# zbqq/aicp_mapping

Hardware: AMD Instinct MI355X
Metric: aligned_clouds_per_s (ICP iterations/sec + aligned clouds/sec, 80-scan VLP-16 batch) (higher is better)
Workload: dtype f32 (point arithmetic; 6x6/3x3 reductions and solves in f64)

## Files before the change

### aicp_mapping_amd/_lib.py

```python
from __future__ import annotations

import ctypes as C
import hashlib
import os

import numpy as np

PKG_DIR = os.path.dirname(os.path.abspath(__file__))
LIB_PATH = os.environ.get("AICP_HIP_LIB") or os.path.join(PKG_DIR, "libaicp_hip.so")

AICP_OK = 0
AICP_ERR_CONVERGENCE = 1
AICP_ERR_INVALID = 2
AICP_ERR_HIP = 3
AICP_ERR_UNSUPPORTED = 4
AICP_ERR_TRANSFORMATION = 5

AICP_RUN_OVERLAP = 1
AICP_RUN_ICP = 2
AICP_RUN_TIME_NN = 4
AICP_SEQ_DEBUG = 8

EXPORTS = [
    "aicp_hip_create", "aicp_hip_destroy", "aicp_hip_last_error", "aicp_hip_version",
    "aicp_hip_default_config", "aicp_hip_parse_pm_yaml", "aicp_hip_replace_ratio_config_file",
    "aicp_hip_autotune_ratio", "aicp_hip_register", "aicp_hip_register_batch",
    "aicp_hip_overlap", "aicp_hip_overlap_batch", "aicp_hip_align_batch", "aicp_hip_transform", "aicp_hip_crop_box",
    "aicp_hip_batch_upload", "aicp_hip_batch_run", "aicp_hip_batch_free",
    "aicp_hip_last_nn_timing", "aicp_hip_last_phase_ms", "aicp_hip_knn", "aicp_hip_normals",
    "aicp_hip_dists_quantile", "aicp_hip_solve6", "aicp_hip_default_prefilter", "aicp_hip_prefilter",
    "aicp_hip_last_prefilter_stats", "aicp_hip_map_create", "aicp_hip_map_free", "aicp_hip_map_size",
    "aicp_hip_map_download", "aicp_hip_map_crop", "aicp_hip_map_merge", "aicp_hip_map_prefilter",
    "aicp_hip_default_sequence_params", "aicp_hip_sequence_run", "aicp_hip_last_sequence_timing",
    "aicp_hip_map_register_batch", "aicp_hip_multi_create", "aicp_hip_multi_destroy", "aicp_hip_multi_size",
    "aicp_hip_multi_context", "aicp_hip_multi_last_error", "aicp_hip_multi_align_batch",
    "aicp_hip_reference_cache_stats", "aicp_hip_default_options", "aicp_hip_set_options", "aicp_hip_get_options",
    "aicp_hip_test_force_scan_stall", "aicp_hip_sequence_run_raw", "aicp_hip_build_info",
]


_NEWEST = {"aicp_hip_reference_cache_stats", "aicp_hip_default_options", "aicp_hip_set_options",
           "aicp_hip_get_options", "aicp_hip_test_force_scan_stall",
           "aicp_hip_sequence_run_raw", "aicp_hip_build_info"}


class IcpConfig(C.Structure):
    _fields_ = [
        ("knn_normals", C.c_int32),
        ("nn_epsilon", C.c_float),
        ("nn_max_dist", C.c_float),
        ("trimmed_ratio", C.c_float),
        ("max_iter", C.c_int32),
        ("min_diff_rot", C.c_float),
        ("min_diff_trans", C.c_float),
        ("smooth_length", C.c_int32),
        ("bucket_size", C.c_int32),
        ("knn_match", C.c_int32),
    ]


class IcpStats(C.Structure):
    _fields_ = [
        ("status", C.c_int32),
        ("iterations", C.c_int32),
        ("converged", C.c_int32),
        ("degenerate_normals", C.c_int32),
        ("inlier_ratio", C.c_float),
        ("trimmed_ratio", C.c_float),
        ("overlap_percent", C.c_float),
        ("tree_depth", C.c_int32),
        ("nn_points_touched", C.c_uint64),
        ("nn_nodes_touched", C.c_uint64),
        ("overlap_keys", C.c_uint64 * 3),
    ]

    def as_dict(self):
        d = {k: getattr(self, k) for k, _ in self._fields_ if k != "overlap_keys"}
        d["overlap_keys"] = [int(x) for x in self.overlap_keys]
        return d


class Pair(C.Structure):
    _fields_ = [
        ("ref", C.POINTER(C.c_float)),
        ("n_ref", C.c_uint64),
        ("ref_stride", C.c_uint64),
        ("read", C.POINTER(C.c_float)),
        ("n_read", C.c_uint64),
        ("read_stride", C.c_uint64),
        ("init_T", C.POINTER(C.c_float)),
        ("ref_origin", C.c_double * 3),
        ("read_origin", C.c_double * 3),
    ]


class PrefilterParams(C.Structure):
    _fields_ = [
        ("leaf_size", C.c_float),
        ("normal_k", C.c_int32),
        ("neighbours", C.c_int32),
        ("min_cluster_size", C.c_int32),
        ("max_cluster_size", C.c_int32),
        ("smoothness_rad", C.c_float),
        ("curvature_threshold", C.c_float),
        ("viewpoint", C.c_float * 3),
    ]


class PrefilterStats(C.Structure):
    _fields_ = [
        ("voxel_ms", C.c_double),
        ("normals_ms", C.c_double),
        ("segment_ms", C.c_double),
        ("device_ms", C.c_double),
        ("wall_ms", C.c_double),
        ("knn_ms", C.c_double),
        ("knn_queries", C.c_uint64),
        ("knn_points_touched", C.c_uint64),
        ("knn_nodes_touched", C.c_uint64),
        ("propagation_passes", C.c_int32),
        ("pad", C.c_int32),
    ]


class Cloud(C.Structure):
    _fields_ = [
# ... 31 lines not shown


class Options(C.Structure):
    _fields_ = [
        ("profile", C.c_int32),
        ("nn_engine", C.c_int32),
        ("overlap_path", C.c_int32),
        ("normals_knn_engine", C.c_int32),
        ("select_pair", C.c_int32),
        ("select_fused_from", C.c_int32),
        ("raw_tree_first", C.c_int32),
        ("raw_first_at", C.c_int32),
        ("no_early_exit", C.c_int32),
        ("tree_plan", C.c_int32),
        ("tree_lvl_min", C.c_uint32),
        ("reference_cache", C.c_int32),
        ("oneshot_keep_mib", C.c_uint32),
        ("early_reference", C.c_int32),
        ("read_order_min", C.c_uint64),
    ]

    def as_dict(self):
        return {k: getattr(self, k) for k, _ in self._fields_}


class SequenceTiming(C.Structure):
    _fields_ = [
        ("windows", C.c_int32),
        ("replans", C.c_int32),
        ("wall_ms", C.c_double),
        ("device_ms", C.c_double),
    ]


def _load():
    if not os.path.exists(LIB_PATH):
        raise ImportError(
            f"{LIB_PATH} is missing: build it with `python -c 'import __graft_entry__ as g; g.build()'` "
            "(hipcc --offload-arch=gfx950). There is no CPU fallback.")
    L = C.CDLL(LIB_PATH)
    for name in EXPORTS:
        if not hasattr(L, name) and not (os.environ.get("AICP_HIP_LIB") and name in _NEWEST):
            raise ImportError(f"{LIB_PATH} does not export {name}")
    vp = C.c_void_p
    fp = C.POINTER(C.c_float)
    dp = C.POINTER(C.c_double)
    ip = C.POINTER(C.c_int32)
    up = C.POINTER(C.c_uint64)
    cfgp = C.POINTER(IcpConfig)
    stp = C.POINTER(IcpStats)
    pp = C.POINTER(Pair)
    sz = C.c_size_t
    L.aicp_hip_create.argtypes = [C.c_int, C.POINTER(vp)]
    L.aicp_hip_destroy.argtypes = [vp]
    L.aicp_hip_destroy.restype = None
    L.aicp_hip_last_error.argtypes = [vp]
    L.aicp_hip_last_error.restype = C.c_char_p
    L.aicp_hip_version.restype = C.c_char_p
    if hasattr(L, "aicp_hip_build_info"):
        L.aicp_hip_build_info.restype = C.c_char_p
    L.aicp_hip_default_config.argtypes = [cfgp]
    L.aicp_hip_default_config.restype = None
    L.aicp_hip_parse_pm_yaml.argtypes = [C.c_char_p, cfgp]
    L.aicp_hip_replace_ratio_config_file.argtypes = [C.c_char_p, C.c_char_p, C.c_float]
    L.aicp_hip_autotune_ratio.argtypes = [C.c_float]
    L.aicp_hip_autotune_ratio.restype = C.c_float
    L.aicp_hip_register.argtypes = [vp, cfgp, pp, fp, stp]
    L.aicp_hip_register_batch.argtypes = [vp, cfgp, pp, sz, fp, stp]
    L.aicp_hip_overlap.argtypes = [vp, pp, C.c_double, fp]
    L.aicp_hip_overlap_batch.argtypes = [vp, pp, sz, C.c_double, fp, stp]
    L.aicp_hip_align_batch.argtypes = [vp, cfgp, pp, sz, C.c_double, C.c_int, fp, stp]
    L.aicp_hip_transform.argtypes = [vp, fp, fp, sz, sz, fp]
    L.aicp_hip_crop_box.argtypes = [vp, fp, sz, sz, C.c_float, C.c_float, fp, fp, C.POINTER(C.c_size_t), fp]
    L.aicp_hip_batch_upload.argtypes = [vp, pp, sz, C.POINTER(vp)]
    L.aicp_hip_batch_run.argtypes = [vp, vp, cfgp, C.c_double, C.c_int, fp, stp]
    L.aicp_hip_batch_free.argtypes = [vp, vp]
    L.aicp_hip_batch_free.restype = None
    L.aicp_hip_last_nn_timing.argtypes = [vp, C.POINTER(C.c_int), dp, dp, up]
    L.aicp_hip_last_phase_ms.argtypes = [vp, dp]
    L.aicp_hip_knn.argtypes = [vp, fp, sz, sz, fp, sz, sz, C.c_int, C.c_float, C.c_float, ip, fp, up]
    L.aicp_hip_normals.argtypes = [vp, fp, sz, sz, C.c_int, fp, ip]
    L.aicp_hip_dists_quantile.argtypes = [vp, fp, sz, C.c_float, fp]
    L.aicp_hip_solve6.argtypes = [vp, dp, dp, dp, ip]
    L.aicp_hip_default_prefilter.argtypes = [C.POINTER(PrefilterParams)]
    L.aicp_hip_default_prefilter.restype = None
    L.aicp_hip_prefilter.argtypes = [vp, C.POINTER(PrefilterParams), fp, sz, sz, fp, C.POINTER(C.c_size_t), fp, ip,
                                     C.POINTER(C.c_size_t), C.POINTER(C.c_size_t)]
    L.aicp_hip_last_prefilter_stats.argtypes = [vp, C.POINTER(PrefilterStats)]
    szp = C.POINTER(C.c_size_t)
    L.aicp_hip_map_create.argtypes = [vp, fp, sz, sz, C.POINTER(vp)]
    L.aicp_hip_map_free.argtypes = [vp, vp]
    L.aicp_hip_map_free.restype = None
    L.aicp_hip_map_size.argtypes = [vp, szp]
    L.aicp_hip_map_download.argtypes = [vp, vp, fp, sz, szp]
    L.aicp_hip_map_crop.argtypes = [vp, vp, C.c_float, C.c_float, fp, fp, sz, szp]
    L.aicp_hip_map_merge.argtypes = [vp, vp, fp, sz, sz, fp]
    L.aicp_hip_map_prefilter.argtypes = [vp, vp, C.POINTER(PrefilterParams)]
    L.aicp_hip_default_sequence_params.argtypes = [C.POINTER(SequenceParams)]
    L.aicp_hip_default_sequence_params.restype = None
    L.aicp_hip_sequence_run.argtypes = [vp, cfgp, C.POINTER(SequenceParams), C.POINTER(Cloud), C.POINTER(Cloud), sz,
                                        fp, C.POINTER(SequenceResult), C.POINTER(C.c_size_t)]
    L.aicp_hip_last_sequence_timing.argtypes = [vp, C.POINTER(SequenceTiming)]
    if hasattr(L, "aicp_hip_sequence_run_raw"):
        L.aicp_hip_sequence_run_raw.argtypes = [vp, cfgp, C.POINTER(SequenceParams), C.POINTER(PrefilterParams),
                                                C.POINTER(Cloud), C.POINTER(Cloud), sz, fp, C.POINTER(SequenceResult),
                                                C.POINTER(C.c_size_t)]
    L.aicp_hip_map_register_batch.argtypes = [vp, cfgp, vp, C.c_float, C.c_float, C.POINTER(Cloud), fp, sz, C.c_int,
                                              fp, stp]
    if hasattr(L, "aicp_hip_reference_cache_stats"):
        L.aicp_hip_reference_cache_stats.argtypes = [vp, C.POINTER(C.c_uint64)]
    if hasattr(L, "aicp_hip_set_options"):
        L.aicp_hip_default_options.argtypes = [C.POINTER(Options)]
        L.aicp_hip_default_options.restype = None
        L.aicp_hip_set_options.argtypes = [vp, C.POINTER(Options)]
        L.aicp_hip_get_options.argtypes = [vp, C.POINTER(Options)]
        L.aicp_hip_test_force_scan_stall.argtypes = [C.c_int]
    L.aicp_hip_multi_create.argtypes = [ip, C.c_int, C.POINTER(vp)]
    L.aicp_hip_multi_destroy.argtypes = [vp]
    L.aicp_hip_multi_destroy.restype = None
    L.aicp_hip_multi_size.argtypes = [vp]
    L.aicp_hip_multi_context.argtypes = [vp, C.c_int]
    L.aicp_hip_multi_context.restype = vp
    L.aicp_hip_multi_last_error.argtypes = [vp]
    L.aicp_hip_multi_last_error.restype = C.c_char_p
    L.aicp_hip_multi_align_batch.argtypes = [vp, cfgp, pp, sz, C.c_double, C.c_int, fp, stp, ip]
    return L


lib = _load()


def build_info() -> str:
    return lib.aicp_hip_build_info().decode() if hasattr(lib, "aicp_hip_build_info") else ""


def source_hash(csrc: str = os.path.join(PKG_DIR, "csrc")) -> str:
    mk = os.path.join(csrc, "Makefile")
    lists = {}
    text = open(mk).read().replace("\\\n", " ")
    for line in text.splitlines():
        for key in ("SRCS_HIP", "SRCS_CPP", "HDRS"):
            if line.startswith(key + " ="):
                lists[key] = line.split("=", 1)[1].split()
    h = hashlib.sha256()
    for f in lists["SRCS_HIP"] + lists["SRCS_CPP"] + lists["HDRS"] + ["Makefile"]:
        with open(os.path.join(csrc, f), "rb") as fh:
            h.update(fh.read())
    return h.hexdigest()[:16]


def provenance() -> dict:
    info = build_info()
    src = info.split()[1] if info.startswith("src ") else ""
    try:
        tree = source_hash()
    except OSError:
        tree = ""
    return {"library": os.path.abspath(LIB_PATH), "build_info": info, "tree_source_hash": tree,
            "built_from_tree": bool(src) and src == tree}


class AicpError(RuntimeError):
    def __init__(self, code, msg):
        super().__init__(f"aicp_hip error {code}: {msg}")
        self.code = code

# ... 58 lines not shown
    ref = as_points(ref)
    read = as_points(read)
    keep = [ref, read]
    p = Pair()
    p.ref = _fptr(ref)
    p.n_ref = ref.shape[0]
    p.ref_stride = ref.shape[1] * 4
    p.read = _fptr(read)
    p.n_read = read.shape[0]
    p.read_stride = read.shape[1] * 4
    if init_T is not None:
        t = np.ascontiguousarray(np.asarray(init_T, np.float32).reshape(4, 4).T.reshape(16))
        keep.append(t)
        p.init_T = _fptr(t)
    for k in range(3):
        p.ref_origin[k] = float(ref_origin[k])
        p.read_origin[k] = float(read_origin[k])
    return p, keep


def default_sequence_params(**kw) -> SequenceParams:
    p = SequenceParams()
    lib.aicp_hip_default_sequence_params(C.byref(p))
    for k, v in kw.items():
        setattr(p, k, v)
    return p


def make_cloud(pts, origin=(0, 0, 0)):
    a = as_points(pts)
    c = Cloud()
    c.pts = _fptr(a)
    c.n = a.shape[0]
    c.stride = a.shape[1] * 4
    for k in range(3):
        c.origin[k] = float(origin[k])
    return c, a


def default_prefilter(**kw) -> PrefilterParams:
    p = PrefilterParams()
    lib.aicp_hip_default_prefilter(C.byref(p))
    for k, v in kw.items():
        if k == "viewpoint":
            for i in range(3):
                p.viewpoint[i] = float(v[i])
        else:
            setattr(p, k, v)
    return p


CONTEXT_OPTIONS: dict = {}


class Context:

    def __init__(self, device: int = 0):
        h = C.c_void_p()
        rc = lib.aicp_hip_create(int(device), C.byref(h))
        if rc != AICP_OK:
            raise AicpError(rc, f"aicp_hip_create(device={device}) failed (no HIP device?)")
        self.h = h
        self.device = device
        if CONTEXT_OPTIONS:
            self.set_options(**CONTEXT_OPTIONS)

    def close(self):
        if getattr(self, "h", None):
            lib.aicp_hip_destroy(self.h)
            self.h = None

    def __del__(self):
        self.close()

    def last_error(self) -> str:
        return lib.aicp_hip_last_error(self.h).decode()

    def get_options(self) -> Options:
        o = Options()
        self.check(lib.aicp_hip_get_options(self.h, C.byref(o)))
        return o

    def set_options(self, opt: Options = None, **kw) -> Options:
        old = self.get_options()
        new = Options.from_buffer_copy(opt if opt is not None else old)
        for k, v in kw.items():
            if not hasattr(new, k):
                raise AttributeError(f"aicp_hip_options has no field {k}")
            setattr(new, k, v)
        self.check(lib.aicp_hip_set_options(self.h, C.byref(new)))
        return old

    def options(self, **kw):
        ctx = self

        class _Scope:
            def __enter__(self):
                self.old = ctx.set_options(**kw)
                return ctx

            def __exit__(self, *exc):
                ctx.set_options(self.old)
                return False

        return _Scope()

    def check(self, rc):
        if rc == AICP_ERR_CONVERGENCE:
            raise ConvergenceError(rc, self.last_error())
        if rc == AICP_ERR_TRANSFORMATION:
            raise TransformationError(rc, self.last_error())
        if rc != AICP_OK:
            raise AicpError(rc, self.last_error())

    def align_batch(self, pairs, cfg=None, resolution=0.2, flags=AICP_RUN_ICP, raise_on_error=True):
        cfg = cfg or default_config()
        arr = (Pair * len(pairs))()
        keep = []
        for i, pr in enumerate(pairs):
            p, k = make_pair(pr["ref"], pr["read"], pr.get("ref_origin", (0, 0, 0)),
                             pr.get("read_origin", (0, 0, 0)), pr.get("init_T"))
            arr[i] = p
            keep.append(k)
        outT = np.zeros((len(pairs), 16), np.float32)
        st = (IcpStats * len(pairs))()
        rc = lib.aicp_hip_align_batch(self.h, C.byref(cfg), arr, len(pairs), float(resolution),
                                      int(flags), _fptr(outT), st)
        if raise_on_error and rc != AICP_OK:
            self.check(rc)
        T = outT.reshape(-1, 4, 4).transpose(0, 2, 1).copy()
        return T, [s.as_dict() for s in st], rc

    def register(self, ref, read, cfg=None):
        cfg = cfg or default_config()
        p, keep = make_pair(ref, read)
        outT = np.zeros(16, np.float32)
        st = IcpStats()
        self.check(lib.aicp_hip_register(self.h, C.byref(cfg), C.byref(p), _fptr(outT), C.byref(st)))
        return outT.reshape(4, 4).T.copy(), st.as_dict()

    def overlap(self, ref, read, ref_origin=(0, 0, 0), read_origin=(0, 0, 0), resolution=0.2):
        p, keep = make_pair(ref, read, ref_origin, read_origin)
        out = np.zeros(1, np.float32)
        self.check(lib.aicp_hip_overlap(self.h, C.byref(p), float(resolution), _fptr(out)))
        return float(out[0])

    def reference_cache_stats(self):
        a = (C.c_uint64 * 4)()
        self.check(lib.aicp_hip_reference_cache_stats(self.h, a))
        return dict(tree_hits=a[0], tree_builds=a[1], ovl_hits=a[2], ovl_builds=a[3])

    def upload(self, pairs):
        return ResidentBatch(self, pairs)

    def sequence_run(self, first, first_origin, readings, origins, cfg=None, params=None, raise_on_error=True,
                     prefilter=None):
        cfg = cfg or default_config()
        prm = params or default_sequence_params()
        if prefilter is True:
            prefilter = default_prefilter()
        n = len(readings)
        fc, keep0 = make_cloud(first, first_origin)
        arr = (Cloud * max(n, 1))()
        keep = [keep0]
        for i, r in enumerate(readings):
            c, k = make_cloud(r, origins[i])
            arr[i] = c
            keep.append(k)
        outT = np.zeros((max(n, 1), 16), np.float32)
        res = (SequenceResult * max(n, 1))()
        done = C.c_size_t(0)
        if prefilter is not None:
            rc = lib.aicp_hip_sequence_run_raw(self.h, C.byref(cfg), C.byref(prm), C.byref(prefilter), C.byref(fc), arr,
                                               n, _fptr(outT), res, C.byref(done))
        else:
            rc = lib.aicp_hip_sequence_run(self.h, C.byref(cfg), C.byref(prm), C.byref(fc), arr, n, _fptr(outT), res,
                                           C.byref(done))
        if raise_on_error and rc != AICP_OK:
            self.check(rc)
        T = outT[:n].reshape(-1, 4, 4).transpose(0, 2, 1).copy()
        return T, [res[i].as_dict() for i in range(done.value)], done.value, rc

    def last_sequence_timing(self):
        t = SequenceTiming()
        self.check(lib.aicp_hip_last_sequence_timing(self.h, C.byref(t)))
        return {k: getattr(t, k) for k, _ in SequenceTiming._fields_}

    def last_nn_timing(self):
        n = C.c_int()
        ms = C.c_double()
        by = C.c_double()
        q = C.c_uint64()
        lib.aicp_hip_last_nn_timing(self.h, C.byref(n), C.byref(ms), C.byref(by), C.byref(q))
        return dict(launches=n.value, total_ms=ms.value, bytes=by.value, queries=q.value)

    def last_phase_ms(self):
        a = (C.c_double * 5)()
        lib.aicp_hip_last_phase_ms(self.h, a)
        return dict(overlap=a[0], normals=a[1], matcher_tree=a[2], icp_loop=a[3], total=a[4])

    def knn(self, pts, queries, k=1, eps=0.0, max_dist=float("inf")):
        pts = as_points(pts)
        q = as_points(queries)
        ids = np.zeros((q.shape[0], k), np.int32)
        d2 = np.zeros((q.shape[0], k), np.float32)
        touched = np.zeros(2, np.uint64)
        rc = lib.aicp_hip_knn(self.h, _fptr(pts), pts.shape[0], pts.shape[1] * 4, _fptr(q), q.shape[0],
                              q.shape[1] * 4, int(k), float(eps), float(max_dist),
                              ids.ctypes.data_as(C.POINTER(C.c_int32)), _fptr(d2),
                              touched.ctypes.data_as(C.POINTER(C.c_uint64)))
        self.check(rc)
        return ids, d2, int(touched[0]), int(touched[1])

    def normals(self, pts, knn=20):
        pts = as_points(pts)
        out = np.zeros((pts.shape[0], 3), np.float32)
        deg = C.c_int32()
        rc = lib.aicp_hip_normals(self.h, _fptr(pts), pts.shape[0], pts.shape[1] * 4, int(knn), _fptr(out),
                                  C.byref(deg))
        self.check(rc)
        return out, deg.value

    def dists_quantile(self, d2, quantile):
        d2 = np.ascontiguousarray(d2, np.float32).ravel()
        out = C.c_float()
        rc = lib.aicp_hip_dists_quantile(self.h, _fptr(d2), d2.size, float(quantile), C.byref(out))
        self.check(rc)
        return out.value

    def solve6(self, A, b):
        A = np.ascontiguousarray(A, np.float64).reshape(36)
        b = np.ascontiguousarray(b, np.float64).reshape(6)
        x = np.zeros(6, np.float64)
        path = C.c_int32()
        dp = C.POINTER(C.c_double)
        rc = lib.aicp_hip_solve6(self.h, A.ctypes.data_as(dp), b.ctypes.data_as(dp), x.ctypes.data_as(dp),
                                 C.byref(path))
        self.check(rc)
        return x, path.value

    def transform(self, T, pts):
        pts = as_points(pts)
        t = np.ascontiguousarray(np.asarray(T, np.float32).reshape(4, 4).T.reshape(16))
        out = np.zeros((pts.shape[0], 3), np.float32)
        rc = lib.aicp_hip_transform(self.h, _fptr(t), _fptr(pts), pts.shape[0], pts.shape[1] * 4, _fptr(out))
        self.check(rc)
        return out

    def crop_box(self, pts, mn, mx, origin):
        pts = as_points(pts)
        o = np.ascontiguousarray(np.asarray(origin, np.float32).reshape(4, 4).T.reshape(16))
        out = np.zeros((pts.shape[0], 3), np.float32)
        m = C.c_size_t(0)
        rpy = np.zeros(3, np.float32)
        rc = lib.aicp_hip_crop_box(self.h, _fptr(pts), pts.shape[0], pts.shape[1] * 4, mn, mx, _fptr(o),
                                   _fptr(out), C.byref(m), _fptr(rpy))
        self.check(rc)
        return out[:m.value].copy(), rpy

    def last_prefilter_stats(self):
        st = PrefilterStats()
        self.check(lib.aicp_hip_last_prefilter_stats(self.h, C.byref(st)))
        return {k: getattr(st, k) for k, _ in PrefilterStats._fields_ if k != "pad"}

    def prefilter(self, pts, params=None, details=False):
        pts = as_points(pts)
        n = pts.shape[0]
        prm = params or default_prefilter()
        out = np.zeros((max(n, 1), 3), np.float32)
        m, ns, nc = C.c_size_t(0), C.c_size_t(0), C.c_size_t(0)
        sampled = np.zeros((max(n, 1), 8), np.float32) if details else None
        labels = np.zeros(max(n, 1), np.int32) if details else None
        rc = lib.aicp_hip_prefilter(self.h, C.byref(prm), _fptr(pts), n, pts.shape[1] * 4, _fptr(out), C.byref(m),
                                    _fptr(sampled) if details else None,
                                    labels.ctypes.data_as(C.POINTER(C.c_int32)) if details else None,
                                    C.byref(ns), C.byref(nc))
        self.check(rc)
        if not details:
            return out[:m.value].copy()
        V = ns.value
        return dict(out=out[:m.value].copy(), sampled=sampled[:V].copy(), labels=labels[:V].copy(),
                    n_clusters=nc.value)


class ResidentBatch:

    def __init__(self, ctx: Context, pairs):
        self.ctx = ctx
        self.n = len(pairs)
        arr = (Pair * self.n)()
        keep = []
        for i, pr in enumerate(pairs):
            p, k = make_pair(pr["ref"], pr["read"], pr.get("ref_origin", (0, 0, 0)),
                             pr.get("read_origin", (0, 0, 0)), pr.get("init_T"))
            arr[i] = p
            keep.append(k)
        h = C.c_void_p()
        rc = lib.aicp_hip_batch_upload(ctx.h, arr, self.n, C.byref(h))
        ctx.check(rc)
        self.h = h
        self.outT = np.zeros((self.n, 16), np.float32)
        self.stats = (IcpStats * self.n)()

    def run(self, cfg=None, resolution=0.2, flags=AICP_RUN_ICP | AICP_RUN_OVERLAP, raise_on_error=True):
        cfg = cfg or default_config()
        rc = lib.aicp_hip_batch_run(self.ctx.h, self.h, C.byref(cfg), float(resolution), int(flags),
                                    _fptr(self.outT), self.stats)
        if raise_on_error and rc != AICP_OK:
            self.ctx.check(rc)
        return rc

    def transforms(self):
        return self.outT.reshape(-1, 4, 4).transpose(0, 2, 1).copy()

    def stats_dicts(self):
        return [s.as_dict() for s in self.stats]

    def free(self):
        if getattr(self, "h", None):
            lib.aicp_hip_batch_free(self.ctx.h, self.h)
# ... 49 lines not shown
```

### aicp_mapping_amd/csrc/aicp_hip.cpp

```cpp
#include <hip/hip_runtime.h>

#include <algorithm>
#include <atomic>
#include <deque>
#include <chrono>
#include <cmath>
#include <cstdio>
#include <cstdlib>
#include <cstring>
#include <limits>
#include <string>
#include <thread>
#include <vector>

#include "../../include/aicp_hip.h"
#include "aicp_common.hpp"
#include "icp_math.hpp"
#include "kernels.hpp"
#include "runtime.hpp"

using namespace aicp;
using namespace aicp::rt;

namespace aicp {
// ... 795 lines not shown
    HIPC(hipEventRecord(ctx->ev[9], s));
    prm.maxE2 = (1 + cfg->nn_epsilon) * (1 + cfg->nn_epsilon);
    prm.maxR2 = cfg->nn_max_dist * cfg->nn_max_dist;
    prm.max_iter = cfg->max_iter;
    prm.smooth = cfg->smooth_length;
    prm.min_rot = cfg->min_diff_rot;
    prm.min_trans = cfg->min_diff_trans;
    prm.knn_normals = cfg->knn_normals;
    uint32_t reads = 0, max_read = 0;
    for (size_t i = 0; i < P; ++i) {
      reads += B->desc[i].n_read;
      max_read = std::max(max_read, B->desc[i].n_read);
    }
    ActiveList* al = ctx->active.as<ActiveList>();
    const int sel_ff = ctx->opt.select_fused_from;
    const bool sel_pair = sel_pair_fits(P, max_read, ctx->opt.select_pair);
    if (!ctx->poll_host) {
      HIPC(hipHostMalloc((void**)&ctx->poll_host, kBatchPolls * 4, hipHostMallocMapped));
      HIPC(hipHostGetDevicePointer((void**)&ctx->poll_dev, ctx->poll_host, 0));
    }
    const bool early = !ctx->opt.no_early_exit;
    auto polled = [&](int k) { return early && k >= cfg->smooth_length && k < kBatchPolls && k < cfg->max_iter; };
    auto written = [&](int k) { return early && k < kBatchPolls; };
    std::deque<int> pending;
    bool stop = false;
    for (int it = 0; it < cfg->max_iter && !stop; ++it) {
      while (!pending.empty() && pending.front() < it && !stop) {
        const int k = pending.front();
        volatile uint32_t* w = ctx->poll_host;
        const auto t0 = std::chrono::steady_clock::now();
        while (w[k] == 0xffffffffu) {
          int m = k - 1;
          while (m >= 0 && w[m] == 0xffffffffu) --m;
          if (m >= 0 && w[m] == 0u) break;
          if (std::chrono::steady_clock::now() - t0 > std::chrono::milliseconds(20)) {
            const hipError_t q = hipStreamQuery(s);
            if (q != hipErrorNotReady) {
              HIPC(q);
              std::atomic_thread_fence(std::memory_order_seq_cst);
              break;
            }
          }
          std::this_thread::yield();
        }
        stop = w[k] == 0u || w[k] == 0xffffffffu;
        pending.pop_front();
      }
      if (stop) break;
      if (it == 0) {
        uint32_t* hn0 = nullptr;
        if (written(0)) {
          ctx->poll_host[0] = 0xffffffffu;
          hn0 = ctx->poll_dev;
        }
        launch_active_list(s, (int)P, dDesc, dState, al, dCtr, hn0);
      }
      prm.prof_slot = nn_launches;
      launch_icp_nn(s, (int)reads, dDesc, dState, al, readc, nodes, ctx->tl_total ? ctx->tl.as<uint4>() : nullptr,
                    nullptr, bpts, ctx->tl_total ? ctx->ptl.as<uint2>() : nullptr, ctx->match.as<int32_t>(),
                    ctx->d2.as<float>(), ctx->touch.as<uint32_t>(), dCtr, prm,
                    timeNN ? ctx->nn_ev[2 * nn_launches] : nullptr, timeNN ? ctx->nn_ev[2 * nn_launches + 1] : nullptr);
      HIPC(hipGetLastError());
      ++nn_launches;
      IcpIterSync y = icp_sync_layout(ctx->isync.as<uint32_t>(), P, 0);
      y.np = (int)P;
      y.pd = dDesc;
      y.st = dState;
      y.al = al;
      y.ctr = dCtr;
      if (written(it + 1)) {
        ctx->poll_host[it + 1] = 0xffffffffu;
        y.host_n = ctx->poll_dev + it + 1;
        if (polled(it + 1)) pending.push_back(it + 1);
      }
      if (sel_pair)
        launch_icp_select_pair(s, (int)P, dDesc, dState, ctx->d2.as<float>(), ctx->sel_cand.as<uint32_t>(), y);
      else if (sel_ff > 0 && it >= sel_ff)
        launch_icp_select_fused(s, B->m_sel, dDesc, dState, ctx->d2.as<float>(), ctx->sel_hist.as<uint32_t>(),
                                ctx->sel_cand.as<uint32_t>(), ctx->sel_cnt.as<uint32_t>(), y);
      else
        launch_icp_select_f(s, B->m_sel, dDesc, dState, ctx->d2.as<float>(), ctx->sel_hist.as<uint32_t>(),
                            ctx->sel_cand.as<uint32_t>(), ctx->sel_cnt.as<uint32_t>(), y);
      launch_icp_reduce_f(s, B->m_red, dDesc, dState, readc, ctx->match.as<int32_t>(), ctx->d2.as<float>(),
                          ctx->touch.as<uint32_t>(), bpts, bnrm, ctx->slab.as<double>(), prm, y);
    }
    launch_finalize(s, (int)P, dDesc, dState, ctx->outT.as<float>());
    if (ctx->opt.profile) {
      HIPC(hipStreamSynchronize(s));
      nn_prof_dump();
      tree_prof_dump();
    }
  } else {
    HIPC(hipEventRecord(ctx->ev[8], s));
    HIPC(hipEventRecord(ctx->ev[10], s));
    HIPC(hipEventRecord(ctx->ev[12], s));
    HIPC(hipEventRecord(ctx->ev[3], s));
    HIPC(hipEventRecord(ctx->ev[4], s));
    HIPC(hipEventRecord(ctx->ev[9], s));
  }
  HIPC(hipGetLastError());
  HIPC(hipEventRecord(ctx->ev[5], s));
  HIPC(hipMemcpyAsync(ctx->pin_state.p, dState, P * sizeof(PairState), hipMemcpyDeviceToHost, s));
  if (doIcp) HIPC(hipMemcpyAsync(ctx->pin_out.p, ctx->outT.p, P * 64, hipMemcpyDeviceToHost, s));
  HIPC(hipMemcpyAsync(pdC, dDesc, P * sizeof(PairDesc), hipMemcpyDeviceToHost, s));
  HIPC(hipStreamSynchronize(s));
  if (doIcp && !hit_trees) {
    rcache.trees = false;
    rc = device_trees_check(ctx->tb[0], ctx->err);
    if (!rc) rc = device_trees_check(ctx->tb[1], ctx->err);
    if (rc) return rc;
    if (ctx->tl_total && (ctx->tb[1].pin_ctl.as<TreeCtl>()->error & 4))
      FAIL(AICP_ERR_HIP, "matcher treelets exceed their allotment");
    if (rcache.use && R == 1) {
      rcache.trees = true;
      rcache.bucket = cfg->bucket_size;
      rcache.knn = cfg->knn_normals;
      rcache.tl_total = ctx->tl_total;
      ++rcache.tree_builds;
    }
  }
  const PairState* hs = ctx->pin_state.as<PairState>();
  int first_err = AICP_OK;
  uint64_t queries = 0, tp = 0, tn = 0;
  for (size_t i = 0; i < P; ++i) {
    const PairState& st = hs[i];
    int status = st.status;
    if (doOvl && st.ovl_err && !status) status = AICP_ERR_HIP;
    if (status && !first_err) first_err = status;
    if (outT && doIcp) std::memcpy(outT + 16 * i, ctx->pin_out.as<float>() + 16 * i, 64);
    if (out_overlap) out_overlap[i] = st.overlap;
    queries += (uint64_t)st.iters * desc[i].n_read;
    const uint64_t ptp = st.touched_pts, ptn = st.touched_nodes;
    tp += ptp;
    tn += ptn;
    if (stats) {
      aicp_icp_stats& o = stats[i];
      std::memset(&o, 0, sizeof(o));
      o.status = status;
      o.iterations = st.iters;
      o.converged = st.converged;
      o.degenerate_normals = st.degenerate;
      o.inlier_ratio = st.inlier_ratio;
      o.trimmed_ratio = st.ratio;
      o.overlap_percent = st.overlap;
      o.tree_depth = pdC[i].tree_depth;
      o.nn_points_touched = ptp;
      o.nn_nodes_touched = ptn;
      for (int k = 0; k < 3; ++k) o.overlap_keys[k] = st.ovl_counts[k];
    }
  }
  ctx->last_nn_launches = timeNN ? nn_launches : 0;
  ctx->last_nn_ms = 0;
  if (timeNN)
    for (int it = 0; it < nn_launches; ++it) ctx->last_nn_ms += ev_ms(ctx->nn_ev[2 * it], ctx->nn_ev[2 * it + 1]);
  ctx->last_nn_bytes = timeNN ? (double)queries * 20.0 + (double)tp * 16.0 + (double)tn * 8.0 : 0.0;
  ctx->last_queries = queries;
  ctx->last_phase[0] = doOvl ? ev_ms(ctx->ev[0], ctx->ev[1]) + ev_ms(ctx->ev[6], ctx->ev[2]) : 0;
  ctx->last_phase[1] = doIcp ? ev_ms(ctx->ev[8], ctx->ev[10]) : 0;
  ctx->last_phase[2] = doIcp ? ev_ms(ctx->ev[12], ctx->ev[3]) : 0;
  ctx->last_phase[3] = doIcp ? ev_ms(ctx->ev[9], ctx->ev[5]) : 0;
  ctx->last_phase[4] =
      std::chrono::duration<double, std::milli>(std::chrono::steady_clock::now() - t_start).count();
  if (first_err) ctx->err = "pair status " + std::to_string(first_err);
  return first_err;
}

void free_batch(aicp_hip_batch* B) {
  if (!B) return;
  release(B->ref_raw);
  release(B->read_raw);
  release(B->maps);
  delete B;
}

int upload_tree(aicp_hip_ctx* ctx, const float* pts, size_t n, size_t stride, PairDesc& d) {
  hipStream_t s = ctx->stream;
  ctx->refc.invalidate();
  HIPC(ensure(ctx->ref1, n * 16));
  HIPC(ensure(ctx->pin_io, n * 16));
  pack_xyz4(pts, n, stride, ctx->pin_io.as<float>());
  HIPC(hipMemcpyAsync(ctx->ref1.p, ctx->pin_io.p, n * 16, hipMemcpyHostToDevice, s));
  d = PairDesc{};
  d.n_ref = (uint32_t)n;
  d.ratio = 0.5f;
  ident4(d.Tin);
  HIPC(ensure(ctx->desc, sizeof(PairDesc)));
  HIPC(hipMemcpyAsync(ctx->desc.p, &d, sizeof(d), hipMemcpyHostToDevice, s));
  int rc = device_trees_begin(ctx->tb[0], ctx->err, s, 1, n, ctx->desc.as<PairDesc>(), ctx->ref1.as<float4>(), 0, 8,
                              ctx->bpts, ctx->nodes);
  if (rc) return rc;
  rc = device_trees_end(ctx->tb[0], ctx->err, s, 1, n, ctx->desc.as<PairDesc>(), 8, ctx->bpts, ctx->nodes, 0);
  if (rc) return rc;
  HIPC(hipMemcpyAsync(&d, ctx->desc.p, sizeof(d), hipMemcpyDeviceToHost, s));
  HIPC(hipStreamSynchronize(s));
  return AICP_OK;
}

}
}

extern "C" {

const char* aicp_hip_version(void) { return "aicp_hip 0.1 (gfx950)"; }

void aicp_hip_default_options(aicp_hip_options* o) {
  if (!o) return;
  *o = aicp_hip_options{};
  o->select_pair = -1;
  o->select_fused_from = 3;
  o->raw_tree_first = -1;
  o->raw_first_at = 2;
  o->tree_lvl_min = 1u << 22;
  o->reference_cache = 1;
  o->oneshot_keep_mib = 4096;
  o->early_reference = 1;
  o->read_order_min = kReadOrderMin;
}

int aicp_hip_set_options(aicp_hip_ctx* ctx, const aicp_hip_options* o) {
  if (!ctx || !o) return AICP_ERR_INVALID;
  if (o->nn_engine < 0 || o->nn_engine > 1 || o->overlap_path < 0 || o->overlap_path > 1 ||
      o->normals_knn_engine < 0 || o->normals_knn_engine > 2 || o->select_pair < -1 || o->select_pair > 1 ||
      o->select_fused_from < 0 || o->raw_tree_first < -1 || o->raw_tree_first > 1 || o->raw_first_at < 1 ||
      o->raw_first_at > 2 || o->tree_plan < -1 || o->reference_cache < 0 || o->reference_cache > 1 ||
      o->early_reference < 0 || o->early_reference > 1)
    FAIL(AICP_ERR_INVALID, "aicp_hip_set_options: value out of range");
  ctx->refc.invalidate();
  ctx->rdc.valid = false;
  ctx->opt = *o;
  for (auto& t : ctx->tb) tree_opts(t, ctx->opt);
  return AICP_OK;
}

int aicp_hip_get_options(const aicp_hip_ctx* ctx, aicp_hip_options* out) {
  if (!ctx || !out) return AICP_ERR_INVALID;
  *out = ctx->opt;
  return AICP_OK;
}

int aicp_hip_test_force_scan_stall(int on) { return set_lb_force_stall(on) == hipSuccess ? AICP_OK : AICP_ERR_HIP; }

int aicp_hip_create(int device, aicp_hip_ctx** out) {
  if (!out) return AICP_ERR_INVALID;
  *out = nullptr;
  int n = 0;
  if (hipGetDeviceCount(&n) != hipSuccess || n <= 0) return AICP_ERR_HIP;
  if (device < 0 || device >= n) return AICP_ERR_INVALID;
  if (hipSetDevice(device) != hipSuccess) return AICP_ERR_HIP;
  aicp_hip_ctx* c = new aicp_hip_ctx();
  c->device = device;
  aicp_hip_default_options(&c->opt);
  for (auto& t : c->tb) tree_opts(t, c->opt);
  int prio_lo = 0, prio_hi = 0;
  if (hipDeviceGetStreamPriorityRange(&prio_lo, &prio_hi) != hipSuccess) prio_lo = prio_hi = 0;
  const int prio3 = prio_hi;
  if (hipStreamCreateWithPriority(&c->stream, hipStreamNonBlocking, prio_lo) != hipSuccess ||
      hipStreamCreateWithPriority(&c->stream2, hipStreamNonBlocking, prio_hi) != hipSuccess ||
      hipStreamCreateWithPriority(&c->stream3, hipStreamNonBlocking, prio3) != hipSuccess) {
    for (hipStream_t q : {c->stream, c->stream2, c->stream3})
      if (q) (void)hipStreamDestroy(q);
    delete c;
    return AICP_ERR_HIP;
  }
  *out = c;
  return AICP_OK;
}

void aicp_hip_destroy(aicp_hip_ctx* ctx) {
  if (!ctx) return;
  (void)hipSetDevice(ctx->device);
  (void)hipDeviceSynchronize();
  for (DevBuf* b : {&ctx->read_s, &ctx->ord_k0, &ctx->ord_k1, &ctx->ord_v0, &ctx->ord_v1, &ctx->ord_tmp, &ctx->read_c, &ctx->bpts, &ctx->bnrm, &ctx->nodes, &ctx->match, &ctx->d2, &ctx->desc,
                    &ctx->state, &ctx->touch, &ctx->slab, &ctx->bitmap, &ctx->outT, &ctx->scratch, &ctx->active,
                    &ctx->ctrs, &ctx->nbids, &ctx->ref1, &ctx->sel_hist, &ctx->sel_cand, &ctx->sel_cnt,
                    &ctx->qmap, &ctx->ovl, &ctx->rdesc, &ctx->rstate, &ctx->rdesc_raw, &ctx->bpts_raw,
                    &ctx->nodes_raw, &ctx->nrm_raw, &ctx->inv, &ctx->gdesc, &ctx->gstate, &ctx->tl, &ctx->ptl,
                    &ctx->tl_rank, &ctx->pf_a, &ctx->pf_b, &ctx->pf_bpts, &ctx->pf_nodes})
    release(*b);
  for (auto& t : ctx->tb) t.release_all();
  free_batch(ctx->oneshot);
  free_batch(ctx->mapbatch);
  release(ctx->crop_ws);
  release(ctx->ovl_sp);
  release(ctx->ovl_keys);
  release(ctx->isync);
  release(ctx->refc.gst);
  release(ctx->pin_crop);
  release(ctx->pin_maps);
  if (ctx->poll_host) (void)hipHostFree(ctx->poll_host);
  delete ctx->pool;
  seq_state_free(ctx->seq);
  for (PinBuf* b : {&ctx->pin_desc, &ctx->pin_state, &ctx->pin_out, &ctx->pin_io, &ctx->pin_ovl,
                    &ctx->pin_rdesc, &ctx->pin_gdesc, &ctx->pin_gstate, &ctx->pin_pf})
    release(*b);
  for (auto e : ctx->nn_ev) (void)hipEventDestroy(e);
  for (auto e : ctx->ev)
    if (e) (void)hipEventDestroy(e);
  for (auto e : ctx->pf_ev)
    if (e) (void)hipEventDestroy(e);
  (void)hipStreamDestroy(ctx->stream);
  if (ctx->stream2) (void)hipStreamDestroy(ctx->stream2);
  if (ctx->stream3) (void)hipStreamDestroy(ctx->stream3);
  delete ctx;
}

const char* aicp_hip_last_error(const aicp_hip_ctx* ctx) { return ctx ? ctx->err.c_str() : "null context"; }

int aicp_hip_batch_upload(aicp_hip_ctx* ctx, const aicp_pair* pairs, size_t n_pairs, aicp_hip_batch** out) {
  if (!ctx || !out) return AICP_ERR_INVALID;
  HIPC(hipSetDevice(ctx->device));
  aicp_hip_batch* B = new aicp_hip_batch();
  const int rc = upload_pairs(ctx, pairs, n_pairs, B, false);
  if (rc) {
    free_batch(B);
    *out = nullptr;
    return rc;
  }
  *out = B;
  return AICP_OK;
}

// ... 332 lines not shown
  HIPC(hipMemcpy(out_ids, ctx->match.p, nq * (size_t)k * 4, hipMemcpyDeviceToHost));
  HIPC(hipMemcpy(out_d2, ctx->d2.p, nq * (size_t)k * 4, hipMemcpyDeviceToHost));
  if (out_touched) HIPC(hipMemcpy(out_touched, ctx->scratch.p, 16, hipMemcpyDeviceToHost));
  return AICP_OK;
}

int aicp_hip_normals(aicp_hip_ctx* ctx, const float* pts, size_t n, size_t stride, int knn, float* out_normals,
                     int32_t* out_degenerate) {
  if (!ctx || !pts || !out_normals || n == 0 || stride < 12) return AICP_ERR_INVALID;
  HIPC(hipSetDevice(ctx->device));
  PairDesc d;
  int rc = upload_tree(ctx, pts, n, stride, d);
  if (rc) return rc;
  hipStream_t st_ = ctx->stream;
  HIPC(ensure(ctx->state, sizeof(PairState)));
  HIPC(ensure(ctx->bnrm, n * 16));
  HIPC(ensure(ctx->nbids, n * 4 * (size_t)std::max(knn, 1)));
  HIPC(ensure(ctx->ctrs, kCtrWords * 4));
  HIPC(hipMemsetAsync(ctx->ctrs.p, 0, kCtrWords * 4, st_));
  launch_init_state(st_, 1, ctx->desc.as<PairDesc>(), ctx->state.as<PairState>());
  if (!launch_normals(st_, 1, (uint32_t)n, ctx->desc.as<PairDesc>(), ctx->state.as<PairState>(),
                      ctx->nodes.as<uint4>(), nullptr, ctx->bpts.as<float4>(),
                      ctx->bnrm.as<float4>(), knn, ctx->nbids.as<int32_t>(), ctx->ctrs.as<uint32_t>(),
                      ctx->opt.normals_knn_engine))
    FAIL(AICP_ERR_UNSUPPORTED, "knn must be 10, 20 or 30");
  HIPC(hipGetLastError());
  HIPC(hipStreamSynchronize(st_));
  std::vector<float> nb(4 * n), bp(4 * n);
  HIPC(hipMemcpy(nb.data(), ctx->bnrm.p, n * 16, hipMemcpyDeviceToHost));
  HIPC(hipMemcpy(bp.data(), ctx->bpts.p, n * 16, hipMemcpyDeviceToHost));
  PairState st;
  HIPC(hipMemcpy(&st, ctx->state.p, sizeof(st), hipMemcpyDeviceToHost));
  for (size_t j = 0; j < n; ++j) {
    int32_t id;
    std::memcpy(&id, &bp[4 * j + 3], 4);
    for (int k = 0; k < 3; ++k) out_normals[3 * (size_t)id + k] = nb[4 * j + k];
  }
  if (out_degenerate) *out_degenerate = st.degenerate;
  return AICP_OK;
}

int aicp_hip_dists_quantile(aicp_hip_ctx* ctx, const float* d2, size_t n, float quantile, float* out_limit) {
  if (!ctx || !d2 || !out_limit || n == 0 || n >= (1ull << 31)) return AICP_ERR_INVALID;
  if (!(quantile >= 0.f && quantile <= 1.f)) return AICP_ERR_INVALID;
  HIPC(hipSetDevice(ctx->device));
  hipStream_t st_ = ctx->stream;
  PairDesc d{};
  d.n_read = (uint32_t)n;
  d.ratio = quantile;
  HIPC(ensure(ctx->desc, sizeof(PairDesc)));
  HIPC(ensure(ctx->state, sizeof(PairState)));
  HIPC(ensure(ctx->d2, n * 4));
  HIPC(ensure(ctx->pin_io, n * 4));
  std::memcpy(ctx->pin_io.p, d2, n * 4);
  HIPC(hipMemcpyAsync(ctx->desc.p, &d, sizeof(d), hipMemcpyHostToDevice, st_));
  HIPC(hipMemcpyAsync(ctx->d2.p, ctx->pin_io.p, n * 4, hipMemcpyHostToDevice, st_));
  const uint32_t per = kNNBlock * kSelPerThread, nb = (uint32_t)((n + per - 1) / per);
  HIPC(ensure(ctx->qmap, (size_t)nb * 8));
  HIPC(ensure(ctx->pin_desc, (size_t)nb * 8));
  uint32_t* hm = ctx->pin_desc.as<uint32_t>();
  for (uint32_t b = 0; b < nb; ++b) {
    hm[b] = 0;
    hm[nb + b] = b * per;
  }
  HIPC(hipMemcpyAsync(ctx->qmap.p, hm, (size_t)nb * 8, hipMemcpyHostToDevice, st_));
  BlockMap qm{ctx->qmap.as<int32_t>(), ctx->qmap.as<uint32_t>() + nb, nb};
  HIPC(ensure(ctx->sel_hist, kHistBins * 4));
  HIPC(ensure(ctx->sel_cand, n * 4));
  HIPC(ensure(ctx->sel_cnt, 4));
  HIPC(hipMemsetAsync(ctx->sel_hist.p, 0, kHistBins * 4, st_));
  HIPC(hipMemsetAsync(ctx->sel_cnt.p, 0, 4, st_));
  launch_init_state(st_, 1, ctx->desc.as<PairDesc>(), ctx->state.as<PairState>());
  launch_icp_select(st_, qm, 1, ctx->desc.as<PairDesc>(), ctx->state.as<PairState>(), ctx->d2.as<float>(),
                    ctx->sel_hist.as<uint32_t>(), ctx->sel_cand.as<uint32_t>(), ctx->sel_cnt.as<uint32_t>());
  HIPC(hipGetLastError());
  HIPC(hipStreamSynchronize(st_));
  PairState st;
  HIPC(hipMemcpy(&st, ctx->state.p, sizeof(st), hipMemcpyDeviceToHost));
  if (st.status) FAIL(st.status, "no outlier to filter");
  *out_limit = st.limit;
  return AICP_OK;
}

int aicp_hip_solve6(aicp_hip_ctx* ctx, const double* A, const double* b, double* out_x, int32_t* out_path) {
  if (!ctx || !A || !b || !out_x) return AICP_ERR_INVALID;
  HIPC(hipSetDevice(ctx->device));
  HIPC(ensure(ctx->scratch, 8 * (36 + 6 + 6) + 8));
  char* d = ctx->scratch.as<char>();
  HIPC(hipMemcpy(d, A, 36 * 8, hipMemcpyHostToDevice));
  HIPC(hipMemcpy(d + 288, b, 6 * 8, hipMemcpyHostToDevice));
  launch_solve6(ctx->stream, (const double*)d, (const double*)(d + 288), (double*)(d + 336), (int32_t*)(d + 384));
  HIPC(hipGetLastError());
  HIPC(hipStreamSynchronize(ctx->stream));
  HIPC(hipMemcpy(out_x, d + 336, 48, hipMemcpyDeviceToHost));
  int32_t path = 0;
  HIPC(hipMemcpy(&path, d + 384, 4, hipMemcpyDeviceToHost));
  if (out_path) *out_path = path;
  return AICP_OK;
}

void aicp_hip_default_prefilter(aicp_prefilter_params* p) {
  if (!p) return;
  *p = aicp_prefilter_params{};
  p->leaf_size = 0.08f;
  p->normal_k = 30;
  p->neighbours = 15;
  p->min_cluster_size = 50;
  p->max_cluster_size = 1000000;
  p->smoothness_rad = (float)(3.0 / 180.0 * M_PI);
  p->curvature_threshold = 1.0f;
}

struct PfRun {
  uint32_t V = 0, n_out = 0, n_clusters = 0;
  const float4* out4 = nullptr;
  const float4* nrm = nullptr;
  const uint32_t* inv = nullptr;
  const int32_t* cluster_of = nullptr;
};
struct PfHost {
  PfCtl hc;
  unsigned long long ht[2];
  uint32_t tl_err;
  uint32_t hf[2];
};
struct PfLayout {
  PfCtl* ctl;
  float4* pts4;
  PfWork W;
};

static int pf_check(aicp_hip_ctx* ctx, const aicp_prefilter_params* prm) {
  if (!(prm->leaf_size > 0.f) || !std::isfinite(prm->leaf_size)) FAIL(AICP_ERR_INVALID, "leaf size must be > 0");
  const int K = prm->normal_k, NB = prm->neighbours;
  if (K != 10 && K != 20 && K != 30) FAIL(AICP_ERR_UNSUPPORTED, "normal_k must be 10, 20 or 30");
  if (NB < 1 || NB > kPfMaxNbrs || NB > K) FAIL(AICP_ERR_UNSUPPORTED, "neighbours must be 1..min(16, normal_k)");
  return AICP_OK;
}

static int pf_layout(aicp_hip_ctx* ctx, size_t n, PfLayout* L) {
  const size_t wn = (n + 1 + 63) & ~size_t(63);
  const size_t temp_b = pf_temp_bytes(n + 1);
  const size_t off_pts = 256, off_w = off_pts + n * 16, off_temp = off_w + 9 * wn * 4;
  HIPC(ensure(ctx->pf_a, off_temp + temp_b));
  char* A = ctx->pf_a.as<char>();
  uint32_t* wb = (uint32_t*)(A + off_w);
  L->ctl = (PfCtl*)A;
  L->pts4 = (float4*)(A + off_pts);
  L->W = PfWork{wb, wb + wn, wb + 2 * wn, wb + 3 * wn, wb + 4 * wn, wb + 5 * wn, wb + 6 * wn, wb + 7 * wn, wb + 8 * wn,
                A + off_temp, temp_b};
  return AICP_OK;
}

static int pf_core(aicp_hip_ctx* ctx, const aicp_prefilter_params* prm, size_t n, const PfLayout& Lo, PfRun* o) {
  hipStream_t s = ctx->stream;
  const int K = prm->normal_k, NB = prm->neighbours;
  for (auto& e : ctx->pf_ev)
    if (!e) HIPC(hipEventCreate(&e));
  hipEvent_t* E = ctx->pf_ev;
  PfCtl* dctl = Lo.ctl;
  const PfWork& W = Lo.W;
  HIPC(ensure(ctx->ref1, n * 16));
  HIPC(ensure(ctx->pin_pf, sizeof(PfHost)));
  HIPC(hipStreamSynchronize(s));
  PfHost& H = *ctx->pin_pf.as<PfHost>();
  PfCtl& hc = H.hc;
  hc = PfCtl{};
  for (int k = 0; k < 3; ++k) hc.lo[k] = 0xFFFFFFFFu;
  HIPC(hipMemcpyAsync(dctl, &hc, sizeof(hc), hipMemcpyHostToDevice, s));
  HIPC(hipStreamSynchronize(s));
  HIPC(hipEventRecord(E[0], s));
  HIPC(launch_pf_voxel(s, (uint32_t)n, Lo.pts4, 1.f / prm->leaf_size, dctl, W, ctx->ref1.as<float4>()));
  HIPC(hipEventRecord(E[1], s));
  HIPC(hipMemcpyAsync(&hc, dctl, sizeof(hc), hipMemcpyDeviceToHost, s));
  HIPC(hipStreamSynchronize(s));
  if (hc.passthrough && hc.n_bad)
    FAIL(AICP_ERR_UNSUPPORTED, "voxel grid overflows 32-bit indices and the cloud has non-finite points");
  const uint32_t V = hc.n_fin ? hc.n_vox : 0u;
  *o = PfRun{};
  o->V = V;
  if (V == 0) return AICP_OK;
// ... 493 lines not shown
```

### aicp_mapping_amd/csrc/icp_math.hpp

```cpp
#pragma once
#include <hip/hip_runtime.h>
#include <math.h>
#include <stdint.h>

#define AICP_HD __host__ __device__ inline

namespace aicp {

constexpr float kFltEps = 1.1920928955078125e-07f;
constexpr double kDblEps = 2.220446049250313e-16;
constexpr double kDblMin = 2.2250738585072014e-308;

AICP_HD float m4(const float* m, int r, int c) { return m[c * 4 + r]; }

AICP_HD void mul4(const float* A, const float* B, float* C) {
  float t[16];
  for (int c = 0; c < 4; ++c)
    for (int r = 0; r < 4; ++r) {
      float s = m4(A, r, 0) * m4(B, 0, c);
      s += m4(A, r, 1) * m4(B, 1, c);
      s += m4(A, r, 2) * m4(B, 2, c);
      s += m4(A, r, 3) * m4(B, 3, c);
      t[c * 4 + r] = s;
    }
  for (int i = 0; i < 16; ++i) C[i] = t[i];
}

AICP_HD void apply4(const float* T, float x, float y, float z, float* o) {
  for (int r = 0; r < 3; ++r) {
    float s = m4(T, r, 0) * x;
    s += m4(T, r, 1) * y;
    s += m4(T, r, 2) * z;
    s += m4(T, r, 3);
    o[r] = s;
  }
}

AICP_HD void ident4(float* T) {
  for (int i = 0; i < 16; ++i) T[i] = (i % 5 == 0) ? 1.f : 0.f;
}

AICP_HD bool rigid_ok(const float* T) {
  const float d0 = m4(T, 0, 0) * (m4(T, 1, 1) * m4(T, 2, 2) - m4(T, 1, 2) * m4(T, 2, 1));
  const float d1 = m4(T, 1, 0) * (m4(T, 0, 1) * m4(T, 2, 2) - m4(T, 0, 2) * m4(T, 2, 1));
  const float d2 = m4(T, 2, 0) * (m4(T, 0, 1) * m4(T, 1, 2) - m4(T, 0, 2) * m4(T, 1, 1));
  const float det = (d0 - d1) + d2;
  return !(fabsf(1.f - det) > 0.001f);
}

AICP_HD void delta_transform(const float* x, float* T) {
  const float sq = (x[0] * x[0] + x[1] * x[1]) + x[2] * x[2];
  const float angle = sqrtf(sq);
  float axis[3] = {x[0], x[1], x[2]};
  if (sq > 0.f) {
    for (int i = 0; i < 3; ++i) axis[i] = x[i] / angle;
  }
  const float sa = (float)sin((double)angle);
  const float c = (float)cos((double)angle);
  float sin_axis[3], cos1_axis[3];
  for (int i = 0; i < 3; ++i) {
    sin_axis[i] = sa * axis[i];
    cos1_axis[i] = (1.f - c) * axis[i];
  }
  float R[9];
  float tmp = cos1_axis[0] * axis[1];
  R[0 * 3 + 1] = tmp - sin_axis[2];
  R[1 * 3 + 0] = tmp + sin_axis[2];
  tmp = cos1_axis[0] * axis[2];
  R[0 * 3 + 2] = tmp + sin_axis[1];
  R[2 * 3 + 0] = tmp - sin_axis[1];
  tmp = cos1_axis[1] * axis[2];
  R[1 * 3 + 2] = tmp - sin_axis[0];
  R[2 * 3 + 1] = tmp + sin_axis[0];
  for (int i = 0; i < 3; ++i) R[i * 3 + i] = cos1_axis[i] * axis[i] + c;
  bool nan = false;
  for (int r = 0; r < 3; ++r)
    for (int cc = 0; cc < 3; ++cc) {
      T[cc * 4 + r] = R[r * 3 + cc];
      nan |= (R[r * 3 + cc] != R[r * 3 + cc]);
    }
  for (int r = 0; r < 3; ++r) {
    T[12 + r] = x[3 + r];
    nan |= (x[3 + r] != x[3 + r]);
  }
  T[3] = T[7] = T[11] = 0.f;
  T[15] = 1.f;
  if (nan)
    for (int r = 0; r < 3; ++r)
      for (int cc = 0; cc < 3; ++cc) T[cc * 4 + r] = (r == cc) ? 1.f : 0.f;
}

AICP_HD void quat_from_T(const float* T, double* q) {
  double m[3][3];
  for (int r = 0; r < 3; ++r)
    for (int c = 0; c < 3; ++c) m[r][c] = (double)m4(T, r, c);
  double t = (m[0][0] + m[1][1]) + m[2][2];
  if (t > 0) {
    t = sqrt(t + 1.0);
    q[0] = 0.5 * t;
    t = 0.5 / t;
    q[1] = (m[2][1] - m[1][2]) * t;
    q[2] = (m[0][2] - m[2][0]) * t;
    q[3] = (m[1][0] - m[0][1]) * t;
  } else {
    int i = 0;
    if (m[1][1] > m[0][0]) i = 1;
    if (m[2][2] > m[i][i]) i = 2;
    const int j = (i + 1) % 3, k = (j + 1) % 3;
    t = sqrt(m[i][i] - m[j][j] - m[k][k] + 1.0);
    double v[3];
    v[i] = 0.5 * t;
    t = 0.5 / t;
    q[0] = (m[k][j] - m[j][k]) * t;
    v[j] = (m[j][i] + m[i][j]) * t;
    v[k] = (m[k][i] + m[i][k]) * t;
    q[1] = v[0];
    q[2] = v[1];
    q[3] = v[2];
  }
}

AICP_HD double quat_angdist(const double* a, const double* b) {
  const double bw = b[0], bx = -b[1], by = -b[2], bz = -b[3];
  const double w = a[0] * bw - a[1] * bx - a[2] * by - a[3] * bz;
  const double x = a[0] * bx + a[1] * bw + a[2] * bz - a[3] * by;
  const double y = a[0] * by + a[2] * bw + a[3] * bx - a[1] * bz;
  const double z = a[0] * bz + a[3] * bw + a[1] * by - a[2] * bx;
  return 2.0 * atan2(sqrt(x * x + y * y + z * z), fabs(w));
}

#define AICP_UNROLL _Pragma("unroll")

template <int N>
struct PivQR {
  int nonzero, rank;
  double a[N * N];
  double tau[N];
  int rowT[N], colT[N];
  double maxpivot;
};

template <int N>
AICP_HD void pivqr(const double* A, PivQR<N>& q) {
  AICP_UNROLL for (int i = 0; i < N * N; ++i) q.a[i] = A[i];
  const double prec = (double)kFltEps * N;
  q.nonzero = N;
  q.maxpivot = 0;
  double biggest = 0;
  bool stop = false;
  AICP_UNROLL for (int k = 0; k < N; ++k) {
    if (stop) {
      q.rowT[k] = k;
      q.colT[k] = k;
      q.tau[k] = 0;
      continue;
    }
    int br = k, bc = k;
    double bv = -1;
    AICP_UNROLL for (int c = k; c < N; ++c)
      AICP_UNROLL for (int r = k; r < N; ++r) {
        const double v = fabs(q.a[r * N + c]);
        if (v > bv) {
          bv = v;
          br = r;
          bc = c;
        }
      }
    if (k == 0) biggest = bv;
    if (bv <= biggest * prec) {
      q.nonzero = k;
      q.rowT[k] = k;
      q.colT[k] = k;
      q.tau[k] = 0;
      stop = true;
      continue;
    }
    q.rowT[k] = br;
    q.colT[k] = bc;
    AICP_UNROLL for (int r = k + 1; r < N; ++r)
      if (r == br)
        AICP_UNROLL for (int c = k; c < N; ++c) {
          const double t = q.a[k * N + c];
          q.a[k * N + c] = q.a[r * N + c];
          q.a[r * N + c] = t;
        }
    AICP_UNROLL for (int c = k + 1; c < N; ++c)
      if (c == bc)
        AICP_UNROLL for (int r = 0; r < N; ++r) {
          const double t = q.a[r * N + k];
          q.a[r * N + k] = q.a[r * N + c];
          q.a[r * N + c] = t;
        }
    double tailSq = 0;
    AICP_UNROLL for (int r = k + 1; r < N; ++r) tailSq += q.a[r * N + k] * q.a[r * N + k];
    const double c0 = q.a[k * N + k];
    double beta, tau;
    if (tailSq <= kDblMin) {
      tau = 0;
      beta = c0;
      AICP_UNROLL for (int r = k + 1; r < N; ++r) q.a[r * N + k] = 0;
    } else {
// ... 136 lines not shown
    const int r = qr.rank;
    double Q[36];
    pivqr_Q<6>(qr, Q);
    int perm[6];
    AICP_UNROLL for (int i = 0; i < n; ++i) perm[i] = i;
    AICP_UNROLL for (int k = 0; k < n; ++k) {
      const int c = (k < qr.nonzero) ? qr.colT[k] : k;
      AICP_UNROLL for (int j = k + 1; j < n; ++j)
        if (j == c) {
          const int t = perm[k];
          perm[k] = perm[j];
          perm[j] = t;
        }
    }
    double AP[36];
    AICP_UNROLL for (int j = 0; j < n; ++j)
      AICP_UNROLL for (int k = 0; k < n; ++k) {
        double v = A[k * n + 0];
        AICP_UNROLL for (int c = 1; c < n; ++c) v = (perm[j] == c) ? A[k * n + c] : v;
        AP[k * n + j] = v;
      }
    double R1[36], RRt[36], qb[6], y[6];
    AICP_UNROLL for (int i = 0; i < n; ++i)
      if (i < r)
        AICP_UNROLL for (int j = 0; j < n; ++j) {
          double s = 0;
          AICP_UNROLL for (int k = 0; k < n; ++k) s += Q[k * n + i] * AP[k * n + j];
          R1[i * n + j] = s;
        }
    AICP_UNROLL for (int i = 0; i < n; ++i)
      AICP_UNROLL for (int j = 0; j < n; ++j)
        if (i < r && j < r) {
          double s = 0;
          AICP_UNROLL for (int k = 0; k < n; ++k) s += R1[i * n + k] * R1[j * n + k];
          RRt[i * n + j] = s;
        }
    AICP_UNROLL for (int i = 0; i < n; ++i)
      if (i < r) {
        double s = 0;
        AICP_UNROLL for (int k = 0; k < n; ++k) s += Q[k * n + i] * b[k];
        qb[i] = s;
      }
    if (llt_solve<6>(RRt, r, qb, y)) {
      double z[6];
      AICP_UNROLL for (int j = 0; j < n; ++j) {
        double s = 0;
        AICP_UNROLL for (int i = 0; i < n; ++i)
          if (i < r && j >= i) s += R1[i * n + j] * y[i];
        z[j] = s;
      }
      AICP_UNROLL for (int c = 0; c < n; ++c) {
        double v = 0;
        AICP_UNROLL for (int i = 0; i < n; ++i) v = (perm[i] == c) ? z[i] : v;
        x[c] = v;
      }
      double nb = 0, nax = 0, nd = 0;
      AICP_UNROLL for (int i = 0; i < n; ++i) {
        double s = 0;
        AICP_UNROLL for (int k = 0; k < n; ++k) s += A[i * n + k] * x[k];
        nb += b[i] * b[i];
        nax += s * s;
        nd += (b[i] - s) * (b[i] - s);
      }
      if (nd <= 1e-10 * (nb < nax ? nb : nax)) return 1;
    }
  }
  double w[6], V[36];
  jacobi_eig<6>(A, w, V);
  double wmax = 0;
  AICP_UNROLL for (int i = 0; i < n; ++i) wmax = fmax(wmax, fabs(w[i]));
  double thr = wmax * (n * kDblEps);
  if (thr < kDblMin) thr = kDblMin;
  AICP_UNROLL for (int i = 0; i < n; ++i) x[i] = 0;
  AICP_UNROLL for (int e = 0; e < n; ++e) {
    if (fabs(w[e]) <= thr) continue;
    double s = 0;
    AICP_UNROLL for (int k = 0; k < n; ++k) s += V[k * n + e] * b[k];
    s /= w[e];
    AICP_UNROLL for (int k = 0; k < n; ++k) x[k] += V[k * n + e] * s;
  }
  return 2;
}

AICP_HD bool normal_from_cov(const double* C, float* nrm) {
  PivQR<3> qr;
  pivqr<3>(C, qr);
  if (qr.rank + 1 >= 3) {
    double w[3], V[9];
    jacobi_eig<3>(C, w, V);
    int s = 0;
    double sv = 1.79769313486231570e308;
    AICP_UNROLL for (int j = 0; j < 3; ++j)
      if (w[j] < sv) {
        sv = w[j];
        s = j;
      }
    AICP_UNROLL for (int r = 0; r < 3; ++r) nrm[r] = (float)(s == 0 ? V[r * 3] : (s == 1 ? V[r * 3 + 1] : V[r * 3 + 2]));
    return false;
  }
  nrm[0] = 0.f;
  nrm[1] = 1.f;
  nrm[2] = 0.f;
  return true;
}

AICP_HD void corrected_origin(const float* T, const double* o, double* out) {
  float m[3][3];
  for (int r = 0; r < 3; ++r)
    for (int c = 0; c < 3; ++c) m[r][c] = T[c * 4 + r];
  float q[4];
  float t = (m[0][0] + m[1][1]) + m[2][2];
  if (t > 0.f) {
    t = (float)sqrt((double)(t + 1.f));
    q[3] = 0.5f * t;
    t = 0.5f / t;
    q[0] = (m[2][1] - m[1][2]) * t;
    q[1] = (m[0][2] - m[2][0]) * t;
    q[2] = (m[1][0] - m[0][1]) * t;
  } else {
    int i = 0;
    if (m[1][1] > m[0][0]) i = 1;
    if (m[2][2] > m[i][i]) i = 2;
    const int j = (i + 1) % 3, k = (j + 1) % 3;
    t = (float)sqrt((double)(((m[i][i] - m[j][j]) - m[k][k]) + 1.f));
    q[i] = 0.5f * t;
    t = 0.5f / t;
    q[3] = (m[k][j] - m[j][k]) * t;
    q[j] = (m[j][i] + m[i][j]) * t;
    q[k] = (m[k][i] + m[i][k]) * t;
  }
  const double x = q[0], y = q[1], z = q[2], w = q[3];
  const double tx = 2.0 * x, ty = 2.0 * y, tz = 2.0 * z;
  const double twx = tx * w, twy = ty * w, twz = tz * w;
  const double txx = tx * x, txy = ty * x, txz = tz * x;
  const double tyy = ty * y, tyz = tz * y, tzz = tz * z;
  const double R[3][3] = {{1.0 - (tyy + tzz), txy - twz, txz + twy},
                          {txy + twz, 1.0 - (txx + tzz), tyz - twx},
                          {txz - twy, tyz + twx, 1.0 - (txx + tyy)}};
  for (int r = 0; r < 3; ++r) out[r] = ((R[r][0] * o[0] + R[r][1] * o[1]) + R[r][2] * o[2]) + (double)T[12 + r];
}

AICP_HD bool correction_rejected(const float* T, float max_corr) {
  return fabsf(T[12]) > max_corr || fabsf(T[13]) > max_corr || fabsf(T[14]) > max_corr;
}

AICP_HD float quantize_ratio_fast(float r) {
  const double m = rint((double)r * 1e6);
  return (float)(m / 1e6);
}

AICP_HD float autotune_ratio_fast(float overlap_percent) {
  float cur = (float)(overlap_percent / 100.0);
  if (cur < 0.25)
    cur = 0.25f;
  else if (cur > 0.70)
    cur = 0.70f;
  if (cur != cur) return cur;
  return quantize_ratio_fast(cur);
}

}

namespace aicp {

AICP_HD int64_t fixed40(float x) {
  const double v = rint((double)x * 1099511627776.0);
// ... 19 lines not shown
```

### aicp_mapping_amd/csrc/kernels.hpp

```cpp
#pragma once
#include <hip/hip_runtime.h>
#include <stdint.h>

#include "aicp_common.hpp"

namespace aicp {

struct BlockMap {
  const int32_t* pair;
  const uint32_t* start;
  uint32_t n_blocks;
};

void launch_prepare_read(hipStream_t s, BlockMap m, const PairDesc* pd, const float4* read_raw,
                         float4* read_c);
size_t read_order_temp_bytes(size_t n, int n_pairs);
hipError_t launch_read_order(hipStream_t s, BlockMap m, int n_pairs, const PairDesc* pd, const float4* raw,
                             uint32_t total, uint64_t* keys0, uint64_t* keys1, uint32_t* vals0, uint32_t* vals1,
                             void* temp, size_t temp_bytes, float4* out);
void launch_gather_ref(hipStream_t s, BlockMap m, const PairDesc* pd, const float4* ref_raw,
                       const int32_t* perm, float4* bpts);
void launch_init_state(hipStream_t s, int n_pairs, const PairDesc* pd, PairState* st);
bool launch_normals(hipStream_t s, int n_pairs, uint32_t total_ref, const PairDesc* pd, PairState* st,
                    const uint4* nodes, const int32_t* parent, const float4* bpts, float4* bnrm, int knn,
                    int32_t* ids, uint32_t* ctr, int engine);
bool launch_knn_ids(hipStream_t s, int n_pairs, uint32_t total_ref, const PairDesc* pd, const uint4* nodes,
                    const float4* bpts, int knn, int32_t* ids, uint32_t* ctr, unsigned long long* touched,
                    int engine);
void launch_active_list(hipStream_t s, int n_pairs, const PairDesc* pd, const PairState* st,
                        ActiveList* al, uint32_t* ctr, uint32_t* host_n = nullptr, uint64_t* done_sig = nullptr,
                        const uint64_t* ticket = nullptr, float* outT = nullptr, int src_pair = -1);
struct IcpIterSync {
  uint32_t* sel1;
  uint32_t* sel2;
  uint32_t* red;
  uint32_t* pairs;
  int np;
  const PairDesc* pd;
  PairState* st;
  ActiveList* al;
  uint32_t* ctr;
  uint32_t* host_n;
  uint64_t* done_sig;
  const uint64_t* ticket;
  float* outT;
  int src_pair = -1;
};
void tree_prof_dump();
void iter_prof_dump();
inline size_t icp_sync_words(size_t n_pairs) { return 3 * n_pairs + 2; }
IcpIterSync icp_sync_layout(uint32_t* words, size_t n_pairs, int group);
void launch_icp_select_f(hipStream_t s, BlockMap m, const PairDesc* pd, PairState* st, const float* d2,
                         uint32_t* hist1, uint32_t* cand, uint32_t* cand_cnt, const IcpIterSync& y);
void launch_icp_select_pair(hipStream_t s, int n_pairs, const PairDesc* pd, PairState* st, const float* d2,
                            uint32_t* cand, const IcpIterSync& y);
bool sel_pair_fits(size_t n_pairs, uint64_t max_read, int force);
void launch_icp_select_fused(hipStream_t s, BlockMap m, const PairDesc* pd, PairState* st, const float* d2,
                             uint32_t* hist1, uint32_t* cand, uint32_t* cand_cnt, const IcpIterSync& y);
void launch_icp_reduce_f(hipStream_t s, BlockMap m, const PairDesc* pd, PairState* st, const float4* read_c,
                         const int32_t* match, const float* d2, const uint32_t* touched, const float4* bpts,
                         const float4* bnrm, double* slab, const IcpParams& prm, const IcpIterSync& y);
void launch_icp_nn(hipStream_t s, int grid_items, const PairDesc* pd, const PairState* st,
                   const ActiveList* al, const float4* read_c, const uint4* nodes, const uint4* tl,
                   const int32_t* parent, const float4* bpts, const uint2* ptl, int32_t* match, float* d2,
                   uint32_t* touched, uint32_t* ctr, const IcpParams& prm, hipEvent_t e0 = nullptr,
                   hipEvent_t e1 = nullptr);
void launch_icp_select(hipStream_t s, BlockMap m, int n_pairs, const PairDesc* pd, PairState* st,
                       const float* d2, uint32_t* hist1, uint32_t* cand, uint32_t* cand_cnt, int p0 = 0);
void launch_icp_reduce(hipStream_t s, BlockMap m, const PairDesc* pd, const PairState* st,
                       const float4* read_c, const int32_t* match, const float* d2,
                       const uint32_t* touched, const float4* bpts, const float4* bnrm, double* slab);
void launch_icp_update(hipStream_t s, int n_pairs, const PairDesc* pd, PairState* st,
                       const double* slab, const IcpParams& prm);
void launch_finalize(hipStream_t s, int n_pairs, const PairDesc* pd, PairState* st,
                     float* outT);

void nn_prof_dump();

bool launch_knn_generic(hipStream_t s, uint32_t nq, const float4* q, const uint4* nodes,
                        const int32_t* parent, const float4* bpts, int k, float maxE2,
                        float maxR2, int32_t* ids, float* d2, unsigned long long* touched,
                        uint32_t* ctr);
void launch_transform(hipStream_t s, int n, const float* T, const float4* in, float4* out);
size_t crop_tiles(size_t n);
void launch_crop_box(hipStream_t s, int n, const float inv[9], const float t[3], float mn, float mx,
                     const float4* pts, uint32_t* tile_cnt, uint32_t* tile_off, uint32_t* total,
                     float4* out);
size_t crop_args_bytes();
void pack_crop_args(const float inv[9], const float t[3], float mn, float mx, void* dst);
void launch_crop_count_multi(hipStream_t s, int n, int n_crops, const void* args, const float4* pts,
                             uint32_t* tile_cnt, uint32_t* tile_off, uint32_t* totals);
void launch_crop_scatter_multi(hipStream_t s, int n, int n_crops, const void* args, const float4* pts,
                               const uint32_t* tile_off, const uint32_t* base_of, float4* out);
void launch_solve6(hipStream_t s, const double* A, const double* b, double* x, int32_t* path);

struct TreeWork {
  float4* W[2];
  int32_t* segof[2];
  TreeSeg* seg[2];
  uint32_t* flag;
  uint32_t* X1;
  uint32_t* X2;
  uint32_t* posL;
  uint32_t* posR;
  NodeEvent* ev;
  uint8_t* valid;
  SubSeg* subs;
  SubSeg* mids;
  uint32_t* ecnt;
  uint64_t* sums;
  int32_t* pair_depth;
  TreeCtl* ctl;
  void* scan_temp;
  size_t scan_temp_bytes;
  size_t max_seg;
  int n_pairs;
  uint64_t* lb;
  size_t lb_stride;
  uint32_t mid_max;
  uint32_t lvl_min;
};
uint32_t tree_mid_max();
hipError_t set_lb_force_stall(int on);
size_t tree_sum_tiles(size_t n);
size_t tree_scan_temp_bytes(size_t n);
size_t lb_bytes(uint32_t total);
size_t lb_stride_words(uint32_t total);
hipError_t launch_treelets(hipStream_t s, int n_refs, uint32_t cap, const PairDesc* rd, const uint4* nodes,
                           int bucket, uint32_t* rank, uint4* tl, uint2* link, const TreeWork& w);
hipError_t launch_tree_prepare(hipStream_t s, int n_pairs, uint32_t total, PairDesc* pd, const float4* raw,
                               int center, const TreeWork& w, float4* bpts, int bucket, int part = 0);
hipError_t launch_tree_level(hipStream_t s, int level, uint32_t total, const TreeWork& w, float4* bpts,
                             int bucket, bool last);
hipError_t launch_tree_mid(hipStream_t s, uint32_t total, const TreeWork& w, float4* bpts, int bucket);
hipError_t launch_tree_subtrees(hipStream_t s, uint32_t total, const TreeWork& w, float4* bpts,
                                int bucket);
hipError_t launch_tree_finish(hipStream_t s, int n_pairs, uint32_t total, PairDesc* pd, const TreeWork& w,
                              uint4* nodes);

void launch_pairs_from_refs(hipStream_t s, int n_pairs, PairDesc* pd, const PairDesc* rd);
void launch_normals_to_matcher(hipStream_t s, int n_refs, uint32_t total, const PairDesc* rd, const float4* bpts,
                               const float4* bpts_raw, const float4* nrm_raw, uint32_t* inv, float4* bnrm);
void launch_pairs_degenerate(hipStream_t s, int n_pairs, const PairDesc* pd, PairState* st, const PairState* rst);
void launch_pairs_degenerate_part(hipStream_t s, int n_pairs, const PairDesc* pd, PairState* st, const PairState* rst,
                                  int what);

void launch_ovl_init(hipStream_t s, int n, const PairDesc* pd, PairState* st, double res, int sides);
void launch_ovl_bbox(hipStream_t s, BlockMap m, const PairDesc* pd, PairState* st,
                     const float4* pts, int side, double res);
void launch_ovl_mark(hipStream_t s, BlockMap m, const PairDesc* pd, const OvlDesc* od, PairState* st,
                     const float4* pts, int side, double res, uint8_t* maps, bool filter,
                     unsigned max_blocks = 0);
void launch_ovl_count(hipStream_t s, int n_pairs, int n_groups, const PairDesc* pd, const OvlDesc* od_read,
                      const OvlDesc* od_ref, PairState* st, PairState* gst, const uint8_t* maps);
void launch_ovl_popcount(hipStream_t s, int n, const OvlDesc* od, PairState* st, int slot, const uint8_t* maps,
                         bool wide = false);
void launch_ovl_intersect(hipStream_t s, int n_pairs, const PairDesc* pd, const OvlDesc* od_read, const OvlDesc* od_ref,
                          PairState* st, const uint8_t* maps, bool wide = false);
void launch_ovl_finish(hipStream_t s, int n_pairs, const PairDesc* pd, PairState* st, const PairState* gst,
                       int set_ratio);

size_t ovl_sparse_scan_bytes(size_t n_points);
size_t ovl_sparse_sort_bytes(size_t n_keys);
hipError_t launch_ovl_sparse_count(hipStream_t s, uint32_t n_blocks, const uint32_t* blk_cloud,
                                   const uint32_t* blk_start, const OvlCloud* clouds, const float4* ref,
                                   const float4* read, double res, uint32_t n_points, uint32_t* cnt, uint64_t* off,
                                   void* temp, size_t temp_bytes);
hipError_t launch_ovl_sparse_sets(hipStream_t s, uint32_t n_blocks, const uint32_t* blk_cloud,
                                  const uint32_t* blk_start, const OvlCloud* clouds, const float4* ref,
                                  const float4* read, double res, const uint64_t* off, uint64_t n_keys,
                                  uint64_t* keys0, uint64_t* keys1, void* temp, size_t temp_bytes, int n_groups,
                                  int n_pairs, const PairDesc* pd, unsigned long long* per_cloud,
                                  unsigned long long* per_pair, PairState* gst, PairState* st);

struct OvlKeySide {
  OvlCloud* clouds;
  int n_clouds;
// ... 70 lines not shown
```

### aicp_mapping_amd/csrc/kernels_icp.hip

```cpp
#include <hip/hip_ext.h>
#include <hip/hip_runtime.h>

#include <algorithm>
#include <atomic>
#include <type_traits>
#include <cstdio>

#include <cstdlib>

#include "aicp_common.hpp"
#include "icp_math.hpp"
#include "kernels.hpp"

namespace aicp {

template <int K>
struct Best {
  float v[K];
  int32_t id[K];
};

template <int K>
__device__ __forceinline__ void best_init(Best<K>& b) {
#pragma unroll
// ... 577 lines not shown
struct is_coop<Trav2C> {
  static constexpr bool value = true;
};

constexpr int kDppXor1 = 0xB1, kDppXor2 = 0x4E, kDppHalfMirror = 0x141;

__device__ __forceinline__ float octet_min(float v) {
  v = fminf(v, __int_as_float(__builtin_amdgcn_mov_dpp(__float_as_int(v), kDppXor1, 0xF, 0xF, false)));
  v = fminf(v, __int_as_float(__builtin_amdgcn_mov_dpp(__float_as_int(v), kDppXor2, 0xF, 0xF, false)));
  v = fminf(v, __int_as_float(__builtin_amdgcn_mov_dpp(__float_as_int(v), kDppHalfMirror, 0xF, 0xF, false)));
  return v;
}

template <class Eng>
__device__ __forceinline__ void coop_bucket(Eng& t, bool act, const float4* __restrict__ pts, float maxR2,
                                            float4* xch) {
  const int lane = threadIdx.x & 63;
  const int oct = lane & ~7, i = lane & 7;
  const uint32_t cnt = act ? min(t.lcnt, (uint32_t)kLeafBatch) : 0u;
  xch[lane] = make_float4(t.q0, t.q1, t.q2, __uint_as_float(((t.pbase + t.lb0) << 4) | cnt));
  __builtin_amdgcn_wave_barrier();
  float3 P[kLeafBatch];
#pragma unroll
  for (int j = 0; j < kLeafBatch; ++j) {
    const uint32_t w = __float_as_uint(xch[oct + j].w);
    if ((uint32_t)i < (w & 15u)) {
      const float4 p = pts[(w >> 4) + i];
      P[j] = make_float3(p.x, p.y, p.z);
    }
  }
  float res_d = __builtin_inff();
  uint32_t res_i = 0;
#pragma unroll
  for (int j = 0; j < kLeafBatch; ++j) {
    float dist = __builtin_inff();
    const float4 Q = xch[oct + j];
    if ((uint32_t)i < (__float_as_uint(Q.w) & 15u)) {
      const float d0 = Q.x - P[j].x, d1 = Q.y - P[j].y, d2 = Q.z - P[j].z;
      float d = 0.f;
      d += d0 * d0;
      d += d1 * d1;
      d += d2 * d2;
      if (d <= maxR2) dist = d;
    }
    const float m = octet_min(dist);
    const uint32_t hit = (uint32_t)(__ballot(dist == m) >> oct) & 0xFFu;
    if (i == j) {
      res_d = m;
      res_i = (uint32_t)__builtin_ctz(hit | 0x100u);
    }
  }
  __builtin_amdgcn_wave_barrier();
  if (act && res_d < t.best.v[0]) best_replace<1>(t.best, (int32_t)(t.lb0 + res_i), res_d);
}

#if AICP_XCD_PROF
__device__ unsigned long long g_xcd_prof[64 * kXcdGroups * 2];
__device__ unsigned long long g_xcd_cost[64 * kXcdGroups];
#endif
#if AICP_QLAT_PROF
__device__ unsigned long long g_qlat[512];
#endif
#if AICP_NN_PROF
__device__ unsigned long long g_nn_prof[8];
#endif
#if AICP_ITER_PROF
__device__ unsigned long long g_iter_prof[16];
#define AICP_IP_T0 const uint64_t ip_t0 = __builtin_amdgcn_s_memrealtime()
#define AICP_IP_BODY(k)                                                                          \
  do {                                                                                           \
    if (threadIdx.x == 0) {                                                                      \
      atomicAdd(&g_iter_prof[4 * (k)], (unsigned long long)(__builtin_amdgcn_s_memrealtime() - ip_t0)); \
      atomicAdd(&g_iter_prof[4 * (k) + 1], 1ull);                                                \
    }                                                                                            \
  } while (0)
#define AICP_IP_TAIL0 const uint64_t ip_t1 = __builtin_amdgcn_s_memrealtime()
#define AICP_IP_TAIL(k)                                                                          \
  do {                                                                                           \
    if (threadIdx.x == 0) {                                                                      \
      atomicAdd(&g_iter_prof[4 * (k) + 2], (unsigned long long)(__builtin_amdgcn_s_memrealtime() - ip_t1)); \
      atomicAdd(&g_iter_prof[4 * (k) + 3], 1ull);                                                \
    }                                                                                            \
  } while (0)
#else
#define AICP_IP_T0 \
  do {             \
  } while (0)
#define AICP_IP_BODY(k) \
  do {                  \
  } while (0)
#define AICP_IP_TAIL0 \
  do {                \
  } while (0)
#define AICP_IP_TAIL(k) \
  do {                  \
  } while (0)
#endif

__device__ __forceinline__ uint32_t head_lo(uint32_t lo, uint32_t hi, uint32_t h) {
  return h >= (uint32_t)kHeads ? hi : lo + ((uint32_t)(((uint64_t)(hi - lo) * h) / kHeads) & ~63u);
}
template <class Eng, class OnChunk, class Fetch, class Done>
__device__ __forceinline__ void persistent_xcd(uint32_t total, uint32_t* ctr, float maxE2, float maxR2,
                                               const uint4* __restrict__ nodes, const float4* __restrict__ pts,
                                               OnChunk&& on_chunk, Fetch&& fetch, Done&& done) {
  const int lane = threadIdx.x & 63;
  const uint32_t g = blockIdx.x % kXcdGroups;
  const uint32_t lo = (uint32_t)(((uint64_t)total * g) / kXcdGroups) & ~63u;
  const uint32_t hi = g + 1 == kXcdGroups ? total : (uint32_t)(((uint64_t)total * (g + 1)) / kXcdGroups) & ~63u;
  uint32_t* gctr = ctr + g * kGroupCtrs * kCtrStride;
  uint32_t h = ((blockIdx.x / kXcdGroups) * (blockDim.x >> 6) + (threadIdx.x >> 6)) % kHeads;
  h = __builtin_amdgcn_readfirstlane(h);
  Eng t;
  typename Eng::Stack fs;
  bool has = false;
  uint32_t pool = 0, pool_end = 0, my = 0;
  bool exhausted = false;
#if AICP_NN_PROF
  uint64_t pf_t = __builtin_amdgcn_s_memtime(), pf_fill = 0, pf_desc = 0, pf_buck = 0, pf_climb = 0, pf_rounds = 0,
           pf_lanes = 0;
#define AICP_PF(acc)                                    \
  do {                                                  \
    const uint64_t now_ = __builtin_amdgcn_s_memtime(); \
    acc += now_ - pf_t;                                 \
    pf_t = now_;                                        \
  } while (0)
#else
#define AICP_PF(acc) \
  do {               \
  } while (0)
#endif
  for (;;) {
    for (;;) {
      const uint64_t needm = __ballot(!has);
      if (needm == 0 || exhausted) break;
      if (pool >= pool_end) {
        uint32_t base = 0, end = 0;
        for (;;) {
          const uint32_t hl = head_lo(lo, hi, h);
          end = head_lo(lo, hi, h + 1);
          uint32_t b = 0;
          if (lane == 0) b = atomicAdd(gctr + h * kCtrStride, 64u);
          base = hl + __builtin_amdgcn_readfirstlane(b);
          if (base < end) break;
          uint32_t m = 0;
          if (lane == 0) m = atomicOr(gctr + kHeads * kCtrStride, 1u << h);
          m = __builtin_amdgcn_readfirstlane(m) | (1u << h);
          if (m == (1u << kHeads) - 1u) {
            exhausted = true;
            break;
          }
          h = (uint32_t)__builtin_ctz(~m & ((1u << kHeads) - 1u));
        }
        if (exhausted) break;
        pool = base;
        pool_end = min(base + 64u, end);
        if constexpr (std::is_invocable_v<OnChunk, uint32_t, Eng&>) on_chunk(base, t);
        else on_chunk(base);
      }
      const uint32_t rank = (uint32_t)__popcll(needm & ((1ull << lane) - 1ull));
      const uint32_t avail = pool_end - pool;
      if (!has && rank < avail) {
        my = pool + rank;
        has = fetch(my, t);
      }
      pool += min(avail, (uint32_t)__popcll(needm));
    }
// ... 43 lines not shown
#if AICP_NN_PROF
  if (lane == 0) {
    atomicAdd(&g_nn_prof[0], (unsigned long long)pf_fill);
    atomicAdd(&g_nn_prof[1], (unsigned long long)pf_desc);
    atomicAdd(&g_nn_prof[2], (unsigned long long)pf_buck);
    atomicAdd(&g_nn_prof[3], (unsigned long long)pf_climb);
    atomicAdd(&g_nn_prof[4], (unsigned long long)pf_rounds);
    atomicAdd(&g_nn_prof[5], (unsigned long long)pf_lanes);
  }
#endif
}

__device__ __forceinline__ void block_map(const BlockMap& m, int& pair, uint32_t& local) {
  pair = m.pair[blockIdx.x];
  local = m.start[blockIdx.x] + threadIdx.x;
}

__global__ __launch_bounds__(256) void k_prepare_read(BlockMap m, const PairDesc* __restrict__ pd,
                                                      const float4* __restrict__ raw,
                                                      float4* __restrict__ out) {
  int pair;
  uint32_t j;
  block_map(m, pair, j);
  const PairDesc& d = pd[pair];
  if (j >= d.n_read) return;
  const float4 p = raw[d.read_off + j];
  float o[3];
  apply4(d.Tinit, p.x, p.y, p.z, o);
  out[d.read_off + j] = make_float4(o[0], o[1], o[2], 1.f);
}

__global__ __launch_bounds__(256) void k_gather_ref(BlockMap m, const PairDesc* __restrict__ pd,
                                                    const float4* __restrict__ raw,
                                                    const int32_t* __restrict__ perm,
                                                    float4* __restrict__ bpts) {
  int pair;
  uint32_t j;
  block_map(m, pair, j);
  const PairDesc& d = pd[pair];
  if (j >= d.n_ref) return;
  const int32_t id = perm[d.ref_off + j];
  const float4 p = raw[d.ref_off + id];
  bpts[d.ref_off + j] =
      make_float4(p.x - d.mean[0], p.y - d.mean[1], p.z - d.mean[2], __int_as_float(id));
}

__global__ void k_init_state(int n_pairs, const PairDesc* __restrict__ pd, PairState* st) {
  const int p = blockIdx.x * blockDim.x + threadIdx.x;
  if (p >= n_pairs) return;
  PairState& s = st[p];
  ident4(s.T);
  s.limit = 0.f;
  s.ratio = pd[p].ratio;
  s.active = 1;
  s.status = 0;
  s.iters = 0;
  s.converged = 0;
  s.kept = 0;
  s.n_finite = 0;
  s.hist_count = 1;
  s.degenerate = 0;
  s.inlier_ratio = 0.f;
  s.overlap = -1.f;
  s.touched_pts = 0;
  s.touched_nodes = 0;
  for (int i = 0; i < 3; ++i) s.ovl_counts[i] = 0;
  s.ovl_err = 0;
  s.sel_b1 = 0;
  s.sel_r1 = 0;
  s.sel_miss = 0;
  quat_from_T(s.T, s.qh[0]);
  s.th[0][0] = s.th[0][1] = s.th[0][2] = 0.0;
}

__device__ void active_list_body(int n_pairs, const PairDesc* __restrict__ pd, const PairState* __restrict__ st,
                                 ActiveList* al, uint32_t* ctr, uint32_t* host_n, uint64_t* done_sig,
                                 const uint64_t* ticket, float* outT, int src_pair) {
  __shared__ uint32_t wsum[16];
  __shared__ uint32_t wcnt[16];
  __shared__ uint32_t carry_off, carry_cnt;
  __shared__ uint32_t r_off[1024];
  const int t = threadIdx.x, lane = t & 63, wave = t >> 6, nt = (int)blockDim.x, nw = nt >> 6;
  uint16_t* chunk = al_chunks(al);
  if (t == 0) carry_off = carry_cnt = 0;
  if (t < kXcdGroups * kGroupCtrs) ctr[t * kCtrStride] = 0;
  __syncthreads();
  for (int base = 0; base < n_pairs; base += nt) {
    const int p = base + t;
    const bool a = p < n_pairs && st[p].active;
    const uint32_t v = a ? (pd[p].n_read + 63u) & ~63u : 0u;
    uint32_t x = v, c = a ? 1u : 0u;
#pragma unroll
    for (int off = 1; off < 64; off <<= 1) {
      const uint32_t y = __shfl_up(x, off, 64), z = __shfl_up(c, off, 64);
      if (lane >= off) {
        x += y;
        c += z;
      }
    }
    if (lane == 63) {
      wsum[wave] = x;
      wcnt[wave] = c;
    }
    __syncthreads();
    const uint32_t e0 = carry_cnt, o0 = carry_off;
    uint32_t bo = o0, bc = e0;
    for (int w = 0; w < wave; ++w) {
      bo += wsum[w];
      bc += wcnt[w];
    }
    uint32_t rn = 0, rs = 0;
    for (int w = 0; w < nw; ++w) {
      rn += wcnt[w];
      rs += wsum[w];
    }
    if (a) {
      const uint32_t e = bc + c - 1, o = bo + x - v;
      al->pair[e] = p;
      al->off[e] = o;
      const PairDesc& d = pd[p];
      al->ent[e] = NnEntry{o, d.n_read, d.read_off, d.tl_off, d.node_off, d.ref_off, p, 0u};
      r_off[e - e0] = o;
    }
    __syncthreads();
    for (uint32_t i = (uint32_t)wave; i < rn; i += (uint32_t)nw) {
      const uint32_t c0 = r_off[i] >> 6, c1 = (i + 1 < rn ? r_off[i + 1] : o0 + rs) >> 6;
      for (uint32_t j = c0 + (uint32_t)lane; j < c1; j += 64) chunk[j] = (uint16_t)(e0 + i);
    }
    if (t == nt - 1) {
      carry_off = bo + x;
      carry_cnt = bc + c;
    }
    __syncthreads();
  }
  if (t == 0) {
    al->n = carry_cnt;
    al->total = carry_off;
    al->off[carry_cnt] = carry_off;
    const bool src_on = src_pair >= 0 && src_pair < n_pairs && st[src_pair].active;
    if (host_n)
      __hip_atomic_store(host_n, carry_cnt | (src_on ? 0x80000000u : 0u), __ATOMIC_RELAXED, __HIP_MEMORY_SCOPE_SYSTEM);
  }
  if (done_sig && carry_cnt == 0) {
    for (int p = t; p < n_pairs; p += nt) {
      float tmp[16];
      mul4(pd[p].Tmean, st[p].T, tmp);
      mul4(tmp, pd[p].Tinit, outT + 16 * (size_t)p);
    }
    __threadfence_system();
    __syncthreads();
    if (t == 0) __hip_atomic_store(done_sig, *ticket, __ATOMIC_RELEASE, __HIP_MEMORY_SCOPE_SYSTEM);
  }
}

__global__ __launch_bounds__(256) void k_active_list(int n_pairs, const PairDesc* __restrict__ pd,
                                                      const PairState* __restrict__ st,
                                                      ActiveList* al, uint32_t* ctr, uint32_t* host_n,
                                                      uint64_t* done_sig, const uint64_t* ticket, float* outT,
                                                      int src_pair) {
  active_list_body(n_pairs, pd, st, al, ctr, host_n, done_sig, ticket, outT, src_pair);
}

__device__ __forceinline__ bool last_arrival(uint32_t* cnt, uint32_t n_expected) {
  __shared__ uint32_t s_last;
  asm volatile("s_waitcnt vmcnt(0)" ::: "memory");
  __syncthreads();
  if (threadIdx.x == 0) {
    __builtin_amdgcn_fence(__ATOMIC_RELEASE, "agent");
    asm volatile("s_waitcnt vmcnt(0)" ::: "memory");
    const uint32_t old = atomicAdd(cnt, 1u);
    const bool last = old + 1 == n_expected;
    if (last) {
      __hip_atomic_store(cnt, 0u, __ATOMIC_RELAXED, __HIP_MEMORY_SCOPE_AGENT);
      __builtin_amdgcn_fence(__ATOMIC_ACQUIRE, "agent");
      asm volatile("s_waitcnt vmcnt(0)" ::: "memory");
    }
    s_last = last ? 1u : 0u;
  }
  __syncthreads();
  return s_last != 0;
}

__device__ __forceinline__ int pair_of_ref(const PairDesc* __restrict__ pd, int n_pairs, uint32_t s) {
  int lo = 0, hi = n_pairs - 1;
  while (lo < hi) {
    const int mid = (lo + hi + 1) >> 1;
    if (pd[mid].ref_off <= s) lo = mid;
    else hi = mid - 1;
  }
  return lo;
}

template <int K>
#ifndef AICP_KNN_WAVES
#define AICP_KNN_WAVES 0
#endif
#if AICP_KNN_WAVES > 0
#define AICP_KNN_ATTR __attribute__((amdgpu_waves_per_eu(AICP_KNN_WAVES)))
#else
#define AICP_KNN_ATTR
#endif
__global__ __launch_bounds__(256) AICP_KNN_ATTR void k_knn_ids(int n_pairs, uint32_t total, const PairDesc* __restrict__ pd,
                                                 const uint4* __restrict__ nodes,
                                                 const int32_t* __restrict__ parent,
                                                 const float4* __restrict__ bpts,
                                                 int32_t* __restrict__ ids, uint32_t* ctr,
                                                 unsigned long long* touched) {
  __shared__ LdsFrame knn_frames[(kKnnLdsFrames > 0 ? kKnnLdsFrames : 1) * kNNBlock];
  uint32_t tp = 0, tn = 0;
  int cur = -1;
  uint32_t cur_end = 0, cur_off = 0;
  persistent_xcd<Trav<K>>(
      total, ctr, 1.f, __builtin_inff(), nodes, bpts, [](uint32_t) {},
      [&](uint32_t s, Trav<K>& t) {
        if (cur < 0 || s < cur_off || s >= cur_end) {
          cur = pair_of_ref(pd, n_pairs, s);
          cur_off = pd[cur].ref_off;
          cur_end = cur_off + pd[cur].n_ref;
        }
        const PairDesc& d = pd[cur];
        t.nodes = nodes + d.node_off;
        t.pts = bpts + d.ref_off;
// ... 1191 lines not shown
    }
    if (fabs(beta) > maxpivot) maxpivot = fabs(beta);
    double v[N];
#pragma unroll
    for (int r = k + 1; r < N; ++r) v[r] = bcast_d(col[r], k);
    if (lane > k && lane < N) {
      double sum = col[k];
#pragma unroll
      for (int r = k + 1; r < N; ++r) sum += v[r] * col[r];
      sum *= tau;
      col[k] -= sum;
#pragma unroll
      for (int r = k + 1; r < N; ++r) col[r] -= sum * v[r];
    }
  }
  const double thr = fabs(maxpivot) * ((double)kFltEps * N);
  int rank = 0;
#pragma unroll
  for (int i = 0; i < N; ++i)
    if (i < nonzero) rank += fabs(bcast_d(col[i], i)) > thr ? 1 : 0;
  return rank;
}

template <class Get>
__device__ bool wave_llt_solve6(Get get, const double* b, double* x) {
  constexpr int N = 6;
  const int lane = threadIdx.x & 63;
  const int i = lane < N ? lane : 0;
  double L[N];
#pragma unroll
  for (int k = 0; k < N; ++k) L[k] = 0;
  bool ok = true;
#pragma unroll
  for (int j = 0; j < N; ++j) {
    double Lj[N];
#pragma unroll
    for (int k = 0; k < j; ++k) Lj[k] = bcast_d(L[k], j);
    double d = get(j, j);
#pragma unroll
    for (int k = 0; k < j; ++k) d -= Lj[k] * Lj[k];
    if (!(d > 0)) ok = false;
    const double ljj = sqrt(d);
    if (lane == j) L[j] = ljj;
    if (lane > j && lane < N) {
      double sum = get(i, j);
#pragma unroll
      for (int k = 0; k < j; ++k) sum -= L[k] * Lj[k];
      L[j] = sum / ljj;
    }
  }
  if (!ok) return false;
  double y[N];
#pragma unroll
  for (int r = 0; r < N; ++r) {
    double Lr[N];
#pragma unroll
    for (int k = 0; k <= r; ++k) Lr[k] = bcast_d(L[k], r);
    double sum = b[r];
#pragma unroll
    for (int k = 0; k < r; ++k) sum -= Lr[k] * y[k];
    y[r] = sum / Lr[r];
  }
#pragma unroll
  for (int r = N - 1; r >= 0; --r) {
    double sum = y[r];
#pragma unroll
    for (int k = r + 1; k < N; ++k) sum -= bcast_d(L[r], k) * x[k];
    x[r] = sum / bcast_d(L[r], r);
  }
  return true;
}

__device__ __forceinline__ void normal_system(const double* tot, double* A, double* b) {
  int c = 0;
  for (int a = 0; a < 6; ++a)
    for (int bb = a; bb < 6; ++bb) {
      A[a * 6 + bb] = tot[c];
      A[bb * 6 + a] = tot[c];
      ++c;
    }
  for (int a = 0; a < 6; ++a) b[a] = -tot[21 + a];
}

__device__ void update_serial(const PairDesc& d, PairState& s, const double* tot, const IcpParams& prm,
                              const double* x_full) {
  s.touched_pts += (uint64_t)tot[28];
  s.touched_nodes += (uint64_t)tot[29];
  const int32_t kept = (int32_t)tot[27];
  s.kept = kept;
  if (kept == 0) {
    s.status = 1;
    s.active = 0;
    return;
  }
  double xd[6];
  if (x_full) {
    for (int a = 0; a < 6; ++a) xd[a] = x_full[a];
  } else {
    double A[36], b[6];
    normal_system(tot, A, b);
    solve6(A, b, xd);
  }
  float x[6];
  for (int a = 0; a < 6; ++a) x[a] = (float)xd[a];
  float dT[16];
  delta_transform(x, dT);
  mul4(dT, s.T, s.T);
  s.inlier_ratio = (float)((double)(float)kept / (double)d.n_read);
  if (!rigid_ok(s.T)) {
    s.iters += 1;
    s.status = 5;
    s.active = 0;
    return;
  }
  bool iterate = true;
  s.iters += 1;
  if (s.iters >= prm.max_iter) iterate = false;
  const int h = s.hist_count % kHistRing;
  quat_from_T(s.T, s.qh[h]);
  for (int i = 0; i < 3; ++i) s.th[h][i] = (double)s.T[12 + i];
  if (s.hist_count >= 1) {
    const int bprev = (s.hist_count - 1) % kHistRing;
    s.dq[h] = fabs(quat_angdist(s.qh[h], s.qh[bprev]));
    const double dx = s.th[h][0] - s.th[bprev][0];
    const double dy = s.th[h][1] - s.th[bprev][1];
    const double dz = s.th[h][2] - s.th[bprev][2];
    s.dt[h] = sqrt(dx * dx + dy * dy + dz * dz);
  }
  s.hist_count += 1;
  const int sz = s.hist_count;
  if (sz > prm.smooth) {
    double cv0 = 0, cv1 = 0;
    for (int i = sz - 1; i >= sz - prm.smooth; --i) {
      const int a = i % kHistRing;
      cv0 += s.dq[a];
      cv1 += s.dt[a];
    }
    cv0 /= prm.smooth;
    cv1 /= prm.smooth;
    if (cv0 != cv0 || cv1 != cv1) {
      s.status = 1;
      s.active = 0;
      return;
    }
    if (cv0 < (double)prm.min_rot && cv1 < (double)prm.min_trans) {
      if (iterate) s.converged = 1;
      iterate = false;
    }
  }
  s.active = iterate ? 1 : 0;
}

__device__ void icp_update_body(const PairDesc& d, PairState& s, const double* __restrict__ slab,
                                const IcpParams& prm) {
  constexpr int kGroups = 256 / kRedCols;
  __shared__ double part[kGroups][kRedCols];
  __shared__ double tot[kRedCols];
  const int t = threadIdx.x;
  if (t < kGroups * kRedCols) {
    const int g = t / kRedCols, c = t - g * kRedCols;
    const double* col = slab + (size_t)d.red_blk_off * kRedCols + c;
    double v = 0.0;
    for (uint32_t r0 = g; r0 < d.n_red_blk; r0 += 16u * kGroups) {
      double x[16];
#pragma unroll
      for (int u = 0; u < 16; ++u) {
        const uint32_t r = r0 + (uint32_t)u * kGroups;
        x[u] = r < d.n_red_blk ? col[(size_t)r * kRedCols] : 0.0;
      }
#pragma unroll
      for (int u = 0; u < 16; ++u)
        if (r0 + (uint32_t)u * kGroups < d.n_red_blk) v += x[u];
    }
    part[g][c] = v;
  }
  __syncthreads();
  if (t < kRedCols) {
    double v = part[0][t];
#pragma unroll
    for (int g = 1; g < kGroups; ++g) v += part[g][t];
    tot[t] = v;
  }
  __syncthreads();
  __shared__ int rank_llt[2];
  __shared__ double xs[6];
  auto tri = [&](int r, int c) {
    const int a = r < c ? r : c, bb = r < c ? c : r;
    return tot[a * 6 - a * (a - 1) / 2 + (bb - a)];
  };
  if (t >= 64 && t < 128) {
    double b[6], x[6];
    for (int a = 0; a < 6; ++a) b[a] = -tot[21 + a];
    const bool ok = wave_llt_solve6(tri, b, x);
    if (t == 64) {
      rank_llt[1] = ok ? 1 : 0;
      for (int a = 0; a < 6; ++a) xs[a] = x[a];
    }
  }
  if (t < 64) {
    const int rk = wave_pivqr_rank6(tri);
    if (t == 0) rank_llt[0] = rk;
  }
  __syncthreads();
  if (t == 0) update_serial(d, s, tot, prm, rank_llt[0] == 6 && rank_llt[1] ? xs : nullptr);
}

__global__ __launch_bounds__(256) void k_icp_update(const PairDesc* __restrict__ pd, PairState* st,
                                                    const double* __restrict__ slab, IcpParams prm) {
  const int pair = blockIdx.x;
  PairState& s = st[pair];
  if (!s.active) return;
  icp_update_body(pd[pair], s, slab, prm);
}

__global__ __launch_bounds__(256) void k_icp_update_f(const PairDesc* __restrict__ pd, PairState* st,
                                                      const double* __restrict__ slab, IcpParams prm, IcpIterSync y) {
  AICP_IP_T0;
  const int pair = blockIdx.x;
  PairState& s = st[pair];
  if (!s.active) return;
  icp_update_body(pd[pair], s, slab, prm);
  AICP_IP_BODY(3);
  AICP_IP_TAIL0;
  pair_done(y);
  AICP_IP_TAIL(3);
}

__global__ void k_finalize(int n_pairs, const PairDesc* __restrict__ pd,
                           PairState* __restrict__ st, float* __restrict__ outT) {
  const int p = blockIdx.x * blockDim.x + threadIdx.x;
  if (p >= n_pairs) return;
  float tmp[16], T[16];
  mul4(pd[p].Tmean, st[p].T, tmp);
  mul4(tmp, pd[p].Tinit, T);
  for (int i = 0; i < 16; ++i) outT[p * 16 + i] = T[i];
  if (st[p].status == 0 && !rigid_ok(T)) st[p].status = 5;
}

template <int K>
__global__ __launch_bounds__(256) void k_knn_generic(uint32_t nq, const float4* __restrict__ q,
                                                     const uint4* __restrict__ nodes,
                                                     const int32_t* __restrict__ parent,
                                                     const float4* __restrict__ bpts, float maxE2,
                                                     float maxR2, int32_t* __restrict__ ids,
                                                     float* __restrict__ d2, unsigned long long* touched,
                                                     uint32_t* ctr) {
  uint32_t tp = 0, tn = 0;
  persistent_xcd<Trav<K>>(
      nq, ctr, maxE2, maxR2, nodes, bpts, [](uint32_t) {},
      [&](uint32_t s, Trav<K>& t) {
        t.nodes = nodes;
        t.pts = bpts;
        const float4 x = q[s];
        t.reset(x.x, x.y, x.z);
        return true;
      },
      [&](uint32_t s, Trav<K>& t) {
#pragma unroll
        for (int j = 0; j < K; ++j) {
          ids[(size_t)s * K + j] = t.best.id[j] < 0 ? -1 : __float_as_int(bpts[t.best.id[j]].w);
          d2[(size_t)s * K + j] = t.best.v[j];
        }
        tp += t.tp;
        tn += t.tn;
      });
  unsigned long long a = tp, b = tn;
#pragma unroll
  for (int o = 32; o > 0; o >>= 1) {
    a += __shfl_xor(a, o, 64);
    b += __shfl_xor(b, o, 64);
  }
  if ((threadIdx.x & 63) == 0) {
    atomicAdd(&touched[0], a);
    atomicAdd(&touched[1], b);
  }
}

template <class Eng>
__global__ __launch_bounds__(256) void k_knn1_generic(uint32_t nq, const float4* __restrict__ q,
                                                      const uint4* __restrict__ nodes,
                                                      const float4* __restrict__ bpts, float maxE2, float maxR2,
                                                      int32_t* __restrict__ ids, float* __restrict__ d2,
                                                      unsigned long long* touched, uint32_t* ctr) {
  uint32_t tp = 0, tn = 0;
  persistent_xcd<Eng>(
      nq, ctr, maxE2, maxR2, nodes, bpts, [](uint32_t) {},
      [&](uint32_t s, Eng& t) {
        t.bind(nodes, bpts, 0, 0);
        const float4 x = q[s];
        t.reset(x.x, x.y, x.z);
        return true;
      },
      [&](uint32_t s, Eng& t) {
        const int32_t id = t.res_id();
        ids[s] = id < 0 ? -1 : __float_as_int(bpts[id].w);
        d2[s] = t.res_d2();
        tp += t.tp;
        tn += t.tn;
      });
  unsigned long long a = tp, b = tn;
#pragma unroll
  for (int o = 32; o > 0; o >>= 1) {
    a += __shfl_xor(a, o, 64);
    b += __shfl_xor(b, o, 64);
  }
  if ((threadIdx.x & 63) == 0) {
    atomicAdd(&touched[0], a);
    atomicAdd(&touched[1], b);
// ... 63 lines not shown
void launch_init_state(hipStream_t s, int n_pairs, const PairDesc* pd, PairState* st) {
  k_init_state<<<(n_pairs + 63) / 64, 64, 0, s>>>(n_pairs, pd, st);
}
bool launch_normals(hipStream_t s, int n_pairs, uint32_t total_ref, const PairDesc* pd, PairState* st,
                    const uint4* nodes, const int32_t* parent, const float4* bpts, float4* bnrm, int knn,
                    int32_t* ids, uint32_t* ctr, int engine) {
  if (!total_ref) return true;
  if (!launch_knn_ids(s, n_pairs, total_ref, pd, nodes, bpts, knn, ids, ctr, nullptr, engine)) return false;
  const int gu = (int)((total_ref + 255) / 256);
  switch (knn) {
    case 10: k_normals_from_ids<10><<<gu, 256, 0, s>>>(n_pairs, total_ref, pd, st, bpts, ids, bnrm); break;
    case 20: k_normals_from_ids<20><<<gu, 256, 0, s>>>(n_pairs, total_ref, pd, st, bpts, ids, bnrm); break;
    case 30: k_normals_from_ids<30><<<gu, 256, 0, s>>>(n_pairs, total_ref, pd, st, bpts, ids, bnrm); break;
    default: return false;
  }
  return true;
}
constexpr uint32_t kKnnOctMax = 300000;
static bool knn_oct_enabled(uint32_t n_queries, int engine) {
  return engine == 0 ? n_queries <= kKnnOctMax : engine == 1;
}

bool launch_knn_ids(hipStream_t s, int n_pairs, uint32_t total_ref, const PairDesc* pd, const uint4* nodes,
                    const float4* bpts, int knn, int32_t* ids, uint32_t* ctr, unsigned long long* touched,
                    int engine) {
  if (!total_ref) return true;
  if (knn_oct_enabled(total_ref, engine)) {
    const unsigned go = (unsigned)(((uint64_t)total_ref * 8 + 255) / 256);
    switch (knn) {
      case 10: k_knn_oct<10, 8><<<go, 256, 0, s>>>(n_pairs, total_ref, pd, nodes, bpts, ids, touched); break;
      case 20: k_knn_oct<20, 8><<<go, 256, 0, s>>>(n_pairs, total_ref, pd, nodes, bpts, ids, touched); break;
      case 30: k_knn_oct<30, 8><<<go, 256, 0, s>>>(n_pairs, total_ref, pd, nodes, bpts, ids, touched); break;
      default: return false;
    }
    return true;
  }
  if (hipMemsetAsync(ctr, 0, kPersistCtrWords * 4, s) != hipSuccess) return false;
  const int g = persistent_grid((int)total_ref);
  switch (knn) {
    case 10: k_knn_ids<10><<<g, 256, 0, s>>>(n_pairs, total_ref, pd, nodes, nullptr, bpts, ids, ctr, touched); break;
    case 20: k_knn_ids<20><<<g, 256, 0, s>>>(n_pairs, total_ref, pd, nodes, nullptr, bpts, ids, ctr, touched); break;
    case 30: k_knn_ids<30><<<g, 256, 0, s>>>(n_pairs, total_ref, pd, nodes, nullptr, bpts, ids, ctr, touched); break;
    default: return false;
  }
  return true;
}
void launch_active_list(hipStream_t s, int n_pairs, const PairDesc* pd, const PairState* st, ActiveList* al,
                        uint32_t* ctr, uint32_t* host_n, uint64_t* done_sig, const uint64_t* ticket, float* outT,
                        int src_pair) {
  k_active_list<<<1, 256, 0, s>>>(n_pairs, pd, st, al, ctr, host_n, done_sig, ticket, outT, src_pair);
}
template <class E, class Tree>
static void nn_launch(hipStream_t s, int g, hipEvent_t e0, hipEvent_t e1, const PairDesc* pd, const PairState* st,
                      const ActiveList* al, const float4* read_c, const Tree* tree, const int32_t* parent,
                      const float4* bpts, const uint2* ptl, int32_t* match, float* d2, uint32_t* touched,
                      uint32_t* ctr, const IcpParams& prm) {
  if (e0)
    hipExtLaunchKernelGGL(k_icp_nn<E>, dim3(g), dim3(256), 0, s, e0, e1, 0, pd, st, al, read_c, tree, parent, bpts,
                          ptl, match, d2, touched, ctr, prm);
  else
    k_icp_nn<E><<<g, 256, 0, s>>>(pd, st, al, read_c, tree, parent, bpts, ptl, match, d2, touched, ctr, prm);
}

void launch_icp_nn(hipStream_t s, int grid_items, const PairDesc* pd, const PairState* st, const ActiveList* al,
                   const float4* read_c, const uint4* nodes, const uint4* tl, const int32_t* parent,
                   const float4* bpts, const uint2* ptl, int32_t* match, float* d2, uint32_t* touched,
                   uint32_t* ctr, const IcpParams& prm, hipEvent_t e0, hipEvent_t e1) {
  const int g = persistent_grid(grid_items, AICP_NN_WAVES);
  if (g == 0) {
    if (e0) (void)hipEventRecord(e0, s);
    if (e1) (void)hipEventRecord(e1, s);
    return;
  }
  if (tl && ptl)
    nn_launch<Trav2C>(s, g, e0, e1, pd, st, al, read_c, tl, parent, bpts, ptl, match, d2, touched, ctr, prm);
  else
    nn_launch<Trav<1>>(s, g, e0, e1, pd, st, al, read_c, nodes, parent, bpts, (const uint2*)nullptr, match, d2,
                       touched, ctr, prm);
}
void iter_prof_dump() {
#if AICP_ITER_PROF
  unsigned long long h[16];
  if (hipMemcpyFromSymbol(h, HIP_SYMBOL(g_iter_prof), sizeof(h)) == hipSuccess) {
    const char* nm[4] = {"hist_f", "compact_f", "reduce", "update_f(body=slab+solve, tail=active list)"};
    for (int k = 0; k < 4; ++k)
      fprintf(stderr, "[iter prof] %s: body %.2f us avg over %llu, tail %.2f us avg over %llu\n", nm[k],
              h[4 * k + 1] ? h[4 * k] / 100.0 / h[4 * k + 1] : 0.0, h[4 * k + 1],
              h[4 * k + 3] ? h[4 * k + 2] / 100.0 / h[4 * k + 3] : 0.0, h[4 * k + 3]);
  }
  unsigned long long z[16] = {};
  (void)hipMemcpyToSymbol(HIP_SYMBOL(g_iter_prof), z, sizeof(z));
#endif
}

void nn_prof_dump() {
#if AICP_XCD_PROF
  static unsigned long long h[64 * kXcdGroups * 2];
  if (hipMemcpyFromSymbol(h, HIP_SYMBOL(g_xcd_prof), sizeof(h)) == hipSuccess) {
    for (int l = 0; l < 64; ++l) {
      unsigned long long t0 = ~0ull, t1 = 0;
      for (int g = 0; g < kXcdGroups; ++g) {
        if (h[(l * kXcdGroups + g) * 2]) t0 = std::min(t0, h[(l * kXcdGroups + g) * 2]);
        t1 = std::max(t1, h[(l * kXcdGroups + g) * 2 + 1]);
      }
      if (t1 == 0) continue;
      unsigned long long c[kXcdGroups];
      (void)hipMemcpyFromSymbol(c, HIP_SYMBOL(g_xcd_cost), sizeof(c), sizeof(c) * l);
      fprintf(stderr, "xcd launch %2d: %6.1f us | per group: start end (us), queries, mean tn+tp:", l,
              (t1 - t0) / 100.0);
      for (int g = 0; g < kXcdGroups; ++g) {
        const unsigned long long q = c[g] >> 40, w = c[g] & ((1ull << 40) - 1);
        const unsigned long long s0 = h[(l * kXcdGroups + g) * 2];
        fprintf(stderr, " [%.1f %.1f %llu %.1f]", s0 ? (s0 - t0) / 100.0 : -1.0,
                (h[(l * kXcdGroups + g) * 2 + 1] - t0) / 100.0, q, q ? (double)w / q : 0.0);
      }
      fprintf(stderr, "\n");
    }
  }
  for (int i = 0; i < 64 * kXcdGroups; ++i) {
    h[2 * i] = ~0ull;
    h[2 * i + 1] = 0;
  }
  (void)hipMemcpyToSymbol(HIP_SYMBOL(g_xcd_prof), h, sizeof(h));
  static unsigned long long zc[64 * kXcdGroups] = {};
  (void)hipMemcpyToSymbol(HIP_SYMBOL(g_xcd_cost), zc, sizeof(zc));
#endif
#if AICP_NN_PROF
  unsigned long long h[8];
  if (hipMemcpyFromSymbol(h, HIP_SYMBOL(g_nn_prof), sizeof(h)) == hipSuccess) {
    const double tot = (double)(h[0] + h[1] + h[2] + h[3]);
    fprintf(stderr, "nn_prof: fill %.1f%% descent %.1f%% bucket %.1f%% climb %.1f%% | rounds %llu, mean active lanes %.1f | cached starts %llu, full %llu\n",
            100.0 * h[0] / tot, 100.0 * h[1] / tot, 100.0 * h[2] / tot, 100.0 * h[3] / tot, h[4],
            h[4] ? (double)h[5] / h[4] : 0.0, h[6], h[7]);
  }
  unsigned long long z[8] = {};
  (void)hipMemcpyToSymbol(HIP_SYMBOL(g_nn_prof), z, sizeof(z));
#endif
#if AICP_QLAT_PROF
  static unsigned long long q[512];
  if (hipMemcpyFromSymbol(q, HIP_SYMBOL(g_qlat), sizeof(q)) == hipSuccess) {
    const char* nm[2] = {"query latency", "completion after wave start"};
    for (int k = 0; k < 2; ++k) {
      const unsigned long long* h = q + 256 * k;
      unsigned long long n = 0, acc = 0;
      double mean = 0;
      for (int b = 0; b < 256; ++b) n += h[b], mean += (b + 0.5) * h[b];
      if (!n) continue;
      fprintf(stderr, "qlat %s: n %llu mean %.1f us |", nm[k], n, mean / n);
      const double ps[6] = {0.5, 0.9, 0.99, 0.999, 0.9999, 1.0};
      int p = 0;
      for (int b = 0; b < 256 && p < 6; ++b) {
        acc += h[b];
        while (p < 6 && acc >= (unsigned long long)(ps[p] * n)) {
          fprintf(stderr, " p%g %d", ps[p] * 100, b + 1);
          ++p;
        }
      }
      fprintf(stderr, " us\nqlat %s histogram (2 us bins):", nm[k]);
      for (int b = 0; b < 256; b += 2) {
        const unsigned long long c = h[b] + h[b + 1];
        if (c) fprintf(stderr, " %d:%llu", b, c);
      }
      fprintf(stderr, "\n");
    }
  }
  for (auto& v : q) v = 0;
  (void)hipMemcpyToSymbol(HIP_SYMBOL(g_qlat), q, sizeof(q));
#endif
}

void launch_icp_select(hipStream_t s, BlockMap m, int n_pairs, const PairDesc* pd, PairState* st, const float* d2,
                       uint32_t* hist1, uint32_t* cand, uint32_t* cand_cnt, int p0) {
  if (!m.n_blocks) return;
  k_sel_hist<<<m.n_blocks, 256, 0, s>>>(m, pd, st, d2, hist1);
  k_sel_find1<<<n_pairs, 1024, 0, s>>>(st + p0, hist1 + (size_t)p0 * kHistBins);
  k_sel_compact<<<m.n_blocks, 256, 0, s>>>(m, pd, st, d2, cand, cand_cnt);
  k_sel_final<<<n_pairs, 1024, 0, s>>>(pd + p0, st + p0, cand, cand_cnt + p0);
}
IcpIterSync icp_sync_layout(uint32_t* words, size_t n_pairs, int group) {
  IcpIterSync y{};
  y.sel1 = words;
  y.sel2 = words + n_pairs;
  y.red = words + 2 * n_pairs;
  y.pairs = words + 3 * n_pairs + group;
  return y;
}
void launch_icp_select_f(hipStream_t s, BlockMap m, const PairDesc* pd, PairState* st, const float* d2,
                         uint32_t* hist1, uint32_t* cand, uint32_t* cand_cnt, const IcpIterSync& y) {
  if (!m.n_blocks) return;
  k_sel_hist_f<kSelHistThreads><<<m.n_blocks, kSelHistThreads, 0, s>>>(m, pd, st, d2, hist1, y);
  k_sel_compact_f<kSelCompactThreads><<<m.n_blocks, kSelCompactThreads, 0, s>>>(m, pd, st, d2, cand, cand_cnt, y);
}
void launch_icp_select_fused(hipStream_t s, BlockMap m, const PairDesc* pd, PairState* st, const float* d2,
                             uint32_t* hist1, uint32_t* cand, uint32_t* cand_cnt, const IcpIterSync& y) {
  if (!m.n_blocks) return;
  if (m.n_blocks > 2048)
    k_sel_fused<256, kHistBins><<<m.n_blocks, 256, 0, s>>>(m, pd, st, d2, hist1, cand, cand_cnt, y);
  else
    k_sel_fused<256, kFinalLds><<<m.n_blocks, 256, 0, s>>>(m, pd, st, d2, hist1, cand, cand_cnt, y);
}
void launch_icp_select_pair(hipStream_t s, int n_pairs, const PairDesc* pd, PairState* st, const float* d2,
                            uint32_t* cand, const IcpIterSync& y) {
  if (n_pairs > 0) k_sel_pair<<<n_pairs, kSelPairThreads, 0, s>>>(pd, st, d2, cand, y);
}
bool sel_pair_fits(size_t n_pairs, uint64_t max_read, int force) {
  if (max_read > kSelPairMax) return false;
  if (force >= 0) return force == 1;
  return n_pairs >= 256;
}
void launch_icp_reduce_f(hipStream_t s, BlockMap m, const PairDesc* pd, PairState* st, const float4* read_c,
                         const int32_t* match, const float* d2, const uint32_t* touched, const float4* bpts,
                         const float4* bnrm, double* slab, const IcpParams& prm, const IcpIterSync& y) {
  if (!m.n_blocks) return;
  k_icp_reduce<<<m.n_blocks, kNNBlock, 0, s>>>(m, pd, st, read_c, match, d2, touched, bpts, bnrm, slab);
  k_icp_update_f<<<y.np, 256, 0, s>>>(y.pd, y.st, slab, prm, y);
}
void launch_icp_reduce(hipStream_t s, BlockMap m, const PairDesc* pd, const PairState* st, const float4* read_c,
                       const int32_t* match, const float* d2, const uint32_t* touched, const float4* bpts,
                       const float4* bnrm, double* slab) {
  if (m.n_blocks)
    k_icp_reduce<<<m.n_blocks, kNNBlock, 0, s>>>(m, pd, st, read_c, match, d2, touched, bpts, bnrm, slab);
}
void launch_icp_update(hipStream_t s, int n_pairs, const PairDesc* pd, PairState* st, const double* slab,
                       const IcpParams& prm) {
  k_icp_update<<<n_pairs, 256, 0, s>>>(pd, st, slab, prm);
}
void launch_finalize(hipStream_t s, int n_pairs, const PairDesc* pd, PairState* st, float* outT) {
  k_finalize<<<(n_pairs + 63) / 64, 64, 0, s>>>(n_pairs, pd, st, outT);
}
bool launch_knn_generic(hipStream_t s, uint32_t nq, const float4* q, const uint4* nodes, const int32_t* parent,
                        const float4* bpts, int k, float maxE2, float maxR2, int32_t* ids, float* d2,
                        unsigned long long* touched, uint32_t* ctr) {
  if (!nq) return true;
  const int g = persistent_grid((int)nq);
  switch (k) {
    case 1: k_knn1_generic<Trav<1>><<<g, 256, 0, s>>>(nq, q, nodes, bpts, maxE2, maxR2, ids, d2, touched, ctr); break;
    case 4: k_knn_generic<4><<<g, 256, 0, s>>>(nq, q, nodes, parent, bpts, maxE2, maxR2, ids, d2, touched, ctr); break;
    case 10: k_knn_generic<10><<<g, 256, 0, s>>>(nq, q, nodes, parent, bpts, maxE2, maxR2, ids, d2, touched, ctr); break;
    case 20: k_knn_generic<20><<<g, 256, 0, s>>>(nq, q, nodes, parent, bpts, maxE2, maxR2, ids, d2, touched, ctr); break;
    case 30: k_knn_generic<30><<<g, 256, 0, s>>>(nq, q, nodes, parent, bpts, maxE2, maxR2, ids, d2, touched, ctr); break;
    default: return false;
  }
  return true;
}
void launch_transform(hipStream_t s, int n, const float* T, const float4* in, float4* out) {
  if (n > 0) k_transform<<<(n + 255) / 256, 256, 0, s>>>(n, T, in, out);
}
void launch_solve6(hipStream_t s, const double* A, const double* b, double* x, int32_t* path) {
  k_solve6<<<1, 64, 0, s>>>(A, b, x, path);
}

}
```

### aicp_mapping_amd/csrc/runtime.hpp

```cpp
#pragma once
#include <hip/hip_runtime.h>

#include <algorithm>
#include <atomic>
#include <condition_variable>
#include <functional>
#include <mutex>
#include <string>
#include <thread>
#include <vector>

#include "../../include/aicp_hip.h"
#include "aicp_common.hpp"
#include "kernels.hpp"

namespace aicp {
namespace rt {

struct DevBuf {
  void* p = nullptr;
  size_t cap = 0;
  template <class T>
  T* as() const {
    return reinterpret_cast<T*>(p);
// ... 169 lines not shown
  bool ovl = false;
  double origin[3] = {0, 0, 0};
  double res = 0;
  OvlDesc od{};
  DevBuf gst;
  bool use = false;
  bool hit_trees = false, hit_ovl = false;
  uint64_t tree_hits = 0, tree_builds = 0, ovl_hits = 0, ovl_builds = 0;
  void invalidate() {
    trees = ovl = false;
    hit_trees = hit_ovl = use = false;
  }
};

struct ReadCache {
  const float* ptr = nullptr;
  uint64_t n = 0, stride = 0;
  std::vector<float> pts;
  bool valid = false;
  bool sorted = false;
  bool hit = false;
  uint64_t hits = 0;
};

struct SeqState;
void seq_state_free(SeqState* s);

}
}

struct aicp_hip_batch {
  size_t P = 0;
  std::vector<aicp::PairDesc> desc;
  std::vector<aicp::PairDesc> rdesc;
  std::vector<aicp::PairDesc> gdesc;
  uint64_t total_ref = 0, total_read = 0;
  uint32_t n_red_total = 0;
  aicp::rt::DevBuf ref_raw, read_raw, maps;
  aicp::BlockMap m_read{}, m_gref{}, m_red{}, m_sel{};
  bool refs_event = false;
};

struct aicp_hip_map {
  aicp::rt::DevBuf pts;
  size_t n = 0;
};

struct aicp_hip_ctx {
  int device = 0;
  hipStream_t stream = nullptr;
  hipStream_t stream2 = nullptr;
  hipStream_t stream3 = nullptr;
  std::string err;
  aicp::rt::DevBuf read_c, bpts, bnrm, nodes, match, d2, desc, state, touch, slab, bitmap, outT, scratch, active,
      ctrs, nbids, ref1, sel_hist, sel_cand, sel_cnt, qmap, ovl, rdesc, rstate, rdesc_raw, bpts_raw, nodes_raw,
      nrm_raw, inv, gdesc, gstate, read_s, ord_k0, ord_k1, ord_v0, ord_v1, ord_tmp, tl, ptl,
      tl_rank, pf_a, pf_b, pf_bpts, pf_nodes;
  uint64_t tl_total = 0;
  aicp::rt::TreeBufs tb[2];
  aicp::rt::PinBuf pin_desc, pin_state, pin_out, pin_io, pin_ovl, pin_rdesc, pin_gdesc, pin_gstate;
  aicp::rt::PinBuf pin_pf;
  std::vector<hipEvent_t> nn_ev;
  hipEvent_t ev[16] = {};
  int last_nn_launches = 0;
  double last_nn_ms = 0, last_nn_bytes = 0;
  uint64_t last_queries = 0;
  double last_phase[5] = {0, 0, 0, 0, 0};
  aicp_prefilter_stats last_pf{};
  aicp_hip_batch* oneshot = nullptr;
  hipEvent_t pf_ev[8] = {};
  aicp::rt::SeqState* seq = nullptr;
  aicp_hip_batch* mapbatch = nullptr;
  aicp::rt::DevBuf crop_ws;
  aicp::rt::DevBuf ovl_sp, ovl_keys;
  aicp::rt::DevBuf isync;
  aicp::rt::PinBuf pin_crop;
  aicp::rt::PinBuf pin_maps;
  aicp::rt::RefCache refc;
  aicp::rt::ReadCache rdc;
  aicp::rt::WorkerPool* pool = nullptr;
  uint32_t* poll_host = nullptr;
  uint32_t* poll_dev = nullptr;
  aicp_hip_options opt{};
};
constexpr int kBatchPolls = 64;

#define HIPC(x)                                                                   \
  do {                                                                            \
    const hipError_t e_ = (x);                                                    \
    if (e_ != hipSuccess) {                                                       \
      ctx->err = std::string(#x) + ": " + hipGetErrorString(e_);                  \
      return AICP_ERR_HIP;                                                        \
    }                                                                             \
  } while (0)

#define FAIL(code, msg)   \
  do {                    \
    ctx->err = (msg);     \
    return (code);        \
  } while (0)

#define TCHK(x)                                                                   \
  do {                                                                            \
    const hipError_t e_ = (x);                                                    \
    if (e_ != hipSuccess) {                                                       \
      err = std::string(#x) + ": " + hipGetErrorString(e_);                       \
      return AICP_ERR_HIP;                                                        \
    }                                                                             \
  } while (0)
#define TFAIL(code, msg) \
  do {                   \
    err = (msg);         \
    return (code);       \
  } while (0)
```

### aicp_mapping_amd/csrc/sequence.cpp

```cpp
#include <hip/hip_runtime.h>

#include <algorithm>
#include <atomic>
#include <chrono>
#include <cmath>
#include <condition_variable>
#include <cstdio>
#include <cstdlib>
#include <cstring>
#include <deque>
#include <functional>
#include <mutex>
#include <string>
#include <thread>
#include <type_traits>
#include <vector>

#include "../../include/aicp_hip.h"
#include "aicp_common.hpp"
#include "icp_math.hpp"
#include "kernels.hpp"
#include "runtime.hpp"

using namespace aicp;
using namespace aicp::rt;

namespace aicp {
namespace rt {

struct GraphCache {
  std::vector<uint64_t> key;
  hipGraphExec_t exec = nullptr;
  bool broken = false;
  void reset() {
    if (exec) (void)hipGraphExecDestroy(exec);
    exec = nullptr;
    key.clear();
  }
};


struct Key {
  std::vector<uint64_t> v;
  template <class T>
  Key& operator<<(const T& x) {
    static_assert(std::is_trivially_copyable<T>::value, "plain values");
    uint64_t w[(sizeof(T) + 7) / 8] = {};
    std::memcpy(w, &x, sizeof(T));
    v.insert(v.end(), w, w + (sizeof(T) + 7) / 8);
    return *this;
  }
};

constexpr int kSlots = 3;
constexpr int kMaxPolls = 64;


struct SeqSlot {
  DevBuf read_raw, read_s, read_c, match, d2, touch, cand, slab, ord_k0, ord_k1, ord_v0, ord_v1, ord_tmp, maps, bitmap,
      ovl, caps, sel_hist, sel_cnt, ctrs, active;
  DevBuf ref_src, ref_raw, bpts, bnrm, nodes, tl, ptl, tl_rank, bpts_raw, nodes_raw, nrm_raw, nbids,
      inv, rd, tsrc,
      wdesc, wstate, woutT, isync,
      sp_par, sp_cnt, sp_off, sp_keys_r, sp_keys_g, sp_tmp_r, sp_tmp_g, sp_pc;
  TreeBufs tb[2];
  PinBuf pin_read, pin_par, pin_src;
  hipEvent_t ev_up = nullptr, ev_rd = nullptr, ev_ref = nullptr, ev_s3 = nullptr, ev_s2 = nullptr, ev_done = nullptr;
  hipEvent_t ev_src = nullptr;
  uint32_t* poll_host = nullptr;
  uint32_t* poll_dev = nullptr;
  GraphCache g_match;
  bool used = false;
};

struct SeqState {
  hipStream_t s_up = nullptr, s_rd = nullptr, s_r2 = nullptr, s_r3 = nullptr, s_icp = nullptr;
  hipStream_t s_probe = nullptr;
  SeqSlot slot[kSlots];
  DevBuf desc, state, outT;
  DevBuf initT;
  PinBuf pin_state, pin_out, pin_ctl, pin_desc;
  std::vector<hipEvent_t> nn_ev;
  hipEvent_t ev_begin = nullptr, ev_end = nullptr;
  std::vector<hipEvent_t> tev;
  aicp_hip_options opt{};
  WorkerPool pool{std::max(1u, std::min(16u, std::thread::hardware_concurrency())) - 1};
  aicp_sequence_timing last{};
  int device = 0;
};

void seq_state_free(SeqState* S) {
  if (!S) return;
  for (hipStream_t q : {S->s_up, S->s_rd, S->s_r2, S->s_r3, S->s_icp})
    if (q) (void)hipStreamSynchronize(q);
  for (SeqSlot& sl : S->slot) {
    for (DevBuf* b : {&sl.read_raw, &sl.read_s, &sl.read_c, &sl.match, &sl.d2, &sl.touch, &sl.cand, &sl.slab,
                      &sl.ord_k0, &sl.ord_k1, &sl.ord_v0, &sl.ord_v1, &sl.ord_tmp, &sl.maps, &sl.bitmap, &sl.ovl,
                      &sl.caps, &sl.sel_hist, &sl.sel_cnt, &sl.ctrs, &sl.active, &sl.ref_src, &sl.ref_raw, &sl.bpts,
                      &sl.bnrm, &sl.nodes, &sl.tl, &sl.ptl, &sl.tl_rank, &sl.bpts_raw,
                      &sl.nodes_raw, &sl.nrm_raw, &sl.nbids, &sl.inv, &sl.rd, &sl.tsrc, &sl.wdesc, &sl.wstate,
                      &sl.woutT, &sl.isync, &sl.sp_par, &sl.sp_cnt, &sl.sp_off, &sl.sp_keys_r,
                      &sl.sp_keys_g, &sl.sp_tmp_r, &sl.sp_tmp_g, &sl.sp_pc})
      release(*b);
    for (auto& t : sl.tb) t.release_all();
    sl.g_match.reset();
    for (PinBuf* b : {&sl.pin_read, &sl.pin_par, &sl.pin_src}) release(*b);
    for (hipEvent_t e : {sl.ev_up, sl.ev_rd, sl.ev_ref, sl.ev_s3, sl.ev_s2, sl.ev_done, sl.ev_src})
      if (e) (void)hipEventDestroy(e);
    if (sl.poll_host) (void)hipHostFree(sl.poll_host);
  }
  for (DevBuf* b : {&S->desc, &S->state, &S->outT, &S->initT}) release(*b);
  for (PinBuf* b : {&S->pin_state, &S->pin_out, &S->pin_ctl, &S->pin_desc}) release(*b);
  for (hipEvent_t e : S->nn_ev) (void)hipEventDestroy(e);
  for (hipEvent_t e : S->tev) (void)hipEventDestroy(e);
  for (hipEvent_t e : {S->ev_begin, S->ev_end})
    if (e) (void)hipEventDestroy(e);
  for (hipStream_t q : {S->s_rd, S->s_icp, S->s_probe})
    if (q) (void)hipStreamDestroy(q);
  delete S;
}

}
}

namespace {

struct Box {
  float lo[3], hi[3];
  void reset() {
    for (int k = 0; k < 3; ++k) {
      lo[k] = INFINITY;
      hi[k] = -INFINITY;
    }
  }
  void add(float x, float y, float z) {
    const float v[3] = {x, y, z};
    for (int k = 0; k < 3; ++k) {
      lo[k] = std::min(lo[k], v[k]);
      hi[k] = std::max(hi[k], v[k]);
    }
  }
  void merge(const Box& b) {
    for (int k = 0; k < 3; ++k) {
      lo[k] = std::min(lo[k], b.lo[k]);
      hi[k] = std::max(hi[k], b.hi[k]);
    }
  }
};

void pack_clouds(WorkerPool& pool, const std::vector<PackSeg>& segs, std::vector<Box>& boxes) {
  constexpr uint64_t kChunk = 1 << 15;
  struct Task {
    size_t seg;
    uint64_t a, b;
  };
  std::vector<Task> tasks;
  for (size_t s = 0; s < segs.size(); ++s)
    for (uint64_t a = 0; a < segs[s].n; a += kChunk) tasks.push_back({s, a, std::min(segs[s].n, a + kChunk)});
  std::vector<Box> part(tasks.size());
  pool.run(tasks.size(), [&](size_t t) {
    const Task& k = tasks[t];
    const PackSeg& g = segs[k.seg];
    Box bx;
    bx.reset();
    const char* src = reinterpret_cast<const char*>(g.src);
    for (uint64_t i = k.a; i < k.b; ++i) {
      const float* p = reinterpret_cast<const float*>(src + i * g.stride);
      float* d = g.dst4 + 4 * i;
// ... 699 lines not shown
  ip.min_rot = cfg->min_diff_rot;
  ip.min_trans = cfg->min_diff_trans;
  ip.knn_normals = cfg->knn_normals;
  return ip;
}

static bool loop_polled(const SeqState* S, const aicp_icp_config* cfg, int k) {
  return !S->opt.no_early_exit && k >= cfg->smooth_length && k < kMaxPolls && k < cfg->max_iter;
}
static bool loop_written(const SeqState* S, int k) { return !S->opt.no_early_exit && k < kMaxPolls; }

struct LoopPairs {
  int np_l;
  PairDesc* gd;
  PairState* gs;
  uint64_t reads;
};

static int loop_part(aicp_hip_ctx* ctx, SeqState* S, const aicp_icp_config* cfg, const aicp_sequence_params* prm,
                     IcpLoop& q, int part, bool timeNN, int& nn_launches) {
  WinRun& R = *q.R;
  WIN_REFS;
  const int it = q.it;
  ActiveList* al = sl.active.as<ActiveList>();
  uint32_t* ctr = sl.ctrs.as<uint32_t>();
  const int r = q.sub;
  const LoopPairs lp{r >= 0 ? 1 : (int)np, r >= 0 ? dDesc + r : dDesc, r >= 0 ? dState + r : dState,
                     r >= 0 ? R.n_read[r] : R.nread};
  uint32_t* poll_host = sl.poll_host + q.area * kMaxPolls;
  uint32_t* poll_dev = sl.poll_dev + q.area * kMaxPolls;
  IcpParams ip = icp_params(cfg);
  ip.prof_slot = nn_launches;
  hipStream_t st = S->s_icp;
  if (part == 0) {
    uint32_t* hn_this = nullptr;
    if (it == 0 && loop_written(S, it)) {
      poll_host[it] = 0xffffffffu;
      hn_this = poll_dev + it;
    }
    if (timeNN)
      while ((int)S->nn_ev.size() < 2 * (nn_launches + 1)) {
        hipEvent_t e;
        HIPC(hipEventCreateWithFlags(&e, hipEventDisableSystemFence));
        S->nn_ev.push_back(e);
      }
    if (it == 0) launch_active_list(st, lp.np_l, lp.gd, lp.gs, al, ctr, hn_this, nullptr, nullptr, nullptr, R.next_src);
    launch_icp_nn(st, (int)lp.reads, lp.gd, lp.gs, al, sl.read_c.as<float4>(), sl.nodes.as<uint4>(),
                  R.use_tl ? sl.tl.as<uint4>() : nullptr, nullptr, sl.bpts.as<float4>(),
                  R.use_tl ? sl.ptl.as<uint2>() : nullptr, sl.match.as<int32_t>(), sl.d2.as<float>(),
                  sl.touch.as<uint32_t>(), ctr, ip, timeNN ? S->nn_ev[2 * nn_launches] : nullptr,
                  timeNN ? S->nn_ev[2 * nn_launches + 1] : nullptr);
    HIPC(hipGetLastError());
    ++nn_launches;
    q.nn = it + 1;
    return AICP_OK;
  }
  const BlockMap msel = r >= 0 ? map_sub(R.m_sel, R.b_sel[r], R.b_sel[r + 1] - R.b_sel[r]) : R.m_sel;
  const BlockMap mred = r >= 0 ? map_sub(R.m_red, R.b_red[r], R.b_red[r + 1] - R.b_red[r]) : R.m_red;
  uint32_t* hn_next = nullptr;
  if (loop_written(S, it + 1)) {
    poll_host[it + 1] = 0xffffffffu;
    hn_next = poll_dev + it + 1;
  }
  IcpIterSync y = icp_sync_layout(sl.isync.as<uint32_t>(), np, 0);
  y.np = lp.np_l;
  y.pd = lp.gd;
  y.st = lp.gs;
  y.al = al;
  y.ctr = ctr;
  y.host_n = hn_next;
  y.src_pair = R.next_src;
  const int ff = S->opt.select_fused_from;
  if (ff > 0 && it >= ff)
    launch_icp_select_fused(st, msel, dDesc, dState, sl.d2.as<float>(), sl.sel_hist.as<uint32_t>(),
                            sl.cand.as<uint32_t>(), sl.sel_cnt.as<uint32_t>(), y);
  else
    launch_icp_select_f(st, msel, dDesc, dState, sl.d2.as<float>(), sl.sel_hist.as<uint32_t>(), sl.cand.as<uint32_t>(),
                        sl.sel_cnt.as<uint32_t>(), y);
  if (it == 0) {
    HIPC(hipStreamWaitEvent(st, sl.ev_s2, 0));
    launch_pairs_degenerate_part(st, lp.np_l, lp.gd, lp.gs, dRst, 1);
  }
  launch_icp_reduce_f(st, mred, dDesc, dState, sl.read_c.as<float4>(), sl.match.as<int32_t>(), sl.d2.as<float>(),
                      sl.touch.as<uint32_t>(), sl.bpts.as<float4>(), sl.bnrm.as<float4>(), sl.slab.as<double>(), ip, y);
  HIPC(hipGetLastError());
  ++q.it;
  if (q.it >= cfg->max_iter) q.stop = true;
  return AICP_OK;
}

static int loop_finish(aicp_hip_ctx* ctx, SeqState* S, const aicp_sequence_params* prm, IcpLoop& q) {
  WinRun& R = *q.R;
  WIN_REFS;
  hipStream_t st = S->s_icp;
  if (!R.debug) launch_finalize(st, (int)np, dDesc, dState, dOutT);
  if (R.tev) HIPC(hipEventRecord(R.tev[4], st));
  launch_seq_commit(st, (int)np, dDesc, dState, dOutT, S->desc.as<PairDesc>() + w.p0, S->state.as<PairState>() + w.p0,
                    S->outT.as<float>() + 16 * w.p0);
  HIPC(hipGetLastError());
  if (R.tev) HIPC(hipEventRecord(R.tev[5], st));
  HIPC(hipEventRecord(sl.ev_done, st));
  return AICP_OK;
}

static int loop_poll(aicp_hip_ctx* ctx, SeqState* S, IcpLoop& q, bool& got) {
  got = false;
  SeqSlot& sl = S->slot[q.R->w.slot];
  volatile uint32_t* w = sl.poll_host + q.area * kMaxPolls;
  if (w[q.it] == 0xffffffffu) {
    int m = q.it - 1;
    while (m >= 0 && w[m] == 0xffffffffu) --m;
    if (m >= 0 && w[m] == 0u) {
      got = true;
      q.stop = true;
      return AICP_OK;
    }
    const auto now = std::chrono::steady_clock::now();
    if (q.wait_it != q.it) {
      q.wait_it = q.it;
      q.wait_t0 = now;
      return AICP_OK;
    }
    if (now - q.wait_t0 < std::chrono::milliseconds(20)) return AICP_OK;
    const hipError_t r = hipStreamQuery(S->s_icp);
    if (r == hipErrorNotReady) return AICP_OK;
    HIPC(r);
    std::atomic_thread_fence(std::memory_order_seq_cst);
    if (w[q.it] == 0xffffffffu) {
      got = true;
      q.stop = true;
      return AICP_OK;
    }
  }
  got = true;
  const uint32_t v = w[q.it];
  if (v == 0) {
    q.stop = true;
  } else if (q.R->next_src >= 0 && !q.src_done && !(v >> 31)) {
    HIPC(hipEventRecord(sl.ev_src, S->s_icp));
    q.src_done = true;
  }
  return AICP_OK;
}

static int sub_prep(aicp_hip_ctx* ctx, SeqState* S, const aicp_sequence_params* prm, IcpLoop& q) {
  WinRun& R = *q.R;
  WIN_REFS;
  const int r = q.sub;
  hipStream_t si = S->s_icp;
  float* initT = S->initT.as<float>();
  float4* pts = sl.read_raw.as<float4>() + R.loff[r];
  launch_debug_prep(si, dDesc + r, initT, initT + 16 * (1 + w.p0 + (size_t)r));
  launch_transform(si, (int)R.n_read[r], initT, pts, pts);
  const BlockMap mrd = map_sub(R.m_read, R.b_read[r], R.b_read[r + 1] - R.b_read[r]);
  if (doOvl) {
    launch_ovl_init(si, 1, dDesc + r, dState + r, res, 2);
    if (R.sparse) {
      HIPC(launch_ovl_keys(si, R.kr1[r], dDesc[r].read_origin, sl.read_raw.as<float4>(), res, dState + r, 1));
      HIPC(launch_ovl_keys_intersect(si, R.kr1[r], R.kg, R.per_pair + r, dState + r));
    } else {
      launch_ovl_bbox(si, mrd, dDesc, dState, sl.read_raw.as<float4>(), 1, res);
      launch_ovl_size(si, 1, dState + r, dOvl + 1 + r, dCap + 1 + r);
      launch_ovl_clear(si, 1, dOvl + 1 + r, bmp, R.cap[1 + r]);
      launch_ovl_mark(si, mrd, dDesc, dOvl + 1, dState, sl.read_raw.as<float4>(), 1, res, bmp, false);
      launch_ovl_popcount(si, 1, dOvl + 1 + r, dState + r, 1, bmp);
      launch_ovl_intersect(si, 1, dDesc + r, dOvl + 1 + r, dOvl, dState + r, bmp);
    }
    launch_ovl_finish(si, 1, dDesc + r, dState + r, dGst, 1);
  }
  launch_prepare_read(si, mrd, dDesc, sl.read_raw.as<float4>(), sl.read_c.as<float4>());
  HIPC(hipGetLastError());
  return AICP_OK;
}

static int sub_post(aicp_hip_ctx* ctx, SeqState* S, const aicp_sequence_params* prm, IcpLoop& q) {
  WinRun& R = *q.R;
  WIN_REFS;
  const int r = q.sub;
  launch_debug_post(S->s_icp, dDesc + r, dState + r, dOutT + 16 * r, S->initT.as<float>(), prm->max_correction_magnitude);
  HIPC(hipGetLastError());
  return AICP_OK;
}

static int seq_init(aicp_hip_ctx* ctx, size_t n) {
  if (!ctx->seq) {
    SeqState* S = new SeqState();
    ctx->seq = S;
    S->device = ctx->device;
    int lo = 0, hi = 0;
    if (hipDeviceGetStreamPriorityRange(&lo, &hi) != hipSuccess) lo = hi = 0;
    HIPC(hipStreamCreateWithPriority(&S->s_rd, hipStreamNonBlocking, lo));
    HIPC(hipStreamCreateWithPriority(&S->s_icp, hipStreamNonBlocking, hi));
    S->s_up = S->s_rd;
    S->s_r2 = ctx->stream2;
    S->s_r3 = ctx->stream3;
    for (SeqSlot& sl : S->slot) {
      HIPC(hipEventCreateWithFlags(&sl.ev_up, hipEventDisableTiming));
      for (hipEvent_t* e : {&sl.ev_rd, &sl.ev_ref, &sl.ev_s3, &sl.ev_s2, &sl.ev_done, &sl.ev_src})
        HIPC(hipEventCreateWithFlags(e, hipEventDisableTiming | hipEventReleaseToDevice));
      HIPC(hipHostMalloc((void**)&sl.poll_host, 2 * kMaxPolls * 4, hipHostMallocMapped));
      HIPC(hipHostGetDevicePointer((void**)&sl.poll_dev, sl.poll_host, 0));
    }
    HIPC(hipEventCreate(&S->ev_begin));
    HIPC(hipEventCreate(&S->ev_end));
    (void)hipGetLastError();
  }
  SeqState* S = ctx->seq;
  S->opt = ctx->opt;
  for (SeqSlot& sl : S->slot) {
    sl.used = false;
    for (auto& t : sl.tb) tree_opts(t, S->opt);
  }
  HIPC(ensure(S->desc, n * sizeof(PairDesc)));
  HIPC(ensure(S->state, n * sizeof(PairState)));
  HIPC(ensure(S->outT, n * 64));
  HIPC(ensure(S->pin_state, n * sizeof(PairState)));
  HIPC(ensure(S->pin_out, n * 64));
  return AICP_OK;
}

static int seq_sync(aicp_hip_ctx* ctx, SeqState* S) {
  for (hipStream_t q : {S->s_up, S->s_rd, S->s_r2, S->s_r3, S->s_icp}) HIPC(hipStreamSynchronize(q));
  return AICP_OK;
}

extern "C" {

void aicp_hip_default_sequence_params(aicp_sequence_params* p) {
  if (!p) return;
  *p = aicp_sequence_params{};
  p->reference_update_frequency = 5;
  p->max_correction_magnitude = 1.0f;
  p->resolution = (double)0.2f;
  p->flags = AICP_RUN_OVERLAP;
}

int aicp_hip_sequence_run(aicp_hip_ctx* ctx, const aicp_icp_config* cfg, const aicp_sequence_params* prm,
                          const aicp_cloud* first, const aicp_cloud* readings, size_t n, float* out_T,
                          aicp_sequence_result* out, size_t* n_done) {
  if (!ctx || !cfg || !prm || !first || (n && (!readings || !out_T || !out)) || !n_done) return AICP_ERR_INVALID;
  const auto t0 = std::chrono::steady_clock::now();
  *n_done = 0;
  const int F = prm->reference_update_frequency;
  if (F < 1) FAIL(AICP_ERR_INVALID, "reference_update_frequency must be >= 1");
  const bool doOvl = prm->flags & AICP_RUN_OVERLAP;
  const bool debug = prm->flags & AICP_SEQ_DEBUG;
  if (doOvl && !(prm->resolution > 0)) FAIL(AICP_ERR_INVALID, "resolution");
  int rc = check_cfg(ctx, cfg, AICP_RUN_ICP | (doOvl ? AICP_RUN_OVERLAP : 0));
  if (rc) return rc;
  auto valid = [](const aicp_cloud& c) {
    return c.pts && c.n >= 1 && c.n < (1ull << 28) && c.stride >= 12 && c.stride % 4 == 0;
  };
  if (!valid(*first)) FAIL(AICP_ERR_INVALID, "invalid first cloud");
  for (size_t i = 0; i < n; ++i)
    if (!valid(readings[i])) FAIL(AICP_ERR_INVALID, "invalid reading " + std::to_string(i));
  if ((size_t)F > (size_t)kMaxPairs) FAIL(AICP_ERR_UNSUPPORTED, "reference_update_frequency above 4096");
  {
    uint64_t run = 0;
    for (size_t i = 0; i < n; ++i) {
      run += readings[i].n;
      if (i >= (size_t)F) run -= readings[i - F].n;
      if (run >= (1ull << 31)) FAIL(AICP_ERR_UNSUPPORTED, "a window's readings exceed 2^31 points");
    }
  }
  if (n == 0) return AICP_OK;
  HIPC(hipSetDevice(ctx->device));
  rc = seq_init(ctx, n);
  if (rc) return rc;
  SeqState* S = ctx->seq;
  S->last = aicp_sequence_timing{};
  if (debug) {
    HIPC(ensure(S->initT, 64 * (n + 1)));
    HIPC(ensure(S->pin_desc, n * sizeof(PairDesc)));
  }
  const bool timeNN = prm->flags & AICP_RUN_TIME_NN;
  int nn_launches = 0, windows = 0, replans = 0;
  HIPC(hipEventRecord(S->ev_begin, S->s_up));
  size_t p = 0;
  int src = -1, acc = 0;
  std::vector<uint8_t> accepted(n, 0);
  std::vector<Box> rbox(n);
  int status = AICP_OK;
  while (p < n) {
    std::vector<Win> plan;
    {
      size_t q = p;
      int s = src, a = acc, k = 0;
      while (q < n) {
        const size_t np = std::min<size_t>((size_t)(F - a), n - q);
        plan.push_back(Win{q, np, s, k % kSlots, k});
        q += np;
// ... 346 lines not shown
```

### include/aicp_hip.h

```cpp
#ifndef AICP_HIP_H_
#define AICP_HIP_H_

#include <stddef.h>
#include <stdint.h>

#ifdef __cplusplus
extern "C" {
#endif

#define AICP_OK 0
#define AICP_ERR_CONVERGENCE 1
#define AICP_ERR_INVALID 2
#define AICP_ERR_HIP 3
#define AICP_ERR_UNSUPPORTED 4
#define AICP_ERR_TRANSFORMATION 5

typedef struct aicp_hip_ctx aicp_hip_ctx;
typedef struct aicp_hip_batch aicp_hip_batch;

typedef struct {
  int32_t knn_normals;
  float nn_epsilon;
  float nn_max_dist;
  float trimmed_ratio;
  int32_t max_iter;
  float min_diff_rot;
  float min_diff_trans;
  int32_t smooth_length;
  int32_t bucket_size;
  int32_t knn_match;
} aicp_icp_config;

typedef struct {
  int32_t status;
  int32_t iterations;
  int32_t converged;
  int32_t degenerate_normals;
  float inlier_ratio;
  float trimmed_ratio;
  float overlap_percent;
  int32_t tree_depth;
  uint64_t nn_points_touched;
  uint64_t nn_nodes_touched;
  uint64_t overlap_keys[3];
} aicp_icp_stats;

typedef struct {
  const float* ref;
  uint64_t n_ref;
  uint64_t ref_stride;
  const float* read;
  uint64_t n_read;
  uint64_t read_stride;
  const float* init_T;
  double ref_origin[3];
  double read_origin[3];
} aicp_pair;

typedef struct {
  const float* pts;
  uint64_t n;
  uint64_t stride;
  double origin[3];
} aicp_cloud;

#define AICP_RUN_OVERLAP 1
#define AICP_RUN_ICP 2
#define AICP_RUN_TIME_NN 4

int aicp_hip_create(int device, aicp_hip_ctx** out);
void aicp_hip_destroy(aicp_hip_ctx* ctx);
const char* aicp_hip_last_error(const aicp_hip_ctx* ctx);
const char* aicp_hip_version(void);
const char* aicp_hip_build_info(void);

typedef struct {
  int32_t profile;
  int32_t nn_engine;
  int32_t overlap_path;
  int32_t normals_knn_engine;
  int32_t select_pair;
  int32_t select_fused_from;
  int32_t raw_tree_first;
  int32_t raw_first_at;
  int32_t no_early_exit;
  int32_t tree_plan;
  uint32_t tree_lvl_min;
  int32_t reference_cache;
  uint32_t oneshot_keep_mib;
  int32_t early_reference;
  uint64_t read_order_min;
} aicp_hip_options;
void aicp_hip_default_options(aicp_hip_options* out);
int aicp_hip_set_options(aicp_hip_ctx* ctx, const aicp_hip_options* opt);
int aicp_hip_get_options(const aicp_hip_ctx* ctx, aicp_hip_options* out);
int aicp_hip_test_force_scan_stall(int on);

void aicp_hip_default_config(aicp_icp_config* out);
int aicp_hip_parse_pm_yaml(const char* path, aicp_icp_config* out);
int aicp_hip_replace_ratio_config_file(const char* in_path, const char* out_path, float ratio);
float aicp_hip_autotune_ratio(float overlap_percent);

int aicp_hip_register(aicp_hip_ctx* ctx, const aicp_icp_config* cfg, const aicp_pair* pair,
                      float out_T[16], aicp_icp_stats* stats );
int aicp_hip_register_batch(aicp_hip_ctx* ctx, const aicp_icp_config* cfg,
                            const aicp_pair* pairs, size_t n_pairs,
                            float* out_T , aicp_icp_stats* stats );
int aicp_hip_overlap(aicp_hip_ctx* ctx, const aicp_pair* pair, double resolution,
                     float* out_overlap_percent);
int aicp_hip_overlap_batch(aicp_hip_ctx* ctx, const aicp_pair* pairs, size_t n_pairs,
                           double resolution, float* out_overlap_percent ,
                           aicp_icp_stats* stats );
int aicp_hip_reference_cache_stats(const aicp_hip_ctx* ctx, uint64_t out[4]);
int aicp_hip_align_batch(aicp_hip_ctx* ctx, const aicp_icp_config* cfg,
                         const aicp_pair* pairs, size_t n_pairs, double resolution, int flags,
                         float* out_T , aicp_icp_stats* stats );
typedef struct aicp_hip_multi aicp_hip_multi;
int aicp_hip_multi_create(const int* devices, int n_devices, aicp_hip_multi** out);
void aicp_hip_multi_destroy(aicp_hip_multi* m);
int aicp_hip_multi_size(const aicp_hip_multi* m);
aicp_hip_ctx* aicp_hip_multi_context(aicp_hip_multi* m, int i);
const char* aicp_hip_multi_last_error(const aicp_hip_multi* m);
int aicp_hip_multi_align_batch(aicp_hip_multi* m, const aicp_icp_config* cfg, const aicp_pair* pairs,
                               size_t n_pairs, double resolution, int flags, float* out_T ,
                               aicp_icp_stats* stats , int* out_device );

int aicp_hip_transform(aicp_hip_ctx* ctx, const float T[16], const float* in, size_t n,
                       size_t stride, float* out );

int aicp_hip_crop_box(aicp_hip_ctx* ctx, const float* pts, size_t n, size_t stride, float min,
                      float max, const float origin[16], float* out , size_t* out_n,
                      float* rpy_out );

typedef struct {
  float leaf_size;
  int32_t normal_k;
  int32_t neighbours;
  int32_t min_cluster_size;
  int32_t max_cluster_size;
  float smoothness_rad;
  float curvature_threshold;
  float viewpoint[3];
} aicp_prefilter_params;
void aicp_hip_default_prefilter(aicp_prefilter_params* out);
int aicp_hip_prefilter(aicp_hip_ctx* ctx, const aicp_prefilter_params* prm, const float* pts, size_t n,
                       size_t stride, float* out , size_t* out_n, float* sampled ,
                       int32_t* labels , size_t* n_sampled ,
                       size_t* n_clusters );

typedef struct {
  double voxel_ms;
  double normals_ms;
  double segment_ms;
  double device_ms;
  double wall_ms;
  double knn_ms;
  uint64_t knn_queries;
  uint64_t knn_points_touched, knn_nodes_touched;
  int32_t propagation_passes;
  int32_t pad;
} aicp_prefilter_stats;
int aicp_hip_last_prefilter_stats(const aicp_hip_ctx* ctx, aicp_prefilter_stats* out);

typedef struct aicp_hip_map aicp_hip_map;
int aicp_hip_map_create(aicp_hip_ctx* ctx, const float* pts, size_t n, size_t stride, aicp_hip_map** out);
void aicp_hip_map_free(aicp_hip_ctx* ctx, aicp_hip_map* map);
int aicp_hip_map_size(const aicp_hip_map* map, size_t* n);
int aicp_hip_map_download(aicp_hip_ctx* ctx, const aicp_hip_map* map, float* out, size_t cap, size_t* out_n);
int aicp_hip_map_crop(aicp_hip_ctx* ctx, const aicp_hip_map* map, float min, float max, const float origin[16],
                      float* out , size_t cap, size_t* out_n);
int aicp_hip_map_register_batch(aicp_hip_ctx* ctx, const aicp_icp_config* cfg, const aicp_hip_map* map, float min,
                                float max, const aicp_cloud* readings, const float* poses , size_t n,
                                int flags, float* out_T , aicp_icp_stats* stats );
int aicp_hip_map_merge(aicp_hip_ctx* ctx, aicp_hip_map* map, const float* pts, size_t n, size_t stride,
                       const float T[16]);
int aicp_hip_map_prefilter(aicp_hip_ctx* ctx, aicp_hip_map* map, const aicp_prefilter_params* prm);

int aicp_hip_batch_upload(aicp_hip_ctx* ctx, const aicp_pair* pairs, size_t n_pairs,
                          aicp_hip_batch** out);
int aicp_hip_batch_run(aicp_hip_ctx* ctx, aicp_hip_batch* batch, const aicp_icp_config* cfg,
                       double resolution, int flags, float* out_T ,
                       aicp_icp_stats* stats );
void aicp_hip_batch_free(aicp_hip_ctx* ctx, aicp_hip_batch* batch);
int aicp_hip_last_nn_timing(const aicp_hip_ctx* ctx, int* n_launches, double* total_ms,
                            double* algorithmic_bytes, uint64_t* queries);
int aicp_hip_last_phase_ms(const aicp_hip_ctx* ctx, double out_ms[5]);


#define AICP_SEQ_DEBUG 8

typedef struct {
  int32_t reference_update_frequency;
  float max_correction_magnitude;
  double resolution;
  int32_t flags;
} aicp_sequence_params;

typedef struct {
  int32_t status;
  int32_t accepted;
  int32_t reference;
  int32_t is_reference;
  double corrected_origin[3];
  aicp_icp_stats icp;
} aicp_sequence_result;

typedef struct {
  int32_t windows;
  int32_t replans;
  double wall_ms;
  double device_ms;
} aicp_sequence_timing;

void aicp_hip_default_sequence_params(aicp_sequence_params* out);
int aicp_hip_sequence_run(aicp_hip_ctx* ctx, const aicp_icp_config* cfg, const aicp_sequence_params* prm,
                          const aicp_cloud* first, const aicp_cloud* readings, size_t n_readings,
                          float* out_T , aicp_sequence_result* out , size_t* n_done);
int aicp_hip_last_sequence_timing(const aicp_hip_ctx* ctx, aicp_sequence_timing* out);

int aicp_hip_sequence_run_raw(aicp_hip_ctx* ctx, const aicp_icp_config* cfg, const aicp_sequence_params* prm,
                              const aicp_prefilter_params* pf, const aicp_cloud* first, const aicp_cloud* readings,
                              size_t n_readings, float* out_T , aicp_sequence_result* out ,
                              size_t* n_done);

int aicp_hip_knn(aicp_hip_ctx* ctx, const float* pts, size_t n, size_t stride,
                 const float* queries, size_t nq, size_t qstride, int k, float epsilon,
                 float max_dist, int32_t* out_ids , float* out_d2 ,
                 uint64_t* out_touched );
int aicp_hip_normals(aicp_hip_ctx* ctx, const float* pts, size_t n, size_t stride, int knn,
                     float* out_normals , int32_t* out_degenerate );
int aicp_hip_dists_quantile(aicp_hip_ctx* ctx, const float* d2, size_t n, float quantile,
                            float* out_limit);
int aicp_hip_solve6(aicp_hip_ctx* ctx, const double* A, const double* b, double* out_x,
                    int32_t* out_path );

#ifdef __cplusplus
}
#endif

#endif
```

Measured before the change: 2903.

## Add optional fused reduce+update kernel and LDS-staged multi-wave ICP update

Adds a k_icp_reduce_u kernel where the last-arriving reduce block of each pair runs the pose update itself, removing the separate update launch. This path sits behind an update_in_reduce flag that defaults to 0. The default k_icp_update_f now calls a new icp_update_body_lds, which stages the pair state in shared memory and splits the QR rank check and Cholesky solve across waves before a serial update. The change also adds a memory-backed solve6 variant, templated quaternion branches and extra profiling counters. The LDS update raises shared-memory use and adds block-level syncs in exchange for less serial work on one thread.

```diff
diff --git a/aicp_mapping_amd/_lib.py b/aicp_mapping_amd/_lib.py
--- a/aicp_mapping_amd/_lib.py
+++ b/aicp_mapping_amd/_lib.py
@@ -28,7 +28,8 @@
     "aicp_hip_overlap", "aicp_hip_overlap_batch", "aicp_hip_align_batch", "aicp_hip_transform", "aicp_hip_crop_box",
     "aicp_hip_batch_upload", "aicp_hip_batch_run", "aicp_hip_batch_free",
     "aicp_hip_last_nn_timing", "aicp_hip_last_phase_ms", "aicp_hip_knn", "aicp_hip_normals",
-    "aicp_hip_dists_quantile", "aicp_hip_solve6", "aicp_hip_default_prefilter", "aicp_hip_prefilter",
+    "aicp_hip_dists_quantile", "aicp_hip_solve6", "aicp_hip_solve6_mem", "aicp_hip_set_update_in_reduce",
+    "aicp_hip_get_update_in_reduce", "aicp_hip_default_prefilter", "aicp_hip_prefilter",
     "aicp_hip_last_prefilter_stats", "aicp_hip_map_create", "aicp_hip_map_free", "aicp_hip_map_size",
     "aicp_hip_map_download", "aicp_hip_map_crop", "aicp_hip_map_merge", "aicp_hip_map_prefilter",
     "aicp_hip_default_sequence_params", "aicp_hip_sequence_run", "aicp_hip_last_sequence_timing",
@@ -41,7 +42,8 @@
 
 _NEWEST = {"aicp_hip_reference_cache_stats", "aicp_hip_default_options", "aicp_hip_set_options",
            "aicp_hip_get_options", "aicp_hip_test_force_scan_stall",
-           "aicp_hip_sequence_run_raw", "aicp_hip_build_info"}
+           "aicp_hip_sequence_run_raw", "aicp_hip_build_info", "aicp_hip_solve6_mem",
+           "aicp_hip_set_update_in_reduce", "aicp_hip_get_update_in_reduce"}
 
 
 class IcpConfig(C.Structure):
@@ -239,6 +241,11 @@
     L.aicp_hip_normals.argtypes = [vp, fp, sz, sz, C.c_int, fp, ip]
     L.aicp_hip_dists_quantile.argtypes = [vp, fp, sz, C.c_float, fp]
     L.aicp_hip_solve6.argtypes = [vp, dp, dp, dp, ip]
+    if hasattr(L, "aicp_hip_set_update_in_reduce"):
+        L.aicp_hip_set_update_in_reduce.argtypes = [vp, C.c_int]
+        L.aicp_hip_get_update_in_reduce.argtypes = [vp]
+    if hasattr(L, "aicp_hip_solve6_mem"):
+        L.aicp_hip_solve6_mem.argtypes = [vp, dp, dp, dp, ip]
     L.aicp_hip_default_prefilter.argtypes = [C.POINTER(PrefilterParams)]
     L.aicp_hip_default_prefilter.restype = None
     L.aicp_hip_prefilter.argtypes = [vp, C.POINTER(PrefilterParams), fp, sz, sz, fp, C.POINTER(C.c_size_t), fp, ip,
@@ -463,6 +470,8 @@
         return o
 
     def set_options(self, opt: Options = None, **kw) -> Options:
+        if "update_in_reduce" in kw:
+            self.check(lib.aicp_hip_set_update_in_reduce(self.h, int(kw.pop("update_in_reduce"))))
         old = self.get_options()
         new = Options.from_buffer_copy(opt if opt is not None else old)
         for k, v in kw.items():
@@ -477,11 +486,14 @@
 
         class _Scope:
             def __enter__(self):
+                self.uir = lib.aicp_hip_get_update_in_reduce(ctx.h) if "update_in_reduce" in kw else None
                 self.old = ctx.set_options(**kw)
                 return ctx
 
             def __exit__(self, *exc):
                 ctx.set_options(self.old)
+                if self.uir is not None:
+                    ctx.set_options(update_in_reduce=self.uir)
                 return False
 
         return _Scope()
@@ -609,14 +621,14 @@
         self.check(rc)
         return out.value
 
-    def solve6(self, A, b):
+    def solve6(self, A, b, mem=False):
         A = np.ascontiguousarray(A, np.float64).reshape(36)
         b = np.ascontiguousarray(b, np.float64).reshape(6)
         x = np.zeros(6, np.float64)
         path = C.c_int32()
         dp = C.POINTER(C.c_double)
-        rc = lib.aicp_hip_solve6(self.h, A.ctypes.data_as(dp), b.ctypes.data_as(dp), x.ctypes.data_as(dp),
-                                 C.byref(path))
+        fn = lib.aicp_hip_solve6_mem if mem else lib.aicp_hip_solve6
+        rc = fn(self.h, A.ctypes.data_as(dp), b.ctypes.data_as(dp), x.ctypes.data_as(dp), C.byref(path))
         self.check(rc)
         return x, path.value
 
diff --git a/aicp_mapping_amd/csrc/aicp_hip.cpp b/aicp_mapping_amd/csrc/aicp_hip.cpp
--- a/aicp_mapping_amd/csrc/aicp_hip.cpp
+++ b/aicp_mapping_amd/csrc/aicp_hip.cpp
@@ -901,7 +901,8 @@
         launch_icp_select_f(s, B->m_sel, dDesc, dState, ctx->d2.as<float>(), ctx->sel_hist.as<uint32_t>(),
                             ctx->sel_cand.as<uint32_t>(), ctx->sel_cnt.as<uint32_t>(), y);
       launch_icp_reduce_f(s, B->m_red, dDesc, dState, readc, ctx->match.as<int32_t>(), ctx->d2.as<float>(),
-                          ctx->touch.as<uint32_t>(), bpts, bnrm, ctx->slab.as<double>(), prm, y);
+                          ctx->touch.as<uint32_t>(), bpts, bnrm, ctx->slab.as<double>(), prm, y,
+                          ctx->update_in_reduce);
     }
     launch_finalize(s, (int)P, dDesc, dState, ctx->outT.as<float>());
     if (ctx->opt.profile) {
@@ -1056,6 +1057,15 @@
   *out = ctx->opt;
   return AICP_OK;
 }
+
+int aicp_hip_set_update_in_reduce(aicp_hip_ctx* ctx, int on) {
+  if (!ctx) return AICP_ERR_INVALID;
+  if (on < 0 || on > 1) FAIL(AICP_ERR_INVALID, "aicp_hip_set_update_in_reduce: value out of range");
+  ctx->update_in_reduce = on;
+  return AICP_OK;
+}
+
+int aicp_hip_get_update_in_reduce(const aicp_hip_ctx* ctx) { return ctx ? ctx->update_in_reduce : 0; }
 
 int aicp_hip_test_force_scan_stall(int on) { return set_lb_force_stall(on) == hipSuccess ? AICP_OK : AICP_ERR_HIP; }
 
@@ -1554,14 +1564,16 @@
   return AICP_OK;
 }
 
-int aicp_hip_solve6(aicp_hip_ctx* ctx, const double* A, const double* b, double* out_x, int32_t* out_path) {
+static int solve6_on_device(aicp_hip_ctx* ctx, const double* A, const double* b, double* out_x, int32_t* out_path,
+                            bool mem) {
   if (!ctx || !A || !b || !out_x) return AICP_ERR_INVALID;
   HIPC(hipSetDevice(ctx->device));
   HIPC(ensure(ctx->scratch, 8 * (36 + 6 + 6) + 8));
   char* d = ctx->scratch.as<char>();
   HIPC(hipMemcpy(d, A, 36 * 8, hipMemcpyHostToDevice));
   HIPC(hipMemcpy(d + 288, b, 6 * 8, hipMemcpyHostToDevice));
-  launch_solve6(ctx->stream, (const double*)d, (const double*)(d + 288), (double*)(d + 336), (int32_t*)(d + 384));
+  (mem ? launch_solve6_mem : launch_solve6)(ctx->stream, (const double*)d, (const double*)(d + 288),
+                                            (double*)(d + 336), (int32_t*)(d + 384));
   HIPC(hipGetLastError());
   HIPC(hipStreamSynchronize(ctx->stream));
   HIPC(hipMemcpy(out_x, d + 336, 48, hipMemcpyDeviceToHost));
@@ -1569,6 +1581,14 @@
   HIPC(hipMemcpy(&path, d + 384, 4, hipMemcpyDeviceToHost));
   if (out_path) *out_path = path;
   return AICP_OK;
+}
+
+int aicp_hip_solve6(aicp_hip_ctx* ctx, const double* A, const double* b, double* out_x, int32_t* out_path) {
+  return solve6_on_device(ctx, A, b, out_x, out_path, false);
+}
+
+int aicp_hip_solve6_mem(aicp_hip_ctx* ctx, const double* A, const double* b, double* out_x, int32_t* out_path) {
+  return solve6_on_device(ctx, A, b, out_x, out_path, true);
 }
 
 void aicp_hip_default_prefilter(aicp_prefilter_params* p) {
diff --git a/aicp_mapping_amd/csrc/icp_math.hpp b/aicp_mapping_amd/csrc/icp_math.hpp
--- a/aicp_mapping_amd/csrc/icp_math.hpp
+++ b/aicp_mapping_amd/csrc/icp_math.hpp
@@ -90,6 +90,17 @@
       for (int cc = 0; cc < 3; ++cc) T[cc * 4 + r] = (r == cc) ? 1.f : 0.f;
 }
 
+template <int I>
+AICP_HD void quat_branch(const double (&m)[3][3], double* q) {
+  constexpr int J = (I + 1) % 3, K = (J + 1) % 3;
+  double t = sqrt(m[I][I] - m[J][J] - m[K][K] + 1.0);
+  q[1 + I] = 0.5 * t;
+  t = 0.5 / t;
+  q[0] = (m[K][J] - m[J][K]) * t;
+  q[1 + J] = (m[J][I] + m[I][J]) * t;
+  q[1 + K] = (m[K][I] + m[I][K]) * t;
+}
+
 AICP_HD void quat_from_T(const float* T, double* q) {
   double m[3][3];
   for (int r = 0; r < 3; ++r)
@@ -105,18 +116,10 @@
   } else {
     int i = 0;
     if (m[1][1] > m[0][0]) i = 1;
-    if (m[2][2] > m[i][i]) i = 2;
-    const int j = (i + 1) % 3, k = (j + 1) % 3;
-    t = sqrt(m[i][i] - m[j][j] - m[k][k] + 1.0);
-    double v[3];
-    v[i] = 0.5 * t;
-    t = 0.5 / t;
-    q[0] = (m[k][j] - m[j][k]) * t;
-    v[j] = (m[j][i] + m[i][j]) * t;
-    v[k] = (m[k][i] + m[i][k]) * t;
-    q[1] = v[0];
-    q[2] = v[1];
-    q[3] = v[2];
+    if (m[2][2] > (i == 1 ? m[1][1] : m[0][0])) i = 2;
+    if (i == 0) quat_branch<0>(m, q);
+    else if (i == 1) quat_branch<1>(m, q);
+    else quat_branch<2>(m, q);
   }
 }
 
@@ -419,6 +422,252 @@
   return 2;
 }
 
+#define AICP_ROLLED _Pragma("nounroll")
+
+struct Solve6Work {
+  double a[36], tau[6];
+  double Q[36], AP[36], R1[36], RRt[36], L[36];
+  double ja[36], V[36], w[6];
+  double qb[6], y[6], z[6];
+  int rowT[6], colT[6], perm[6];
+  int nonzero, rank;
+  double A[36], b[6], x[6];
+};
+
+AICP_HD void pivqr6_mem(const double* A, Solve6Work& W) {
+  constexpr int N = 6;
+  AICP_ROLLED for (int i = 0; i < N * N; ++i) W.a[i] = A[i];
+  const double prec = (double)kFltEps * N;
+  W.nonzero = N;
+  double maxpivot = 0, biggest = 0;
+  bool stop = false;
+  AICP_ROLLED for (int k = 0; k < N; ++k) {
+    if (stop) {
+      W.rowT[k] = k;
+      W.colT[k] = k;
+      W.tau[k] = 0;
+      continue;
+    }
+    int br = k, bc = k;
+    double bv = -1;
+    AICP_ROLLED for (int c = k; c < N; ++c)
+      AICP_ROLLED for (int r = k; r < N; ++r) {
+        const double v = fabs(W.a[r * N + c]);
+        if (v > bv) {
+          bv = v;
+          br = r;
+          bc = c;
+        }
+      }
+    if (k == 0) biggest = bv;
+    if (bv <= biggest * prec) {
+      W.nonzero = k;
+      W.rowT[k] = k;
+      W.colT[k] = k;
+      W.tau[k] = 0;
+      stop = true;
+      continue;
+    }
+    W.rowT[k] = br;
+    W.colT[k] = bc;
+    if (br != k)
+      AICP_ROLLED for (int c = k; c < N; ++c) {
+        const double t = W.a[k * N + c];
+        W.a[k * N + c] = W.a[br * N + c];
+        W.a[br * N + c] = t;
+      }
+    if (bc != k)
+      AICP_ROLLED for (int r = 0; r < N; ++r) {
+        const double t = W.a[r * N + k];
+        W.a[r * N + k] = W.a[r * N + bc];
+        W.a[r * N + bc] = t;
+      }
+    double tailSq = 0;
+    AICP_ROLLED for (int r = k + 1; r < N; ++r) tailSq += W.a[r * N + k] * W.a[r * N + k];
+    const double c0 = W.a[k * N + k];
+    double beta, tau;
+    if (tailSq <= kDblMin) {
+      tau = 0;
+      beta = c0;
+      AICP_ROLLED for (int r = k + 1; r < N; ++r) W.a[r * N + k] = 0;
+    } else {
+      beta = sqrt(c0 * c0 + tailSq);
+      if (c0 >= 0) beta = -beta;
+      const double den = c0 - beta;
+      AICP_ROLLED for (int r = k + 1; r < N; ++r) W.a[r * N + k] /= den;
+      tau = (beta - c0) / beta;
+    }
+    W.tau[k] = tau;
+    W.a[k * N + k] = beta;
+    if (fabs(beta) > maxpivot) maxpivot = fabs(beta);
+    AICP_ROLLED for (int c = k + 1; c < N; ++c) {
+      double s = W.a[k * N + c];
+      AICP_ROLLED for (int r = k + 1; r < N; ++r) s += W.a[r * N + k] * W.a[r * N + c];
+      s *= tau;
+      W.a[k * N + c] -= s;
+      AICP_ROLLED for (int r = k + 1; r < N; ++r) W.a[r * N + c] -= s * W.a[r * N + k];
+    }
+  }
+  const double thr = fabs(maxpivot) * ((double)kFltEps * N);
+  W.rank = 0;
+  AICP_ROLLED for (int i = 0; i < W.nonzero; ++i) W.rank += (fabs(W.a[i * N + i]) > thr) ? 1 : 0;
+}
+
+AICP_HD bool llt_solve6_mem(const double* M, int r, const double* b, double* x, double* L, double* y) {
+  constexpr int N = 6;
+  bool ok = true;
+  AICP_ROLLED for (int j = 0; j < r; ++j) {
+    double d = M[j * N + j];
+    AICP_ROLLED for (int k = 0; k < j; ++k) d -= L[j * N + k] * L[j * N + k];
+    if (!(d > 0)) ok = false;
+    const double ljj = sqrt(d);
+    L[j * N + j] = ljj;
+    AICP_ROLLED for (int i = j + 1; i < r; ++i) {
+      double s = M[i * N + j];
+      AICP_ROLLED for (int k = 0; k < j; ++k) s -= L[i * N + k] * L[j * N + k];
+      L[i * N + j] = s / ljj;
+    }
+  }
+  if (!ok) return false;
+  AICP_ROLLED for (int i = 0; i < r; ++i) {
+    double s = b[i];
+    AICP_ROLLED for (int k = 0; k < i; ++k) s -= L[i * N + k] * y[k];
+    y[i] = s / L[i * N + i];
+  }
+  AICP_ROLLED for (int i = r - 1; i >= 0; --i) {
+    double s = y[i];
+    AICP_ROLLED for (int k = i + 1; k < r; ++k) s -= L[k * N + i] * x[k];
+    x[i] = s / L[i * N + i];
+  }
+  return true;
+}
+
+AICP_HD int solve6_mem(const double* A, const double* b, double* x, Solve6Work& W) {
+  constexpr int n = 6;
+  pivqr6_mem(A, W);
+  if (W.rank == n) {
+    if (llt_solve6_mem(A, n, b, x, W.L, W.y)) return 0;
+  } else if (W.rank > 0) {
+    const int r = W.rank;
+    AICP_ROLLED for (int i = 0; i < n * n; ++i) W.Q[i] = 0;
+    AICP_ROLLED for (int i = 0; i < n; ++i) W.Q[i * n + i] = 1;
+    AICP_ROLLED for (int k = n - 1; k >= 0; --k) {
+      const double tau = (k < W.nonzero) ? W.tau[k] : 0.0;
+      if (tau != 0) {
+        AICP_ROLLED for (int c = k; c < n; ++c) {
+          double s = W.Q[k * n + c];
+          AICP_ROLLED for (int rr = k + 1; rr < n; ++rr) s += W.a[rr * n + k] * W.Q[rr * n + c];
+          s *= tau;
+          W.Q[k * n + c] -= s;
+          AICP_ROLLED for (int rr = k + 1; rr < n; ++rr) W.Q[rr * n + c] -= s * W.a[rr * n + k];
+        }
+      }
+      const int rr = (k < W.nonzero) ? W.rowT[k] : k;
+      if (rr != k)
+        AICP_ROLLED for (int c = 0; c < n; ++c) {
+          const double t = W.Q[k * n + c];
+          W.Q[k * n + c] = W.Q[rr * n + c];
+          W.Q[rr * n + c] = t;
+        }
+    }
+    AICP_ROLLED for (int i = 0; i < n; ++i) W.perm[i] = i;
+    AICP_ROLLED for (int k = 0; k < n; ++k) {
+      const int c = (k < W.nonzero) ? W.colT[k] : k;
+      if (c > k) {
+        const int t = W.perm[k];
+        W.perm[k] = W.perm[c];
+        W.perm[c] = t;
+      }
+    }
+    AICP_ROLLED for (int j = 0; j < n; ++j)
+      AICP_ROLLED for (int k = 0; k < n; ++k) W.AP[k * n + j] = A[k * n + W.perm[j]];
+    AICP_ROLLED for (int i = 0; i < r; ++i)
+      AICP_ROLLED for (int j = 0; j < n; ++j) {
+        double s = 0;
+        AICP_ROLLED for (int k = 0; k < n; ++k) s += W.Q[k * n + i] * W.AP[k * n + j];
+        W.R1[i * n + j] = s;
+      }
+    AICP_ROLLED for (int i = 0; i < r; ++i)
+      AICP_ROLLED for (int j = 0; j < r; ++j) {
+        double s = 0;
+        AICP_ROLLED for (int k = 0; k < n; ++k) s += W.R1[i * n + k] * W.R1[j * n + k];
+        W.RRt[i * n + j] = s;
+      }
+    AICP_ROLLED for (int i = 0; i < r; ++i) {
+      double s = 0;
+      AICP_ROLLED for (int k = 0; k < n; ++k) s += W.Q[k * n + i] * b[k];
+      W.qb[i] = s;
+    }
+    if (llt_solve6_mem(W.RRt, r, W.qb, W.y, W.L, W.z)) {
+      AICP_ROLLED for (int j = 0; j < n; ++j) {
+        double s = 0;
+        AICP_ROLLED for (int i = 0; i < r && i <= j; ++i) s += W.R1[i * n + j] * W.y[i];
+        W.z[j] = s;
+      }
+      AICP_ROLLED for (int i = 0; i < n; ++i) x[W.perm[i]] = W.z[i];
+      double nb = 0, nax = 0, nd = 0;
+      AICP_ROLLED for (int i = 0; i < n; ++i) {
+        double s = 0;
+        AICP_ROLLED for (int k = 0; k < n; ++k) s += A[i * n + k] * x[k];
+        nb += b[i] * b[i];
+        nax += s * s;
+        nd += (b[i] - s) * (b[i] - s);
+      }
+      if (nd <= 1e-10 * (nb < nax ? nb : nax)) return 1;
+    }
+  }
+  AICP_ROLLED for (int i = 0; i < n * n; ++i) W.ja[i] = A[i];
+  AICP_ROLLED for (int i = 0; i < n * n; ++i) W.V[i] = 0;
+  AICP_ROLLED for (int i = 0; i < n; ++i) W.V[i * n + i] = 1;
+  AICP_ROLLED for (int sweep = 0; sweep < 64; ++sweep) {
+    double offn = 0, diag = 0;
+    AICP_ROLLED for (int p = 0; p < n; ++p) {
+      diag += W.ja[p * n + p] * W.ja[p * n + p];
+      AICP_ROLLED for (int q = p + 1; q < n; ++q) offn += W.ja[p * n + q] * W.ja[p * n + q];
+    }
+    if (offn <= 1e-30 * diag || offn == 0) break;
+    AICP_ROLLED for (int p = 0; p < n; ++p)
+      AICP_ROLLED for (int q = p + 1; q < n; ++q) {
+        const double apq = W.ja[p * n + q];
+        if (apq != 0) {
+          const double app = W.ja[p * n + p], aqq = W.ja[q * n + q];
+          const double theta = (aqq - app) / (2 * apq);
+          const double t = (theta >= 0 ? 1.0 : -1.0) / (fabs(theta) + sqrt(theta * theta + 1));
+          const double c = 1 / sqrt(t * t + 1), s = t * c;
+          AICP_ROLLED for (int k = 0; k < n; ++k) {
+            const double akp = W.ja[k * n + p], akq = W.ja[k * n + q];
+            W.ja[k * n + p] = c * akp - s * akq;
+            W.ja[k * n + q] = s * akp + c * akq;
+          }
+          AICP_ROLLED for (int k = 0; k < n; ++k) {
+            const double apk = W.ja[p * n + k], aqk = W.ja[q * n + k];
+            W.ja[p * n + k] = c * apk - s * aqk;
+            W.ja[q * n + k] = s * apk + c * aqk;
+          }
+          AICP_ROLLED for (int k = 0; k < n; ++k) {
+            const double vkp = W.V[k * n + p], vkq = W.V[k * n + q];
+            W.V[k * n + p] = c * vkp - s * vkq;
+            W.V[k * n + q] = s * vkp + c * vkq;
+          }
+        }
+      }
+  }
+  AICP_ROLLED for (int i = 0; i < n; ++i) W.w[i] = W.ja[i * n + i];
+  double wmax = 0;
+  AICP_ROLLED for (int i = 0; i < n; ++i) wmax = fmax(wmax, fabs(W.w[i]));
+  double thr = wmax * (n * kDblEps);
+  if (thr < kDblMin) thr = kDblMin;
+  AICP_ROLLED for (int i = 0; i < n; ++i) x[i] = 0;
+  AICP_ROLLED for (int e = 0; e < n; ++e) {
+    if (fabs(W.w[e]) <= thr) continue;
+    double s = 0;
+    AICP_ROLLED for (int k = 0; k < n; ++k) s += W.V[k * n + e] * b[k];
+    s /= W.w[e];
+    AICP_ROLLED for (int k = 0; k < n; ++k) x[k] += W.V[k * n + e] * s;
+  }
+  return 2;
+}
+
 AICP_HD bool normal_from_cov(const double* C, float* nrm) {
   PivQR<3> qr;
   pivqr<3>(C, qr);
diff --git a/aicp_mapping_amd/csrc/kernels.hpp b/aicp_mapping_amd/csrc/kernels.hpp
--- a/aicp_mapping_amd/csrc/kernels.hpp
+++ b/aicp_mapping_amd/csrc/kernels.hpp
@@ -59,7 +59,8 @@
                              uint32_t* hist1, uint32_t* cand, uint32_t* cand_cnt, const IcpIterSync& y);
 void launch_icp_reduce_f(hipStream_t s, BlockMap m, const PairDesc* pd, PairState* st, const float4* read_c,
                          const int32_t* match, const float* d2, const uint32_t* touched, const float4* bpts,
-                         const float4* bnrm, double* slab, const IcpParams& prm, const IcpIterSync& y);
+                         const float4* bnrm, double* slab, const IcpParams& prm, const IcpIterSync& y,
+                         int update_in_reduce);
 void launch_icp_nn(hipStream_t s, int grid_items, const PairDesc* pd, const PairState* st,
                    const ActiveList* al, const float4* read_c, const uint4* nodes, const uint4* tl,
                    const int32_t* parent, const float4* bpts, const uint2* ptl, int32_t* match, float* d2,
@@ -93,6 +94,7 @@
 void launch_crop_scatter_multi(hipStream_t s, int n, int n_crops, const void* args, const float4* pts,
                                const uint32_t* tile_off, const uint32_t* base_of, float4* out);
 void launch_solve6(hipStream_t s, const double* A, const double* b, double* x, int32_t* path);
+void launch_solve6_mem(hipStream_t s, const double* A, const double* b, double* x, int32_t* path);
 
 struct TreeWork {
   float4* W[2];
diff --git a/aicp_mapping_amd/csrc/kernels_icp.hip b/aicp_mapping_amd/csrc/kernels_icp.hip
--- a/aicp_mapping_amd/csrc/kernels_icp.hip
+++ b/aicp_mapping_amd/csrc/kernels_icp.hip
@@ -683,7 +683,25 @@
       atomicAdd(&g_iter_prof[4 * (k) + 3], 1ull);                                                \
     }                                                                                            \
   } while (0)
+constexpr int kUpPhases = 5;
+__device__ unsigned long long g_up_prof[4 * kUpPhases];
+#define AICP_UP_T0 uint64_t up_t = __builtin_amdgcn_s_memrealtime()
+#define AICP_UP(k)                                                         \
+  do {                                                                     \
+    if (threadIdx.x == 0) {                                                \
+      const uint64_t now_ = __builtin_amdgcn_s_memrealtime();              \
+      atomicAdd(&g_up_prof[2 * (k)], (unsigned long long)(now_ - up_t));   \
+      atomicAdd(&g_up_prof[2 * (k) + 1], 1ull);                            \
+      up_t = now_;                                                         \
+    }                                                                      \
+  } while (0)
 #else
+#define AICP_UP_T0 \
+  do {             \
+  } while (0)
+#define AICP_UP(k) \
+  do {             \
+  } while (0)
 #define AICP_IP_T0 \
   do {             \
   } while (0)
@@ -893,12 +911,14 @@
   __shared__ uint32_t r_off[1024];
   const int t = threadIdx.x, lane = t & 63, wave = t >> 6, nt = (int)blockDim.x, nw = nt >> 6;
   uint16_t* chunk = al_chunks(al);
-  if (t == 0) carry_off = carry_cnt = 0;
+  __shared__ uint32_t src_on;
+  if (t == 0) carry_off = carry_cnt = src_on = 0;
   if (t < kXcdGroups * kGroupCtrs) ctr[t * kCtrStride] = 0;
   __syncthreads();
   for (int base = 0; base < n_pairs; base += nt) {
     const int p = base + t;
     const bool a = p < n_pairs && st[p].active;
+    if (a && p == src_pair) src_on = 1u;
     const uint32_t v = a ? (pd[p].n_read + 63u) & ~63u : 0u;
     uint32_t x = v, c = a ? 1u : 0u;
 #pragma unroll
@@ -948,7 +968,6 @@
     al->n = carry_cnt;
     al->total = carry_off;
     al->off[carry_cnt] = carry_off;
-    const bool src_on = src_pair >= 0 && src_pair < n_pairs && st[src_pair].active;
     if (host_n)
       __hip_atomic_store(host_n, carry_cnt | (src_on ? 0x80000000u : 0u), __ATOMIC_RELAXED, __HIP_MEMORY_SCOPE_SYSTEM);
   }
@@ -2306,8 +2325,9 @@
   for (int a = 0; a < 6; ++a) b[a] = -tot[21 + a];
 }
 
+template <bool kMem = false>
 __device__ void update_serial(const PairDesc& d, PairState& s, const double* tot, const IcpParams& prm,
-                              const double* x_full) {
+                              const double* x_full, Solve6Work* ws = nullptr) {
   s.touched_pts += (uint64_t)tot[28];
   s.touched_nodes += (uint64_t)tot[29];
   const int32_t kept = (int32_t)tot[27];
@@ -2320,6 +2340,10 @@
   double xd[6];
   if (x_full) {
     for (int a = 0; a < 6; ++a) xd[a] = x_full[a];
+  } else if constexpr (kMem) {
+    normal_system(tot, ws->A, ws->b);
+    solve6_mem(ws->A, ws->b, ws->x, *ws);
+    for (int a = 0; a < 6; ++a) xd[a] = ws->x[a];
   } else {
     double A[36], b[6];
     normal_system(tot, A, b);
@@ -2381,6 +2405,7 @@
   __shared__ double part[kGroups][kRedCols];
   __shared__ double tot[kRedCols];
   const int t = threadIdx.x;
+  AICP_UP_T0;
   if (t < kGroups * kRedCols) {
     const int g = t / kRedCols, c = t - g * kRedCols;
     const double* col = slab + (size_t)d.red_blk_off * kRedCols + c;
@@ -2406,6 +2431,7 @@
     tot[t] = v;
   }
   __syncthreads();
+  AICP_UP(kUpPhases + 0);
   __shared__ int rank_llt[2];
   __shared__ double xs[6];
   auto tri = [&](int r, int c) {
@@ -2426,7 +2452,9 @@
     if (t == 0) rank_llt[0] = rk;
   }
   __syncthreads();
+  AICP_UP(kUpPhases + 1);
   if (t == 0) update_serial(d, s, tot, prm, rank_llt[0] == 6 && rank_llt[1] ? xs : nullptr);
+  AICP_UP(kUpPhases + 2);
 }
 
 __global__ __launch_bounds__(256) void k_icp_update(const PairDesc* __restrict__ pd, PairState* st,
@@ -2437,17 +2465,156 @@
   icp_update_body(pd[pair], s, slab, prm);
 }
 
+#ifndef AICP_UPD_SPECULATE
+#define AICP_UPD_SPECULATE 1
+#endif
+struct UpdLds {
+  PairState s;
+  Solve6Work w;
+};
+__device__ void icp_update_body_lds(const PairDesc& d, PairState& s, const double* slab, const IcpParams& prm,
+                                    UpdLds& u) {
+  static_assert(kNNBlock == 256, "the update's thread layout");
+  constexpr int kGroups = 256 / kRedCols;
+  __shared__ double part[kGroups][kRedCols];
+  __shared__ double tot[kRedCols];
+  const int t = threadIdx.x;
+  AICP_UP_T0;
+  {
+    static_assert(sizeof(PairState) % 4 == 0, "PairState is copied in words");
+    const uint32_t* src = reinterpret_cast<const uint32_t*>(&s);
+    uint32_t* dst = reinterpret_cast<uint32_t*>(&u.s);
+    for (int i = t; i < (int)(sizeof(PairState) / 4); i += kNNBlock) dst[i] = src[i];
+  }
+  if (t < kGroups * kRedCols) {
+    const int g = t / kRedCols, c = t - g * kRedCols;
+    const double* col = slab + (size_t)d.red_blk_off * kRedCols + c;
+    double v = 0.0;
+    for (uint32_t r0 = g; r0 < d.n_red_blk; r0 += 16u * kGroups) {
+      double x[16];
+#pragma unroll
+      for (int k = 0; k < 16; ++k) {
+        const uint32_t r = r0 + (uint32_t)k * kGroups;
+        x[k] = r < d.n_red_blk ? col[(size_t)r * kRedCols] : 0.0;
+      }
+#pragma unroll
+      for (int k = 0; k < 16; ++k)
+        if (r0 + (uint32_t)k * kGroups < d.n_red_blk) v += x[k];
+    }
+    part[g][c] = v;
+  }
+  __syncthreads();
+  const int h = u.s.hist_count % kHistRing;
+  if (t < kRedCols) {
+    double v = part[0][t];
+#pragma unroll
+    for (int g = 1; g < kGroups; ++g) v += part[g][t];
+    tot[t] = v;
+  }
+  __syncthreads();
+  AICP_UP(0);
+  __shared__ int rank_llt[2];
+  __shared__ double xs[6];
+  auto tri = [&](int r, int c) {
+    const int a = r < c ? r : c, bb = r < c ? c : r;
+    return tot[a * 6 - a * (a - 1) / 2 + (bb - a)];
+  };
+  if (t >= 64 && t < 128) {
+    double b[6], x[6];
+    for (int a = 0; a < 6; ++a) b[a] = -tot[21 + a];
+    const bool ok = wave_llt_solve6(tri, b, x);
+    if (t == 64) {
+      rank_llt[1] = ok ? 1 : 0;
+      for (int a = 0; a < 6; ++a) xs[a] = x[a];
+#if AICP_UPD_SPECULATE
+      if (ok) update_serial<true>(d, u.s, tot, prm, xs, &u.w);
+#endif
+    }
+  }
+  if (t < 64) {
+    const int rk = wave_pivqr_rank6(tri);
+    if (t == 0) rank_llt[0] = rk;
+  }
+  __syncthreads();
+  AICP_UP(1);
+  const bool full = rank_llt[0] == 6 && rank_llt[1];
+#if AICP_UPD_SPECULATE
+  if (!full) {
+    if (rank_llt[1]) {
+      const uint32_t* src = reinterpret_cast<const uint32_t*>(&s);
+      uint32_t* dst = reinterpret_cast<uint32_t*>(&u.s);
+      for (int i = t; i < (int)(sizeof(PairState) / 4); i += kNNBlock) dst[i] = src[i];
+      __syncthreads();
+    }
+    if (t == 0) update_serial<true>(d, u.s, tot, prm, nullptr, &u.w);
+  }
+#else
+  if (t == 0) update_serial<true>(d, u.s, tot, prm, full ? xs : nullptr, &u.w);
+#endif
+  __syncthreads();
+  AICP_UP(2);
+  if (t < 16) s.T[t] = u.s.T[t];
+  if (t >= 16 && t < 20) s.qh[h][t - 16] = u.s.qh[h][t - 16];
+  if (t >= 20 && t < 23) s.th[h][t - 20] = u.s.th[h][t - 20];
+  if (t == 23) s.dq[h] = u.s.dq[h];
+  if (t == 24) s.dt[h] = u.s.dt[h];
+  if (t == 25) s.touched_pts = u.s.touched_pts;
+  if (t == 26) s.touched_nodes = u.s.touched_nodes;
+  if (t == 27) s.kept = u.s.kept;
+  if (t == 28) s.status = u.s.status;
+  if (t == 29) s.active = u.s.active;
+  if (t == 30) s.iters = u.s.iters;
+  if (t == 31) s.converged = u.s.converged;
+  if (t == 32) s.hist_count = u.s.hist_count;
+  if (t == 33) s.inlier_ratio = u.s.inlier_ratio;
+  AICP_UP(3);
+}
+
 __global__ __launch_bounds__(256) void k_icp_update_f(const PairDesc* __restrict__ pd, PairState* st,
                                                       const double* __restrict__ slab, IcpParams prm, IcpIterSync y) {
   AICP_IP_T0;
   const int pair = blockIdx.x;
   PairState& s = st[pair];
   if (!s.active) return;
-  icp_update_body(pd[pair], s, slab, prm);
+  __shared__ UpdLds u;
+  icp_update_body_lds(pd[pair], s, slab, prm, u);
   AICP_IP_BODY(3);
   AICP_IP_TAIL0;
+  AICP_UP_T0;
   pair_done(y);
   AICP_IP_TAIL(3);
+  AICP_UP(kUpPhases + 4);
+}
+
+__global__ __launch_bounds__(kNNBlock) void k_icp_reduce_u(
+    BlockMap m, const PairDesc* __restrict__ pd, PairState* st, const float4* __restrict__ read_c,
+    const int32_t* __restrict__ match, const float* __restrict__ d2, const uint32_t* __restrict__ touched,
+    const float4* __restrict__ bpts, const float4* __restrict__ bnrm, double* slab, IcpParams prm, IcpIterSync y) {
+  AICP_IP_T0;
+  const int pair = m.pair[blockIdx.x];
+  PairState& s = st[pair];
+  if (!s.active) return;
+  const PairDesc& d = pd[pair];
+  icp_reduce_body(m, d, s, read_c, match, d2, touched, bpts, bnrm, slab);
+  AICP_IP_BODY(2);
+  if (!last_arrival(&y.red[pair], d.n_red_blk)) return;
+  AICP_IP_TAIL0;
+  __shared__ UpdLds u;
+  icp_update_body_lds(d, s, slab, prm, u);
+  AICP_IP_TAIL(2);
+  AICP_UP_T0;
+  pair_done(y);
+  AICP_UP(4);
+}
+
+__global__ __launch_bounds__(64) void k_solve6_mem(const double* A, const double* b, double* x, int32_t* path) {
+  __shared__ Solve6Work w;
+  if (threadIdx.x == 0 && blockIdx.x == 0) {
+    for (int i = 0; i < 36; ++i) w.A[i] = A[i];
+    for (int i = 0; i < 6; ++i) w.b[i] = b[i];
+    *path = solve6_mem(w.A, w.b, w.x, w);
+    for (int i = 0; i < 6; ++i) x[i] = w.x[i];
+  }
 }
 
 __global__ void k_finalize(int n_pairs, const PairDesc* __restrict__ pd,
@@ -2677,7 +2844,8 @@
 #if AICP_ITER_PROF
   unsigned long long h[16];
   if (hipMemcpyFromSymbol(h, HIP_SYMBOL(g_iter_prof), sizeof(h)) == hipSuccess) {
-    const char* nm[4] = {"hist_f", "compact_f", "reduce", "update_f(body=slab+solve, tail=active list)"};
+    const char* nm[4] = {"hist_f", "compact_f", "reduce(tail=the last arrival's update, update_in_reduce)",
+                         "update_f(body=slab+solve, tail=active list)"};
     for (int k = 0; k < 4; ++k)
       fprintf(stderr, "[iter prof] %s: body %.2f us avg over %llu, tail %.2f us avg over %llu\n", nm[k],
               h[4 * k + 1] ? h[4 * k] / 100.0 / h[4 * k + 1] : 0.0, h[4 * k + 1],
@@ -2685,6 +2853,22 @@
   }
   unsigned long long z[16] = {};
   (void)hipMemcpyToSymbol(HIP_SYMBOL(g_iter_prof), z, sizeof(z));
+  unsigned long long u[4 * kUpPhases];
+  if (hipMemcpyFromSymbol(u, HIP_SYMBOL(g_up_prof), sizeof(u)) == hipSuccess) {
+    const char* ph[kUpPhases] = {"slab sum (+ state staging)",
+                                 "solve waves (QR rank | LLT, then update_serial on the LLT's wave)",
+                                 "update_serial (the fallback's only)",
+                                 "state write-back", "pair_done + active list"};
+    for (int v = 0; v < 2; ++v)
+      for (int k = 0; k < kUpPhases; ++k) {
+        const unsigned long long *e = u + 2 * (v * kUpPhases + k);
+        if (e[1])
+          fprintf(stderr, "[iter prof] update %s, %s: %.2f us avg over %llu\n", v ? "(icp_update_body)" : "(icp_update_body_lds)",
+                  ph[k], e[0] / 100.0 / e[1], e[1]);
+      }
+  }
+  unsigned long long zu[4 * kUpPhases] = {};
+  (void)hipMemcpyToSymbol(HIP_SYMBOL(g_up_prof), zu, sizeof(zu));
 #endif
 }
 
@@ -2805,8 +2989,13 @@
 }
 void launch_icp_reduce_f(hipStream_t s, BlockMap m, const PairDesc* pd, PairState* st, const float4* read_c,
                          const int32_t* match, const float* d2, const uint32_t* touched, const float4* bpts,
-                         const float4* bnrm, double* slab, const IcpParams& prm, const IcpIterSync& y) {
+                         const float4* bnrm, double* slab, const IcpParams& prm, const IcpIterSync& y,
+                         int update_in_reduce) {
   if (!m.n_blocks) return;
+  if (update_in_reduce) {
+    k_icp_reduce_u<<<m.n_blocks, kNNBlock, 0, s>>>(m, pd, st, read_c, match, d2, touched, bpts, bnrm, slab, prm, y);
+    return;
+  }
   k_icp_reduce<<<m.n_blocks, kNNBlock, 0, s>>>(m, pd, st, read_c, match, d2, touched, bpts, bnrm, slab);
   k_icp_update_f<<<y.np, 256, 0, s>>>(y.pd, y.st, slab, prm, y);
 }
@@ -2844,5 +3033,8 @@
 void launch_solve6(hipStream_t s, const double* A, const double* b, double* x, int32_t* path) {
   k_solve6<<<1, 64, 0, s>>>(A, b, x, path);
 }
-
-}
+void launch_solve6_mem(hipStream_t s, const double* A, const double* b, double* x, int32_t* path) {
+  k_solve6_mem<<<1, 64, 0, s>>>(A, b, x, path);
+}
+
+}
diff --git a/aicp_mapping_amd/csrc/runtime.hpp b/aicp_mapping_amd/csrc/runtime.hpp
--- a/aicp_mapping_amd/csrc/runtime.hpp
+++ b/aicp_mapping_amd/csrc/runtime.hpp
@@ -275,6 +275,7 @@
   uint32_t* poll_host = nullptr;
   uint32_t* poll_dev = nullptr;
   aicp_hip_options opt{};
+  int update_in_reduce = 0;
 };
 constexpr int kBatchPolls = 64;
 
diff --git a/aicp_mapping_amd/csrc/sequence.cpp b/aicp_mapping_amd/csrc/sequence.cpp
--- a/aicp_mapping_amd/csrc/sequence.cpp
+++ b/aicp_mapping_amd/csrc/sequence.cpp
@@ -84,6 +84,7 @@
   hipEvent_t ev_begin = nullptr, ev_end = nullptr;
   std::vector<hipEvent_t> tev;
   aicp_hip_options opt{};
+  int update_in_reduce = 0;
   WorkerPool pool{std::max(1u, std::min(16u, std::thread::hardware_concurrency())) - 1};
   aicp_sequence_timing last{};
   int device = 0;
@@ -949,7 +950,8 @@
     launch_pairs_degenerate_part(st, lp.np_l, lp.gd, lp.gs, dRst, 1);
   }
   launch_icp_reduce_f(st, mred, dDesc, dState, sl.read_c.as<float4>(), sl.match.as<int32_t>(), sl.d2.as<float>(),
-                      sl.touch.as<uint32_t>(), sl.bpts.as<float4>(), sl.bnrm.as<float4>(), sl.slab.as<double>(), ip, y);
+                      sl.touch.as<uint32_t>(), sl.bpts.as<float4>(), sl.bnrm.as<float4>(), sl.slab.as<double>(), ip, y,
+                      S->update_in_reduce);
   HIPC(hipGetLastError());
   ++q.it;
   if (q.it >= cfg->max_iter) q.stop = true;
@@ -1074,6 +1076,7 @@
   }
   SeqState* S = ctx->seq;
   S->opt = ctx->opt;
+  S->update_in_reduce = ctx->update_in_reduce;
   for (SeqSlot& sl : S->slot) {
     sl.used = false;
     for (auto& t : sl.tb) tree_opts(t, S->opt);
diff --git a/include/aicp_hip.h b/include/aicp_hip.h
--- a/include/aicp_hip.h
+++ b/include/aicp_hip.h
@@ -94,6 +94,8 @@
 void aicp_hip_default_options(aicp_hip_options* out);
 int aicp_hip_set_options(aicp_hip_ctx* ctx, const aicp_hip_options* opt);
 int aicp_hip_get_options(const aicp_hip_ctx* ctx, aicp_hip_options* out);
+int aicp_hip_set_update_in_reduce(aicp_hip_ctx* ctx, int on);
+int aicp_hip_get_update_in_reduce(const aicp_hip_ctx* ctx);
 int aicp_hip_test_force_scan_stall(int on);
 
 void aicp_hip_default_config(aicp_icp_config* out);
@@ -233,6 +235,7 @@
                             float* out_limit);
 int aicp_hip_solve6(aicp_hip_ctx* ctx, const double* A, const double* b, double* out_x,
                     int32_t* out_path );
+int aicp_hip_solve6_mem(aicp_hip_ctx* ctx, const double* A, const double* b, double* out_x, int32_t* out_path);
 
 #ifdef __cplusplus
 }
```

New measurement: 2896, median of 3. No clear change (-0.2%).
